# nintendops/DynamicFusion_Body

Hardware: NVIDIA B200
Metric: warped_tsdf_voxels_per_sec (higher is better)
Workload: dtype f32

## Files before the change

### dynamicfusion_body_b200/_capi.py

```python
import ctypes as C
import os

DFB_MAX_K = 8
DFB_MAX_VIEWS = 8
DFB_NODE_REC_FLOATS = 12
DFB_COMM_ID_BYTES = 128
MODE_HYBRID = 0
MODE_EXACT = 1
MODE_FAST_ONLY = 2
MODE_LIST_ONLY = 3
MODE_BRICK_CLASSIFY = 4
MODE_BRICK_STREAM = 5
MODE_BRICK_MIXED = 6
MODE_BRICK_UPDATE = 7

_PKG_DIR = os.path.dirname(os.path.abspath(__file__))
LIB_PATH = os.environ.get("DFB_LIB") or os.path.join(_PKG_DIR, "libdfb_b200.so")

c_f32p = C.POINTER(C.c_float)
c_f64p = C.POINTER(C.c_double)
c_u8p = C.POINTER(C.c_uint8)
c_u16p = C.POINTER(C.c_uint16)
c_u32p = C.POINTER(C.c_uint32)
c_i32p = C.POINTER(C.c_int32)


class Volume(C.Structure):
    _fields_ = [("tsdf", C.c_void_p), ("weight", C.c_void_p),
                ("rx", C.c_int), ("ry", C.c_int), ("rz", C.c_int),
                ("x0", C.c_int), ("x1", C.c_int)]


class WarpField(C.Structure):
    _fields_ = [("node_rec", C.c_void_p), ("node_pos", C.c_void_p), ("node_dq", C.c_void_p),
                ("node_w", C.c_void_p), ("n_nodes", C.c_int), ("k", C.c_int), ("knn", C.c_void_p),
                ("has_lw", C.c_int), ("lw_is_f32", C.c_int), ("lw", C.c_double * 8),
                ("brick_nodes", C.c_void_p), ("brick_count", C.c_void_p), ("brick_pairs", C.c_void_p),
                ("region_nodes", C.c_void_p), ("region_count", C.c_void_p), ("region_pairs", C.c_void_p),
                ("region_rec", C.c_void_p)]


class Views(C.Structure):
    _fields_ = [("n_views", C.c_int), ("depth", C.c_void_p * DFB_MAX_VIEWS),
                ("rows", C.c_int), ("cols", C.c_int),
                ("K", C.c_double * 9), ("Kinv", C.c_double * 9),
                ("has_extrinsics", C.c_int), ("E", (C.c_double * 12) * DFB_MAX_VIEWS)]


class Workspace(C.Structure):
    _fields_ = [("list", C.c_void_p), ("capacity", C.c_uint32), ("counters", C.c_void_p),
                ("brick_cls", C.c_void_p), ("brick_lists", C.c_void_p), ("overflow_bits", C.c_void_p)]


class GNProblem(C.Structure):
    _fields_ = [("n_vert", C.c_int64), ("vertices", C.c_void_p), ("normals", C.c_void_p), ("corr", C.c_void_p),
                ("vert_knn", C.c_void_p), ("n_nodes", C.c_int), ("k", C.c_int), ("node_pos", C.c_void_p),
                ("node_w", C.c_void_p), ("node_nbr", C.c_void_p), ("lw", C.c_double * 8), ("lw_is_f32", C.c_int),
                ("rw", C.c_double), ("huber", C.c_int), ("f_scale", C.c_double), ("order", C.c_void_p)]


class FrameIO(C.Structure):
    _fields_ = [("comm", C.c_void_p), ("comm_prefetch", C.c_void_p), ("root", C.c_int), ("dq_src", C.c_void_p),
                ("prefetch_dst", C.c_void_p), ("prefetch_src", C.c_void_p), ("prefetch_bytes", C.c_int64),
                ("counters_host", C.c_void_p)]


class PointGrid(C.Structure):
    _fields_ = [("pts", C.c_void_p), ("n", C.c_int64), ("origin", C.c_double * 3), ("cell", C.c_double),
                ("dims", C.c_int * 3), ("cell_start", C.c_void_p), ("order", C.c_void_p)]


def declare(lib, prefix="dfb_", device=True):
    vp = C.c_void_p
    sig = {
        "version": ([], C.c_int),
        "last_error": ([], C.c_char_p),
        "nodes_pack": ([vp, vp, vp, C.c_int, vp] + ([vp] if device else []), None if not device else C.c_int),
        "knn_build_volume": ([vp, C.c_int, C.c_int, C.c_int, C.c_int, C.c_int, C.c_int, C.c_int, vp, vp], C.c_int),
        "knn_brick_count": ([C.c_int, C.c_int, C.c_int], C.c_int64),
        "knn_build_volume_radii": ([vp, C.c_int, C.c_int, C.c_int, C.c_int, C.c_int, C.c_int, C.c_int, vp, vp, vp], C.c_int),
        "knn_update_volume": ([vp, C.c_int, C.c_int, C.c_int, C.c_int, C.c_int, C.c_int, C.c_int, C.c_int, vp, vp, vp, vp], C.c_int),
        "brick_nodes_update": ([vp, C.c_int, C.c_int, C.c_int, C.c_int, C.c_int, C.c_int, vp, vp, vp, vp, vp], C.c_int),
        "region_update": ([vp, C.c_int, C.c_int, C.c_int, C.c_int, C.c_int, C.c_int, vp, vp, vp, vp, vp], C.c_int),
        "brick_count": ([C.c_int, C.c_int, C.c_int], C.c_int64),
        "brick_nodes_build": ([vp, C.c_int, C.c_int, C.c_int, C.c_int, C.c_int, C.c_int, vp, vp, vp, vp], C.c_int),
        "region_count": ([C.c_int, C.c_int, C.c_int], C.c_int64),
        "region_build": ([vp, C.c_int, C.c_int, C.c_int, C.c_int, C.c_int, C.c_int, vp, vp, vp, vp], C.c_int),
        "knn_points": ([vp, C.c_int64, vp, C.c_int, C.c_int, vp, vp], C.c_int),
        "tsdf_update_projective": ([C.POINTER(Volume), C.POINTER(WarpField), C.POINTER(Views), C.c_double, C.c_double,
                                    C.c_int, C.POINTER(Workspace), vp, vp, vp], C.c_int),
        "fuse_depth_rigid": ([C.POINTER(Volume), C.c_int, vp, C.c_int, C.c_int, c_f64p, c_f64p, c_f64p, C.c_double,
                              c_f64p, C.c_double, C.c_double, C.c_int, C.POINTER(Workspace), vp, vp, vp], C.c_int),
        "tsdf_update_volume": ([C.POINTER(Volume), C.POINTER(WarpField), vp, C.c_int, C.c_int, C.c_int, C.c_double,
                                C.c_double, C.c_int, C.POINTER(Workspace), vp, vp], C.c_int),
        "warp_points": ([vp, vp, C.c_int64, vp, C.POINTER(WarpField), vp, vp] + ([vp] if device else []), C.c_int),
        "dq_blend_points": ([vp, C.c_int64, vp, C.POINTER(WarpField), vp] + ([vp] if device else []), C.c_int),
        "gn_residuals": ([C.POINTER(GNProblem), vp, C.c_int, vp] + ([vp] if device else []), C.c_int),
        "gn_residuals_lw": ([C.POINTER(GNProblem), vp, C.c_int, c_f64p, C.c_int, vp] + ([vp] if device else []), C.c_int),
        "gn_pattern_rows": ([C.POINTER(GNProblem), vp, vp, vp], C.c_int),
        "gn_pattern_cols": ([C.c_int, vp, vp, vp, vp], C.c_int),
        "gn_normal_eq": ([C.POINTER(GNProblem), vp, vp, vp, C.c_int64, vp, vp, vp] + ([vp] if device else []), C.c_int),
        "gn_lw_normal_eq": ([C.POINTER(GNProblem), vp, c_f64p, vp, vp, vp] + ([vp] if device else []), C.c_int),
        "gn_solve_workspace_doubles": ([C.c_int], C.c_int64),
        "point_grid_scratch_ints": ([C.c_int64], C.c_int64),
        "point_grid_build": ([C.POINTER(PointGrid), vp, vp, vp, vp], C.c_int),
        "point_grid_knn": ([C.POINTER(PointGrid), vp, C.c_int64, C.c_int, vp, vp, vp], C.c_int),
        "corr_select": ([vp, vp, C.c_int64, vp, vp, C.c_int, vp, vp, vp], C.c_int),
        "corr_projective": ([vp, vp, C.c_int64, C.POINTER(Views), C.c_double, C.c_double, vp, vp, vp] + ([vp] if device else []), C.c_int),
        "graph_unsupported": ([vp, C.c_int64, vp, C.c_int, vp, vp, vp, vp], C.c_int),
        "graph_sample_rounds": ([C.POINTER(PointGrid), C.c_double, C.c_int, vp, vp, vp], C.c_int),
        "mc_level_scratch_floats": ([], C.c_int64),
        "mc_level": ([vp, C.c_int64, vp, vp, vp], C.c_int),
        "mc_rows": ([C.c_int, C.c_int, C.c_int], C.c_int64),
        "mc_chunks": ([C.c_int, C.c_int, C.c_int, C.c_int], C.c_int64),
        "mc_count": ([vp, C.c_int, C.c_int, C.c_int, C.c_int, vp, vp, vp, vp, vp], C.c_int),
        "mc_emit": ([vp, C.c_int, C.c_int, C.c_int, C.c_int, vp, vp, vp, vp, vp, vp, vp, vp, vp], C.c_int),
        "gn_solve": ([C.c_int, vp, vp, vp, vp, C.c_double, C.c_int, C.c_double, vp, vp, vp, vp, vp], C.c_int),
        "comm_available": ([], C.c_int),
        "comm_unique_id": ([vp], C.c_int),
        "comm_init": ([C.POINTER(vp), vp, C.c_int, C.c_int, C.c_int], C.c_int),
        "comm_destroy": ([vp], C.c_int),
        "comm_rank": ([vp], C.c_int),
        "comm_world": ([vp], C.c_int),
        "comm_broadcast": ([vp, vp, C.c_int64, C.c_int, vp], C.c_int),
        "comm_broadcast_frame": ([vp, vp, C.c_int64, vp, C.c_int, vp, C.c_int, vp], C.c_int),
        "comm_allreduce_f64": ([vp, vp, C.c_int64, C.c_int, vp], C.c_int),
        "comm_sendrecv": ([vp, vp, C.c_int64, C.c_int, vp, C.c_int64, C.c_int, vp], C.c_int),
        "frame_step_create": ([C.POINTER(vp)], C.c_int),
        "frame_step_destroy": ([vp], None),
        "frame_step_run": ([vp, C.POINTER(Volume), C.POINTER(WarpField), C.POINTER(Views), C.c_double, C.c_double,
                            C.POINTER(Workspace), C.POINTER(FrameIO), vp], C.c_int),
        "frame_step_stats": ([vp, C.POINTER(C.c_int64)], C.c_int),
    }
    for name, (argtypes, restype) in sig.items():
        fn = getattr(lib, prefix + name, None)
        if fn is None:
            continue
        fn.argtypes = argtypes
        fn.restype = restype
    return lib


_lib = None


def lib():
    global _lib
    if _lib is None:
        if not os.path.isfile(LIB_PATH):
            raise ImportError(
                "libdfb_b200.so is not built (%s). There is no CPU fallback: run "
                "`python -m dynamicfusion_body_b200.build` (needs nvcc)." % LIB_PATH)
        _lib = declare(C.CDLL(LIB_PATH))
    return _lib


class DfbError(RuntimeError):
    pass


def check(rc):
    if rc != 0:
        msg = lib().dfb_last_error()
        raise DfbError("libdfb_b200 error %d: %s" % (rc, msg.decode() if msg else "?"))


EXPORTS = [
    "dfb_version", "dfb_last_error", "dfb_nodes_pack", "dfb_knn_build_volume", "dfb_knn_points", "dfb_brick_count", "dfb_brick_nodes_build", "dfb_region_count", "dfb_region_build",
    "dfb_tsdf_update_projective", "dfb_tsdf_update_volume", "dfb_fuse_depth_rigid", "dfb_warp_points", "dfb_dq_blend_points",
    "dfb_gn_residuals", "dfb_gn_residuals_lw", "dfb_gn_pattern_rows", "dfb_gn_pattern_cols", "dfb_gn_normal_eq",
    "dfb_gn_lw_normal_eq", "dfb_gn_solve_workspace_doubles", "dfb_gn_solve",
    "dfb_point_grid_scratch_ints", "dfb_point_grid_build", "dfb_point_grid_knn", "dfb_corr_select", "dfb_corr_projective", "dfb_graph_unsupported", "dfb_graph_sample_rounds",
    "dfb_mc_level_scratch_floats", "dfb_mc_level", "dfb_mc_rows", "dfb_mc_chunks", "dfb_mc_count", "dfb_mc_emit",
    "dfb_knn_brick_count", "dfb_knn_build_volume_radii", "dfb_knn_update_volume", "dfb_brick_nodes_update", "dfb_region_update",
    "dfb_comm_available", "dfb_comm_unique_id", "dfb_comm_init", "dfb_comm_destroy", "dfb_comm_rank", "dfb_comm_world",
    "dfb_comm_broadcast", "dfb_comm_broadcast_frame", "dfb_comm_allreduce_f64", "dfb_comm_sendrecv",
    "dfb_frame_step_create", "dfb_frame_step_destroy", "dfb_frame_step_run", "dfb_frame_step_stats",
]
```

### dynamicfusion_body_b200/csrc/dfb_math.h

```cpp
#pragma once
#include <math.h>
#include <stdint.h>

#if defined(__CUDACC__)
#define DFB_HD __host__ __device__ __forceinline__
#define DFB_HDN inline __host__ __device__
#else
#define DFB_HD inline
#define DFB_HDN inline
#endif

#if !defined(__CUDACC__)
struct float4 { float x, y, z, w; };
#endif

namespace dfb {

#if defined(__CUDA_ARCH__)
DFB_HD float fmul(float a, float b) { return __fmul_rn(a, b); }
DFB_HD float fadd(float a, float b) { return __fadd_rn(a, b); }
DFB_HD float fsub(float a, float b) { return __fsub_rn(a, b); }
DFB_HD float fdiv(float a, float b) { return __fdiv_rn(a, b); }
DFB_HD float fsqrt(float a) { return __fsqrt_rn(a); }
DFB_HD double dmul(double a, double b) { return __dmul_rn(a, b); }
DFB_HD double dadd(double a, double b) { return __dadd_rn(a, b); }
DFB_HD double dsub(double a, double b) { return __dsub_rn(a, b); }
DFB_HD double ddiv(double a, double b) { return __ddiv_rn(a, b); }
DFB_HD double dsqrt(double a) { return __dsqrt_rn(a); }
DFB_HD double drint(double a) { return rint(a); }
#else
DFB_HD float fmul(float a, float b) { volatile float r = a * b; return r; }
DFB_HD float fadd(float a, float b) { volatile float r = a + b; return r; }
DFB_HD float fsub(float a, float b) { volatile float r = a - b; return r; }
DFB_HD float fdiv(float a, float b) { volatile float r = a / b; return r; }
DFB_HD float fsqrt(float a) { volatile float r = sqrtf(a); return r; }
DFB_HD double dmul(double a, double b) { volatile double r = a * b; return r; }
DFB_HD double dadd(double a, double b) { volatile double r = a + b; return r; }
DFB_HD double dsub(double a, double b) { volatile double r = a - b; return r; }
DFB_HD double ddiv(double a, double b) { volatile double r = a / b; return r; }
DFB_HD double dsqrt(double a) { volatile double r = sqrt(a); return r; }
DFB_HD double drint(double a) { return nearbyint(a); }
#endif

struct OpsF {
    typedef float T;
    static DFB_HD T mul(T a, T b) { return fmul(a, b); }
    static DFB_HD T add(T a, T b) { return fadd(a, b); }
    static DFB_HD T sub(T a, T b) { return fsub(a, b); }
};
struct OpsD {
    typedef double T;
    static DFB_HD T mul(T a, T b) { return dmul(a, b); }
    static DFB_HD T add(T a, T b) { return dadd(a, b); }
    static DFB_HD T sub(T a, T b) { return dsub(a, b); }
};

template <class Ops>
DFB_HD void qmul_ref(const typename Ops::T* q1, const typename Ops::T* q0, double* out) {
    typedef typename Ops::T T;
    const T w0 = q0[0], x0 = q0[1], y0 = q0[2], z0 = q0[3];
    const T w1 = q1[0], x1 = q1[1], y1 = q1[2], z1 = q1[3];
    out[0] = (double)Ops::add(Ops::sub(Ops::sub(Ops::mul(-x1, x0), Ops::mul(y1, y0)), Ops::mul(z1, z0)), Ops::mul(w1, w0));
    out[1] = (double)Ops::add(Ops::sub(Ops::add(Ops::mul(x1, w0), Ops::mul(y1, z0)), Ops::mul(z1, y0)), Ops::mul(w1, x0));
    out[2] = (double)Ops::add(Ops::add(Ops::add(Ops::mul(-x1, z0), Ops::mul(y1, w0)), Ops::mul(z1, x0)), Ops::mul(w1, y0));
    out[3] = (double)Ops::add(Ops::add(Ops::sub(Ops::mul(x1, y0), Ops::mul(y1, x0)), Ops::mul(z1, w0)), Ops::mul(w1, z0));
}

DFB_HDN void dqb_warp_ref(const double* dq, bool dq_is_f32, const double* pos, double* out) {
    const float vr[4] = {1.f, 0.f, 0.f, 0.f};
    const float vd[4] = {0.f, (float)pos[0], (float)pos[1], (float)pos[2]};
    double qr[4], qd[4], t0[4], t1[4];
    if (dq_is_f32) {
        const float r[4] = {(float)dq[0], (float)dq[1], (float)dq[2], (float)dq[3]};
        const float d[4] = {(float)dq[4], (float)dq[5], (float)dq[6], (float)dq[7]};
        qmul_ref<OpsF>(r, vr, qr);
        qmul_ref<OpsF>(r, vd, t0);
        qmul_ref<OpsF>(d, vr, t1);
    } else {
        const double vrd[4] = {1.0, 0.0, 0.0, 0.0};
        const double vdd[4] = {0.0, (double)vd[1], (double)vd[2], (double)vd[3]};
        qmul_ref<OpsD>(dq, vrd, qr);
        qmul_ref<OpsD>(dq, vdd, t0);
        qmul_ref<OpsD>(dq + 4, vrd, t1);
    }
    for (int i = 0; i < 4; ++i) qd[i] = dadd(t0[i], t1[i]);
    const double cr[4] = {dq[0], -dq[1], -dq[2], -dq[3]};
    const double cd[4] = {-dq[4], dq[5], dq[6], dq[7]};
    qmul_ref<OpsD>(qr, cd, t0);
    qmul_ref<OpsD>(qd, cr, t1);
    out[0] = dadd(t0[1], t1[1]);
    out[1] = dadd(t0[2], t1[2]);
    out[2] = dadd(t0[3], t1[3]);
}

DFB_HDN void dqb_warp_closed(const double* q, const double* pos, double* out) {
    const double p[3] = {(double)(float)pos[0], (double)(float)pos[1], (double)(float)pos[2]};
    const double w = q[0], x = q[1], y = q[2], z = q[3], dw = q[4], dx = q[5], dy = q[6], dz = q[7];
    const double s = w * w - (x * x + y * y + z * z);
    const double vp = x * p[0] + y * p[1] + z * p[2];
    const double cx = y * p[2] - z * p[1], cy = z * p[0] - x * p[2], cz = x * p[1] - y * p[0];
    out[0] = s * p[0] + 2.0 * (vp * x + w * cx + (w * dx - dw * x + (y * dz - z * dy)));
    out[1] = s * p[1] + 2.0 * (vp * y + w * cy + (w * dy - dw * y + (z * dx - x * dz)));
    out[2] = s * p[2] + 2.0 * (vp * z + w * cz + (w * dz - dw * z + (x * dy - y * dx)));
}

DFB_HDN void dqb_warp_normal_ref(const double* dq, const double* n, double* out) {
    const double rq[8] = {dq[0], dq[1], dq[2], dq[3], 0.0, 0.0, 0.0, 0.0};
    dqb_warp_ref(rq, false, n, out);
}

DFB_HD float norm3_f32_ref(float ax, float ay, float az, float bx, float by, float bz) {
    const float dx = fsub(ax, bx), dy = fsub(ay, by), dz = fsub(az, bz);
    const double s = dadd(dadd((double)fmul(dx, dx), (double)fmul(dy, dy)), (double)fmul(dz, dz));
    return fsqrt((float)s);
}

template <int KT = 0>
DFB_HDN void dq_blend_ref(const float* p, const int* ids, int k_rt, const float* node_pos, const float* node_dq,
                          const float* node_w, double* se3, float* wi_out, double* n2_out = nullptr, const float4* rec = nullptr) {
    double b[8] = {0, 0, 0, 0, 0, 0, 0, 0};
    float wi = 0.f;
    const int k = KT > 0 ? KT : k_rt;
    double wts[KT > 0 ? KT : 1];
    if (KT > 0) {
#pragma unroll
        for (int i = 0; i < (KT > 0 ? KT : 1); ++i) {
            float nx, ny, nz;
            if (rec) { const float4 r0 = rec[3 * (size_t)ids[i]]; nx = r0.x; ny = r0.y; nz = r0.z; }
            else { const float* np_ = node_pos + 3 * (size_t)ids[i]; nx = np_[0]; ny = np_[1]; nz = np_[2]; }
            const float nrm = norm3_f32_ref(p[0], p[1], p[2], nx, ny, nz);
            const float q = fdiv(nrm, fmul(2.0f, node_w[ids[i]]));
            wts[i] = exp((double)fmul(-1.0f, fmul(q, q)));
        }
    }
#pragma unroll
    for (int i = 0; i < k; ++i) {
        const int id = ids[i];
        float npx = 0.f, npy = 0.f, npz = 0.f;
        if (!(KT > 0) || wi_out) {
            if (rec) { const float4 r0 = rec[3 * (size_t)id]; npx = r0.x; npy = r0.y; npz = r0.z; }
            else { const float* np_ = node_pos + 3 * (size_t)id; npx = np_[0]; npy = np_[1]; npz = np_[2]; }
        }
        double w;
        if (KT > 0) {
            w = wts[KT > 0 ? i : 0];
        } else {
            const float nrm = norm3_f32_ref(p[0], p[1], p[2], npx, npy, npz);
            const float two_w = fmul(2.0f, node_w[id]);
            const float q = fdiv(nrm, two_w);
            const float arg = fmul(-1.0f, fmul(q, q));
            w = exp((double)arg);
        }
        const float wf = (float)w;
        float dqi[8];
        if (rec) {
            const float4 r1 = rec[3 * (size_t)id + 1], r2 = rec[3 * (size_t)id + 2];
            dqi[0] = r1.x; dqi[1] = r1.y; dqi[2] = r1.z; dqi[3] = r1.w; dqi[4] = r2.x; dqi[5] = r2.y; dqi[6] = r2.z; dqi[7] = r2.w;
        } else {
            const float* dq_ = node_dq + 8 * (size_t)id;
            for (int c = 0; c < 8; ++c) dqi[c] = dq_[c];
        }
        for (int c = 0; c < 8; ++c) b[c] = dadd(b[c], (double)fmul(wf, dqi[c]));
        if (wi_out) {
            const float nrm2 = norm3_f32_ref(npx, npy, npz, p[0], p[1], p[2]);
            const float term = fdiv(nrm2, (float)k);
            wi = (i == 0) ? term : fadd(wi, term);
        }
    }
    if (wi_out) *wi_out = wi;
    double s = 0.0;
    for (int c = 0; c < 8; ++c) s = dadd(s, dmul(b[c], b[c]));
    if (n2_out) {
        *n2_out = s;
        if (s == 0.0) {
            se3[0] = 1.0;
            for (int c = 1; c < 8; ++c) se3[c] = 0.0;
            *n2_out = 1.0;
        } else {
            for (int c = 0; c < 8; ++c) se3[c] = b[c];
        }
        return;
    }
    const double nrm8 = dsqrt(s);
    if (nrm8 == 0.0) {
        se3[0] = 1.0;
        for (int c = 1; c < 8; ++c) se3[c] = 0.0;
        return;
    }
    for (int c = 0; c < 8; ++c) se3[c] = ddiv(b[c], nrm8);
}

template <int KT = 0>
DFB_HDN void warp_ref(const float* p, const float* nrm_in, const int* ids, int k, const float* node_pos,
                      const float* node_dq, const float* node_w, const double* lw, bool has_lw, bool lw_is_f32,
                      double* out_p, double* out_n, float* wi_out, bool closed_form = false, const float4* rec = nullptr) {
    double pd[3] = {(double)p[0], (double)p[1], (double)p[2]};
    double se3[8];
    if (k > 0) {
        if (closed_form && !(nrm_in && out_n)) {
            double n2;
            dq_blend_ref<KT>(p, ids, k, node_pos, node_dq, node_w, se3, wi_out, &n2, rec);
            dqb_warp_closed(se3, pd, out_p);
            const double inv = 1.0 / n2;
            out_p[0] *= inv; out_p[1] *= inv; out_p[2] *= inv;
        } else {
            dq_blend_ref<KT>(p, ids, k, node_pos, node_dq, node_w, se3, wi_out, nullptr, rec);
            if (closed_form) dqb_warp_closed(se3, pd, out_p);
            else dqb_warp_ref(se3, false, pd, out_p);
        }
    } else {
        out_p[0] = pd[0]; out_p[1] = pd[1]; out_p[2] = pd[2];
    }
    if (has_lw) {
        double t[3] = {out_p[0], out_p[1], out_p[2]};
        if (closed_form && !lw_is_f32) dqb_warp_closed(lw, t, out_p);
        else dqb_warp_ref(lw, lw_is_f32, t, out_p);
    }
    if (nrm_in && out_n) {
        double nd[3] = {(double)nrm_in[0], (double)nrm_in[1], (double)nrm_in[2]};
        if (k > 0) dqb_warp_normal_ref(se3, nd, out_n);
        else { out_n[0] = nd[0]; out_n[1] = nd[1]; out_n[2] = nd[2]; }
        if (has_lw) {
            double t[3] = {out_n[0], out_n[1], out_n[2]};
            dqb_warp_normal_ref(lw, t, out_n);
        }
    }
}

DFB_HD double dot3_ref(const double* r, double a, double b, double c) {
    return dadd(dadd(dmul(r[0], a), dmul(r[1], b)), dmul(r[2], c));
}
DFB_HD double dot4_ref(const double* r, double a, double b, double c, double d) {
    return dadd(dadd(dadd(dmul(r[0], a), dmul(r[1], b)), dmul(r[2], c)), dmul(r[3], d));
}

DFB_HD float fast_exp2(float x) {
#if defined(__CUDA_ARCH__)
    float y;
    asm("ex2.approx.ftz.f32 %0, %1;" : "=f"(y) : "f"(x));
    return y;
#else
    return exp2f(x);
#endif
}
DFB_HD float fast_rcp(float x) {
#if defined(__CUDA_ARCH__)
    float y;
    asm("rcp.approx.ftz.f32 %0, %1;" : "=f"(y) : "f"(x));
    return y;
#else
    return 1.0f / x;
#endif
}

DFB_HD void clamp_update(float& v, float& w, float tdist, float wmax, float scale) {
#if defined(__CUDA_ARCH__)
    v = __fmul_rn(__fmaf_rn(__fmul_rn(scale, v), w, tdist), fast_rcp(__fmul_rn(scale, __fadd_rn(1.0f, w))));
#else
    v = fmul(fmaf(fmul(scale, v), w, tdist), fast_rcp(fmul(scale, fadd(1.0f, w))));
#endif
    w = fminf(fadd(1.0f, w), wmax);
}

DFB_HDN int project_fuse_ref(const double* lpos, const float* depth, int rows, int cols, const double* K,
                             const double* Kinv, double tdist, double scale, double wmax, double* v, double* w) {
    const double p0 = dot3_ref(K, lpos[0], lpos[1], lpos[2]);
    const double p1 = dot3_ref(K + 3, lpos[0], lpos[1], lpos[2]);
    const double p2 = dot3_ref(K + 6, lpos[0], lpos[1], lpos[2]);
    if (p2 == 0.0) return 0;
    const double u = ddiv(p0, p2), vv = ddiv(p1, p2);
    if (!(u >= 0.0 && u < (double)(cols - 1) && vv >= 0.0 && vv < (double)(rows - 1))) return 0;
    const long ui = (long)drint(u), vi = (long)drint(vv);
    const double z = -1.0 * (double)depth[(size_t)vi * cols + ui];
    if (!(z > 0.0)) return 2;
    const double c2 = dot3_ref(Kinv + 6, dmul(z, u), dmul(z, vv), dmul(z, 1.0));
    const double tl = dsub(c2, lpos[2]);
    if (!(tl > -1.0 * tdist)) return 2;
    if (!(tl < tdist)) {
        float vf = (float)*v, wf = (float)*w;
        clamp_update(vf, wf, (float)tdist, (float)wmax, (float)scale);
        *v = (double)vf;
        *w = (double)wf;
        return 3;
    }
    const double m = tl;
    const double wt = *w;
    *v = ddiv(dadd(dmul(dmul(scale, *v), wt), dmul(m, 1.0)), dmul(scale, dadd(1.0, wt)));
    const double s = dadd(1.0, wt);
    *w = (wmax < s) ? wmax : s;
    return 3;
}

DFB_HDN int assoc_projective_ref(const double* w, const double* m, const float* const* depth, int n_views, int rows, int cols,
                                 const double* K, const double* Kinv, const double* E, double max_distance, double min_normal_dot,
                                 double* cost_out, double* corr_out) {
    int best = -1;
    double best_cost = INFINITY, bc[3] = {0.0, 0.0, 0.0};
    const double md2 = dmul(max_distance, max_distance);
    for (int v = 0; v < n_views; ++v) {
        const double* Ev = E ? E + 12 * v : nullptr;
        double l[3], ln[3];
        for (int r = 0; r < 3; ++r) {
            l[r] = Ev ? dot4_ref(Ev + 4 * r, w[0], w[1], w[2], 1.0) : w[r];
            ln[r] = Ev ? dot3_ref(Ev + 4 * r, m[0], m[1], m[2]) : m[r];
        }
        if (!(dot3_ref(ln, l[0], l[1], l[2]) < 0.0)) continue;
        const double p0 = dot3_ref(K, l[0], l[1], l[2]);
        const double p1 = dot3_ref(K + 3, l[0], l[1], l[2]);
        const double p2 = dot3_ref(K + 6, l[0], l[1], l[2]);
        if (p2 == 0.0) continue;
        const double u = ddiv(p0, p2), vv = ddiv(p1, p2);
        if (!(u >= 0.0 && u < (double)(cols - 1) && vv >= 0.0 && vv < (double)(rows - 1))) continue;
        const long ui = (long)drint(u), vi = (long)drint(vv);
        if (ui < 1 || ui > cols - 2 || vi < 1 || vi > rows - 2) continue;
        const float* D = depth[v];
        const long pu[5] = {ui, ui - 1, ui + 1, ui, ui};
        const long pv[5] = {vi, vi, vi, vi - 1, vi + 1};
        double z[5];
        bool ok = true;
        for (int j = 0; j < 5 && ok; ++j) {
            z[j] = -1.0 * (double)D[(size_t)pv[j] * cols + pu[j]];
            ok = z[j] > 0.0 && (j == 0 || fabs(dsub(z[j], z[0])) <= max_distance);
        }
        if (!ok) continue;
        double P[5][3];
        for (int j = 0; j < 5; ++j) {
            const double a = dmul(z[j], (double)pu[j]), b = dmul(z[j], (double)pv[j]), c2 = dmul(z[j], 1.0);
            for (int r = 0; r < 3; ++r) P[j][r] = dot3_ref(Kinv + 3 * r, a, b, c2);
        }
        const double* c = P[0];
        const double du[3] = {dsub(P[2][0], P[1][0]), dsub(P[2][1], P[1][1]), dsub(P[2][2], P[1][2])};
        const double dv[3] = {dsub(P[4][0], P[3][0]), dsub(P[4][1], P[3][1]), dsub(P[4][2], P[3][2])};
        double g[3] = {dsub(dmul(du[1], dv[2]), dmul(du[2], dv[1])), dsub(dmul(du[2], dv[0]), dmul(du[0], dv[2])),
                       dsub(dmul(du[0], dv[1]), dmul(du[1], dv[0]))};
        const double gc = dot3_ref(g, c[0], c[1], c[2]);
        if (gc == 0.0) continue;
        if (gc > 0.0) { g[0] = -g[0]; g[1] = -g[1]; g[2] = -g[2]; }
        const double d[3] = {dsub(l[0], c[0]), dsub(l[1], c[1]), dsub(l[2], c[2])};
        if (!(dot3_ref(d, d[0], d[1], d[2]) <= md2)) continue;
        const double nl = dsqrt(dot3_ref(ln, ln[0], ln[1], ln[2])), ng = dsqrt(dot3_ref(g, g[0], g[1], g[2]));
        if (!(dot3_ref(ln, g[0], g[1], g[2]) >= dmul(dmul(min_normal_dot, nl), ng))) continue;
        const double cost = fabs(dot3_ref(ln, d[0], d[1], d[2]));
        if (!(cost < best_cost)) continue;
        best = v;
        best_cost = cost;
        if (Ev) {
            const double e[3] = {dsub(c[0], Ev[3]), dsub(c[1], Ev[7]), dsub(c[2], Ev[11])};
            for (int j = 0; j < 3; ++j) bc[j] = dadd(dadd(dmul(Ev[j], e[0]), dmul(Ev[4 + j], e[1])), dmul(Ev[8 + j], e[2]));
        } else {
            bc[0] = c[0]; bc[1] = c[1]; bc[2] = c[2];
        }
    }
    *cost_out = best_cost;
    corr_out[0] = bc[0]; corr_out[1] = bc[1]; corr_out[2] = bc[2];
    return best;
}

DFB_HDN bool interpolate_tsdf_ref(const double* pos, const float* t, int rx, int ry, int rz, double* out) {
    const double mn = fmin(fmin(pos[0], pos[1]), pos[2]);
    if (!(mn >= 0.0) || pos[0] > rx - 1 || pos[1] > ry - 1 || pos[2] > rz - 1) return false;
    if (!(pos[0] == pos[0] && pos[1] == pos[1] && pos[2] == pos[2])) return false;
    const double fx = floor(pos[0]), fy = floor(pos[1]), fz = floor(pos[2]);
    const long x0 = (long)fx, y0 = (long)fy, z0 = (long)fz;
    const long x1 = (long)ceil(pos[0]), y1 = (long)ceil(pos[1]), z1 = (long)ceil(pos[2]);
    const double xd = dsub(pos[0], fx), yd = dsub(pos[1], fy), zd = dsub(pos[2], fz);
#define DFB_T(a, b, c) ((double)t[((size_t)(a) * ry + (size_t)(b)) * rz + (size_t)(c)])
    const double c000 = DFB_T(x0, y0, z0), c100 = DFB_T(x1, y0, z0), c001 = DFB_T(x0, y1, z0), c101 = DFB_T(x1, y1, z0);
    const double c010 = DFB_T(x0, y0, z1), c110 = DFB_T(x1, y0, z1), c011 = DFB_T(x0, y1, z1), c111 = DFB_T(x1, y1, z1);
#undef DFB_T
    const double ix = dsub(1.0, xd), iy = dsub(1.0, yd), iz = dsub(1.0, zd);
    const double c00 = dadd(dmul(c000, ix), dmul(c100, xd));
    const double c01 = dadd(dmul(c001, ix), dmul(c101, xd));
    const double c10 = dadd(dmul(c010, ix), dmul(c110, xd));
    const double c11 = dadd(dmul(c011, ix), dmul(c111, xd));
    const double c0 = dadd(dmul(c00, iy), dmul(c10, yd));
    const double c1 = dadd(dmul(c01, iy), dmul(c11, yd));
    *out = dadd(dmul(c0, iz), dmul(c1, zd));
    return true;
}

DFB_HD bool volume_fuse_ref(bool valid, double tl, float wi_f, int k, double tdist, double wmax, double* v, double* w) {
    if (!valid || !(tl > -1.0 * tdist)) return false;
    if (k == 0) {
        const double wt = *w;
        const double m = (tl < tdist) ? tl : tdist;
        *v = ddiv(dadd(dmul(*v, wt), dmul(m, 1.0)), dadd(1.0, wt));
        const double s = dadd(1.0, wt);
        *w = (wmax < s) ? wmax : s;
        return true;
    }
    const double wi = (double)wi_f;
    const double wt = (*w == 0.0) ? wi : *w;
    const double term = (tl < tdist) ? dmul(tl, wi) : (double)fmul((float)tdist, wi_f);
    *v = ddiv(dadd(dmul(*v, wt), term), dadd(wi, wt));
    const double s = dadd(wi, wt);
    *w = (wmax < s) ? wmax : s;
    return true;
}

struct Affine34 {
    float m[12];
};

DFB_HD void dq_apply_unnormalised(const float* b, float px, float py, float pz, float* o) {
    const float w = b[0], x = b[1], y = b[2], z = b[3], dw = b[4], dx = b[5], dy = b[6], dz = b[7];
    const float vv = x * x + y * y + z * z;
    const float s = w * w - vv;
    const float vp = x * px + y * py + z * pz;
    const float cx = y * pz - z * py, cy = z * px - x * pz, cz = x * py - y * px;
    const float tx = w * dx - dw * x + (y * dz - z * dy);
    const float ty = w * dy - dw * y + (z * dx - x * dz);
    const float tz = w * dz - dw * z + (x * dy - y * dx);
    o[0] = s * px + 2.f * (vp * x + w * cx + tx);
    o[1] = s * py + 2.f * (vp * y + w * cy + ty);
    o[2] = s * pz + 2.f * (vp * z + w * cz + tz);
}

inline void dq_to_affine(const double* q, double* A ) {
    const double w = q[0], x = q[1], y = q[2], z = q[3], dw = q[4], dx = q[5], dy = q[6], dz = q[7];
    const double s = w * w - (x * x + y * y + z * z);
    A[0] = s + 2 * x * x;        A[1] = 2 * (x * y - w * z);  A[2] = 2 * (x * z + w * y);
    A[4] = 2 * (x * y + w * z);  A[5] = s + 2 * y * y;        A[6] = 2 * (y * z - w * x);
    A[8] = 2 * (x * z - w * y);  A[9] = 2 * (y * z + w * x);  A[10] = s + 2 * z * z;
    A[3] = 2 * (w * dx - dw * x + (y * dz - z * dy));
    A[7] = 2 * (w * dy - dw * y + (z * dx - x * dz));
    A[11] = 2 * (w * dz - dw * z + (x * dy - y * dx));
}

}
```

### dynamicfusion_body_b200/csrc/dfb_params.h

```cpp
#pragma once
#include <math.h>
#include <stdarg.h>
#include <stdio.h>
#include <string.h>

#include "../../include/dfb.h"
#include "dfb_voxel.h"

namespace dfb {

void set_error(const char* fmt, ...);

#define DFB_REQUIRE(cond, ...)            \
    do {                                  \
        if (!(cond)) {                    \
            dfb::set_error(__VA_ARGS__);  \
            return DFB_ERR_INVALID;       \
        }                                 \
    } while (0)

inline void mat34_mul(const double* A, const double* B, double* C) {
    for (int r = 0; r < 3; ++r)
        for (int c = 0; c < 4; ++c) {
            double s = 0;
            for (int j = 0; j < 3; ++j) s += A[4 * r + j] * B[4 * j + c];
            if (c == 3) s += A[4 * r + 3];
            C[4 * r + c] = s;
        }
}

inline void k_mul34(const double* K, const double* A, double* C) {
    for (int r = 0; r < 3; ++r)
        for (int c = 0; c < 4; ++c) {
            double s = 0;
            for (int j = 0; j < 3; ++j) s += K[3 * r + j] * A[4 * j + c];
            C[4 * r + c] = s;
        }
}

inline double affine_corner_mag(const double* A, double ex, double ey, double ez) {
    double mag = 0;
    for (int c = 0; c < 8; ++c) {
        const double p[3] = {(c & 1) * ex, ((c >> 1) & 1) * ey, ((c >> 2) & 1) * ez};
        for (int r = 0; r < 3; ++r) {
            const double v = A[4 * r] * p[0] + A[4 * r + 1] * p[1] + A[4 * r + 2] * p[2] + A[4 * r + 3];
            mag = fmax(mag, fabs(v));
            for (int j = 0; j < 3; ++j) mag = fmax(mag, fabs(A[4 * r + j] * p[j]));
            mag = fmax(mag, fabs(A[4 * r + 3]));
        }
    }
    return mag;
}

inline int validate_volume(const dfb_volume* vol) {
    DFB_REQUIRE(vol && vol->tsdf && vol->weight, "volume pointers are null");
    DFB_REQUIRE(vol->rx > 0 && vol->ry > 0 && vol->rz > 0, "bad volume resolution");
    DFB_REQUIRE(vol->x0 >= 0 && vol->x1 > vol->x0 && vol->x1 <= vol->rx, "bad slab [%d,%d) of %d", vol->x0, vol->x1, vol->rx);
    DFB_REQUIRE(vol->ry <= 65535 && (vol->x1 - vol->x0) <= 65535, "ry and slab thickness must be <= 65535");
    DFB_REQUIRE((size_t)(vol->x1 - vol->x0) * vol->ry * vol->rz < ((size_t)1 << 32), "slab has >= 2^32 voxels");
    return DFB_OK;
}

inline int validate_warpfield(const dfb_warpfield* wf, bool need_knn) {
    DFB_REQUIRE(wf, "warpfield is null");
    DFB_REQUIRE(wf->k >= 0 && wf->k <= DFB_MAX_K, "k=%d out of range [0,%d]", wf->k, DFB_MAX_K);
    if (wf->k > 0) {
        DFB_REQUIRE(wf->node_rec && wf->node_pos && wf->node_dq && wf->node_w, "node arrays are null");
        DFB_REQUIRE(wf->n_nodes >= wf->k && wf->n_nodes <= 65535, "n_nodes=%d must be in [k,65535]", wf->n_nodes);
        if (need_knn) DFB_REQUIRE(wf->knn, "knn table is null");
    }
    return DFB_OK;
}

inline int validate_ws(const dfb_workspace* ws) {
    DFB_REQUIRE(ws && ws->counters, "workspace/counters are null");
    DFB_REQUIRE(ws->capacity == 0 || ws->list, "workspace list is null");
    return DFB_OK;
}

inline void fill_common(ProjParams& P, const dfb_volume* vol, const dfb_workspace* ws, double tdist, double wmax,
                        uint8_t* mask_out, uint8_t* frustum_out) {
    P.tsdf = vol->tsdf; P.weight = vol->weight;
    P.rx = vol->rx; P.ry = vol->ry; P.rz = vol->rz; P.x0 = vol->x0; P.x1 = vol->x1;
    P.tdist = fabs(tdist); P.wmax = wmax;
    P.tdist_f = (float)fabs(tdist); P.wmax_f = (float)wmax;
    P.list = ws->list; P.capacity = ws->capacity; P.counters = ws->counters; P.overflow_bits = ws->overflow_bits;
    P.mask_out = mask_out; P.frustum_out = frustum_out;
}

inline void fill_intrinsics(ProjParams& P, const double* K, const double* Kinv) {
    for (int i = 0; i < 9; ++i) { P.K[i] = K[i]; P.Kinv[i] = Kinv[i]; }
    for (int i = 0; i < 3; ++i) P.kin[i] = (float)Kinv[6 + i];
    for (int i = 0; i < 6; ++i) P.kf[i] = (float)K[i];
    P.k_pinhole = (K[6] == 0.0 && K[7] == 0.0 && K[8] == 1.0) ? 1 : 0;
    P.knorm = (float)fmax(fabs(K[0]) + fabs(K[1]) + fabs(K[2]), fabs(K[3]) + fabs(K[4]) + fabs(K[5]));
    P.kin_uv = (float)(fabs(Kinv[6]) + fabs(Kinv[7]));
    P.ezf = (float)(fmax(1.0, fabs(K[6]) + fabs(K[7]) + fabs(K[8])) * 1.000001);
}

static const double kIdent34[12] = {1, 0, 0, 0, 0, 1, 0, 0, 0, 0, 1, 0};

inline int build_projective(ProjParams& P, const dfb_volume* vol, const dfb_warpfield* wf, const dfb_views* views,
                            double tdist, double wmax, int mode, const dfb_workspace* ws, uint8_t* mask_out,
                            uint8_t* frustum_out) {
    if (int r = validate_volume(vol)) return r;
    if (int r = validate_warpfield(wf, true)) return r;
    if (int r = validate_ws(ws)) return r;
    DFB_REQUIRE(views && views->n_views >= 1 && views->n_views <= DFB_MAX_VIEWS, "n_views out of range");
    DFB_REQUIRE(views->rows >= 2 && views->cols >= 2, "depth map too small");
    DFB_REQUIRE(mode >= DFB_MODE_HYBRID && mode <= DFB_MODE_BRICK_UPDATE, "bad mode");
    DFB_REQUIRE(wf->k > 0, "projective update needs k >= 1 (use dfb_fuse_depth_rigid for the rigid path)");
    DFB_REQUIRE(tdist != 0, "truncation distance must be non-zero");
    memset(&P, 0, sizeof(P));
    fill_common(P, vol, ws, tdist, wmax, mask_out, frustum_out);
    P.scale = 1.0;
    P.node_rec = reinterpret_cast<const float4*>(wf->node_rec);
    P.node_pos = wf->node_pos; P.node_dq = wf->node_dq; P.node_w = wf->node_w; P.knn = wf->knn; P.k = wf->k;
    P.has_lw = wf->has_lw; P.lw_is_f32 = wf->lw_is_f32;
    for (int i = 0; i < 8; ++i) P.lw[i] = wf->lw[i];
    P.n_views = views->n_views; P.rows = views->rows; P.cols = views->cols; P.has_E = views->has_extrinsics;
    fill_intrinsics(P, views->K, views->Kinv);
    double A[12];
    if (wf->has_lw) dq_to_affine(wf->lw, A);
    else memcpy(A, kIdent34, sizeof(A));
    double mag = fmax(fmax(vol->rx, vol->ry), vol->rz);
    mag = fmax(mag, affine_corner_mag(A, vol->rx, vol->ry, vol->rz));
    double tnorm = 0.0;
    for (int v = 0; v < views->n_views; ++v) {
        DFB_REQUIRE(views->depth[v], "depth[%d] is null", v);
        P.depth[v] = views->depth[v];
        double T[12], PK[12];
        if (views->has_extrinsics) {
            for (int i = 0; i < 12; ++i) P.E[v][i] = views->E[v][i];
            mat34_mul(views->E[v], A, T);
        } else {
            memcpy(T, A, sizeof(T));
        }
        mag = fmax(mag, affine_corner_mag(T, vol->rx, vol->ry, vol->rz));
        k_mul34(views->K, T, PK);
        for (int i = 0; i < 12; ++i) P.vf[v].P[i] = (float)PK[i];
        for (int i = 0; i < 4; ++i) P.vf[v].L[i] = (float)T[8 + i];
        for (int i = 0; i < 12; ++i) P.vf[v].T[i] = (float)T[i];
        for (int r = 0; r < 3; ++r) tnorm = fmax(tnorm, fabs(T[4 * r]) + fabs(T[4 * r + 1]) + fabs(T[4 * r + 2]));
    }
    P.tnorm = (float)(tnorm * 1.000001);
    P.coord_mag = (float)(2.0 * mag + 8.0);
    return DFB_OK;
}

inline int build_rigid(ProjParams& P, const dfb_volume* vol, int tsdf_res, const float* depth, int rows, int cols,
                       const double* lw34, const double* K, const double* Kinv, double scale, const double* center,
                       double tdist, double wmax, int mode, const dfb_workspace* ws, uint8_t* mask_out,
                       uint8_t* frustum_out) {
    if (int r = validate_volume(vol)) return r;
    if (int r = validate_ws(ws)) return r;
    DFB_REQUIRE(depth && lw34 && K && Kinv && center, "null pointer");
    DFB_REQUIRE(rows >= 2 && cols >= 2, "depth map too small");
    DFB_REQUIRE(mode >= DFB_MODE_HYBRID && mode <= DFB_MODE_BRICK_UPDATE, "bad mode");
    DFB_REQUIRE(scale > 0, "scale must be positive");
    DFB_REQUIRE(tdist != 0, "truncation distance must be non-zero");
    memset(&P, 0, sizeof(P));
    fill_common(P, vol, ws, tdist, wmax, mask_out, frustum_out);
    P.scale = scale;
    P.rigid = 1;
    P.k = 0;
    P.g_scale = scale; P.g_half = tsdf_res / 2.0;
    for (int i = 0; i < 3; ++i) P.g_center[i] = center[i];
    for (int i = 0; i < 12; ++i) P.lw34[i] = lw34[i];
    P.n_views = 1; P.rows = rows; P.cols = cols; P.has_E = 0;
    P.depth[0] = depth;
    fill_intrinsics(P, K, Kinv);
    const double G[12] = {scale, 0, 0, center[0] - scale * P.g_half, 0, scale, 0, center[1] - scale * P.g_half,
                          0, 0, scale, center[2] - scale * P.g_half};
    double T[12], PK[12];
    mat34_mul(lw34, G, T);
    k_mul34(K, T, PK);
    for (int i = 0; i < 12; ++i) P.vf[0].P[i] = (float)PK[i];
    for (int i = 0; i < 4; ++i) P.vf[0].L[i] = (float)T[8 + i];
    for (int i = 0; i < 12; ++i) P.vf[0].T[i] = (float)T[i];
    const double mag = fmax(affine_corner_mag(G, vol->rx, vol->ry, vol->rz), affine_corner_mag(T, vol->rx, vol->ry, vol->rz));
    P.coord_mag = (float)(2.0 * mag + 8.0 * scale);
    return DFB_OK;
}

inline int build_volume(VolParams& P, const dfb_volume* vol, const dfb_warpfield* wf, const float* curr, int cx, int cy,
                        int cz, double tdist, double wmax, int mode, const dfb_workspace* ws, uint8_t* mask_out) {
    if (int r = validate_volume(vol)) return r;
    if (int r = validate_warpfield(wf, true)) return r;
    if (int r = validate_ws(ws)) return r;
    DFB_REQUIRE(curr && cx > 0 && cy > 0 && cz > 0, "tsdf of live frame has not been loaded");
    DFB_REQUIRE(mode >= DFB_MODE_HYBRID && mode <= DFB_MODE_BRICK_UPDATE, "bad mode");
    DFB_REQUIRE(tdist != 0, "truncation distance must be non-zero");
    memset(&P, 0, sizeof(P));
    P.tsdf = vol->tsdf; P.weight = vol->weight;
    P.rx = vol->rx; P.ry = vol->ry; P.rz = vol->rz; P.x0 = vol->x0; P.x1 = vol->x1;
    P.node_rec = reinterpret_cast<const float4*>(wf->node_rec);
    P.node_pos = wf->node_pos; P.node_dq = wf->node_dq; P.node_w = wf->node_w; P.knn = wf->knn; P.k = wf->k;
    P.has_lw = wf->has_lw; P.lw_is_f32 = wf->lw_is_f32;
    for (int i = 0; i < 8; ++i) P.lw[i] = wf->lw[i];
    double A[12];
    if (wf->has_lw) dq_to_affine(wf->lw, A);
    else memcpy(A, kIdent34, sizeof(A));
    for (int i = 0; i < 12; ++i) P.A[i] = (float)A[i];
    P.curr = curr; P.cx = cx; P.cy = cy; P.cz = cz;
    P.tdist = fabs(tdist); P.wmax = wmax; P.tdist_f = (float)fabs(tdist); P.wmax_f = (float)wmax;
    double mag = fmax(fmax(vol->rx, vol->ry), vol->rz);
    mag = fmax(mag, affine_corner_mag(A, vol->rx, vol->ry, vol->rz));
    P.coord_mag = (float)(2.0 * mag + 8.0);
    P.list = ws->list; P.capacity = ws->capacity; P.counters = ws->counters; P.overflow_bits = ws->overflow_bits;
    P.mask_out = mask_out;
    return DFB_OK;
}

}
```

### dynamicfusion_body_b200/csrc/dfb_voxel.h

```cpp
#pragma once
#include "dfb_math.h"

namespace dfb {

enum { CLS_SKIP = 0, CLS_CLAMP = 1, CLS_UNCERTAIN = 2 };

struct ViewFast {
    float P[12];
    float L[4];
    float T[12];
};

struct ProjParams {
    float* tsdf;
    float* weight;
    int rx, ry, rz, x0, x1;
    const float4* node_rec;
    const float* node_pos;
    const float* node_dq;
    const float* node_w;
    const uint16_t* knn;
    int k;
    int has_lw, lw_is_f32;
    double lw[8];
    int rigid;
    double g_scale, g_half, g_center[3];
    double lw34[12];
    float G[12];
    int n_views, rows, cols, has_E;
    const float* depth[8];
    double K[9], Kinv[9];
    double E[8][12];
    ViewFast vf[8];
    float kf[6];
    int k_pinhole;
    float kin[3];
    float tnorm;
    float knorm;
    float ezf;
    float kin_uv;
    float coord_mag;
    double tdist, wmax, scale;
    float tdist_f, wmax_f;
    uint32_t* list;
    uint32_t capacity;
    uint32_t* counters;
    uint32_t* overflow_bits;
    uint8_t* mask_out;
    uint8_t* frustum_out;
};

struct VolParams {
    float* tsdf;
    float* weight;
    int rx, ry, rz, x0, x1;
    const float4* node_rec;
    const float* node_pos;
    const float* node_dq;
    const float* node_w;
    const uint16_t* knn;
    int k;
    int has_lw, lw_is_f32;
    double lw[8];
    float A[12];
    const float* curr;
    int cx, cy, cz;
    double tdist, wmax;
    float tdist_f, wmax_f, coord_mag;
    uint32_t* list;
    uint32_t capacity;
    uint32_t* counters;
    uint32_t* overflow_bits;
    uint8_t* mask_out;
};

struct RecGlobal {
    const float4* p;
    DFB_HD float4 ld(size_t i) const { return p[i]; }
};
#if defined(__CUDACC__)
struct RecShared {
    uint32_t base;
    __device__ __forceinline__ float4 ld(size_t i) const {
        float4 r;
        asm("ld.shared.v4.f32 {%0, %1, %2, %3}, [%4];" : "=f"(r.x), "=f"(r.y), "=f"(r.z), "=f"(r.w) : "r"(base + (uint32_t)i * 16u));
        return r;
    }
};
#endif

template <int KMAX, class Rec>
DFB_HD bool blend_warp_fast(const Rec rec, const uint16_t* ids, int k_rt, float px, float py, float pz, float* out,
                            float* amin_out, bool exact_k = false) {
    const int k = exact_k ? KMAX : k_rt;
    float a[KMAX];
    float amax = -3.0e38f, amin = 0.f;
#pragma unroll
    for (int i = 0; i < KMAX; ++i) {
        if (i < k) {
            const float4 r0 = rec.ld(3 * (size_t)ids[i]);
            const float dx = px - r0.x, dy = py - r0.y, dz = pz - r0.z;
            a[i] = (dx * dx + dy * dy + dz * dz) * r0.w;
            amax = fmaxf(amax, a[i]);
            amin = fminf(amin, a[i]);
        }
    }
    *amin_out = amin * 0.69314718f;
    if (!(amax > -125.f)) return false;
    float b[8] = {0.f, 0.f, 0.f, 0.f, 0.f, 0.f, 0.f, 0.f};
#pragma unroll
    for (int i = 0; i < KMAX; ++i) {
        if (i < k) {
            const float w = fast_exp2(a[i] - amax);
            const float4 r1 = rec.ld(3 * (size_t)ids[i] + 1);
            const float4 r2 = rec.ld(3 * (size_t)ids[i] + 2);
            b[0] += w * r1.x; b[1] += w * r1.y; b[2] += w * r1.z; b[3] += w * r1.w;
            b[4] += w * r2.x; b[5] += w * r2.y; b[6] += w * r2.z; b[7] += w * r2.w;
        }
    }
    float n2 = 0.f;
#pragma unroll
    for (int c = 0; c < 8; ++c) n2 += b[c] * b[c];
    if (!(n2 > 1e-30f)) return false;
    float o[3];
    dq_apply_unnormalised(b, px, py, pz, o);
    const float inv = fast_rcp(n2);
    out[0] = o[0] * inv; out[1] = o[1] * inv; out[2] = o[2] * inv;
    return true;
}

DFB_HD float pos_err_bound(float coord_mag, float amin_nat) {
    return 1.1920929e-7f * coord_mag * (32.f - 4.f * amin_nat);
}

DFB_HD int classify_view(float pu, float pv, float pz, float lz, float e, const float* depth, int rows, int cols,
                         const float* kin, float knorm, float ezf, float kin_uv, float tdist, int* frustum_bit) {
    *frustum_bit = 0;
    const float apz = fabsf(pz);
    const float ez = e * ezf;
    if (!(apz > 64.f * ez)) return CLS_UNCERTAIN;
    const float inv = fast_rcp(pz);
    const float u = pu * inv, v = pv * inv;
    const float ainv = fabsf(inv) * 1.02f;
    const float eu = (knorm * e + fabsf(u) * ez) * ainv + 4.8e-7f * fabsf(u) + 1e-6f;
    const float ev = (knorm * e + fabsf(v) * ez) * ainv + 4.8e-7f * fabsf(v) + 1e-6f;
    const float umax = (float)(cols - 1), vmax = (float)(rows - 1);
    if (u < -eu || u >= umax + eu || v < -ev || v >= vmax + ev) return CLS_SKIP;
    if (!(u >= eu && u < umax - eu && v >= ev && v < vmax - ev)) return CLS_UNCERTAIN;
    *frustum_bit = 1;
    const int u0 = (int)rintf(u - eu), u1 = (int)rintf(u + eu);
    const int v0 = (int)rintf(v - ev), v1 = (int)rintf(v + ev);
    const float kz = kin[0] * u + kin[1] * v + kin[2];
    const float et0 = kin_uv * (eu + ev) + 4.8e-7f * fabsf(kz);
    const float et1 = e + 2.4e-7f * fabsf(lz);
    if ((u0 != u1 && v0 != v1) || u1 - u0 > 1 || v1 - v0 > 1) return CLS_UNCERTAIN;
    const float za = -depth[(size_t)v0 * cols + u0];
    const float zb = -depth[(size_t)v1 * cols + u1];
    const float tla = za * kz - lz, tlb = zb * kz - lz;
    const float eta = fabsf(za) * et0 + et1, etb = fabsf(zb) * et0 + et1;
    const bool skip_a = !(za > 0.f) || tla < -tdist - eta, skip_b = !(zb > 0.f) || tlb < -tdist - etb;
    const bool clamp_a = za > 0.f && tla > tdist + eta, clamp_b = zb > 0.f && tlb > tdist + etb;
    if (skip_a && skip_b) return CLS_SKIP;
    if (clamp_a && clamp_b) return CLS_CLAMP;
    return CLS_UNCERTAIN;
}

template <int KT = 0>
DFB_HDN void voxel_projective_exact(const ProjParams& P, int x, int y, int z, const uint16_t* ids16, float* v_io,
                                    float* w_io, int* mask, int* frus) {
    double base[3];
    if (P.rigid) {
        const double idx[3] = {(double)x, (double)y, (double)z};
        for (int c = 0; c < 3; ++c) base[c] = dadd(dmul(P.g_scale, dsub(idx[c], P.g_half)), P.g_center[c]);
    } else {
        const float p[3] = {(float)x, (float)y, (float)z};
        int ids[8];
        if (KT > 0) {
#pragma unroll
            for (int i = 0; i < (KT > 0 ? KT : 1); ++i) ids[i] = ids16[i];
        } else {
            for (int i = 0; i < P.k; ++i) ids[i] = ids16[i];
        }
#ifndef DFB_EXACT_REC
#define DFB_EXACT_REC 0
#endif
        warp_ref<KT>(p, nullptr, ids, P.k, P.node_pos, P.node_dq, P.node_w, P.lw, P.has_lw != 0, P.lw_is_f32 != 0, base,
                     nullptr, nullptr, true, DFB_EXACT_REC ? P.node_rec : nullptr);
    }
    double v = (double)*v_io, w = (double)*w_io;
    int m = 0, f = 0;
    for (int vi = 0; vi < P.n_views; ++vi) {
        double lpos[3];
        if (P.rigid) {
            for (int r = 0; r < 3; ++r) lpos[r] = dot4_ref(P.lw34 + 4 * r, base[0], base[1], base[2], 1.0);
        } else if (P.has_E) {
            for (int r = 0; r < 3; ++r) lpos[r] = dot4_ref(P.E[vi] + 4 * r, base[0], base[1], base[2], 1.0);
        } else {
            lpos[0] = base[0]; lpos[1] = base[1]; lpos[2] = base[2];
        }
        const int r = project_fuse_ref(lpos, P.depth[vi], P.rows, P.cols, P.K, P.Kinv, P.tdist, P.scale, P.wmax, &v, &w);
        if (r & 1) m |= 1 << vi;
        if (r & 2) f |= 1 << vi;
    }
    *v_io = (float)v;
    *w_io = (float)w;
    *mask = m;
    *frus = f;
}

template <int KMAX, bool EXACTK, bool ONEVIEW, class Rec>
DFB_HD int voxel_projective_classify_rec(const ProjParams& P, int x, int y, int z, const uint16_t* ids, int* mask, int* frus,
                                         int views, int m0, int f0, const Rec rec) {
    float pw[3];
    float e;
    if (P.rigid) {
        pw[0] = (float)x; pw[1] = (float)y; pw[2] = (float)z;
        e = 1.1920929e-7f * P.coord_mag * 32.f;
    } else {
        float amin;
        if (!blend_warp_fast<KMAX>(rec, ids, P.k, (float)x, (float)y, (float)z, pw, &amin, EXACTK)) return CLS_UNCERTAIN;
        e = pos_err_bound(P.coord_mag, amin);
    }
    int m = m0, f = f0;
    const int nv = ONEVIEW ? 1 : P.n_views;
#pragma unroll 1
    for (int vi = 0; vi < nv; ++vi) {
        if (!ONEVIEW && !((views >> vi) & 1)) continue;
        const ViewFast& V = P.vf[ONEVIEW ? 0 : vi];
        const float pu = V.P[0] * pw[0] + V.P[1] * pw[1] + V.P[2] * pw[2] + V.P[3];
        const float pv = V.P[4] * pw[0] + V.P[5] * pw[1] + V.P[6] * pw[2] + V.P[7];
        const float pz = V.P[8] * pw[0] + V.P[9] * pw[1] + V.P[10] * pw[2] + V.P[11];
        const float lz = V.L[0] * pw[0] + V.L[1] * pw[1] + V.L[2] * pw[2] + V.L[3];
        int fb;
        const int c = classify_view(pu, pv, pz, lz, e, P.depth[ONEVIEW ? 0 : vi], P.rows, P.cols, P.kin, P.knorm, P.ezf, P.kin_uv, P.tdist_f, &fb);
        if (c == CLS_UNCERTAIN) return CLS_UNCERTAIN;
        if (c == CLS_CLAMP) m |= 1 << vi;
        if (fb) f |= 1 << vi;
    }
    *mask = m;
    *frus = f;
    return m ? CLS_CLAMP : CLS_SKIP;
}

template <int KMAX, bool EXACTK = false, bool ONEVIEW = false>
DFB_HD int voxel_projective_classify(const ProjParams& P, int x, int y, int z, const uint16_t* ids, int* mask, int* frus,
                                     int views = 0xff, int m0 = 0, int f0 = 0) {
    const RecGlobal rec = {P.node_rec};
    return voxel_projective_classify_rec<KMAX, EXACTK, ONEVIEW>(P, x, y, z, ids, mask, frus, views, m0, f0, rec);
}

template <int KT = 0>
DFB_HDN bool voxel_volume_exact(const VolParams& P, int x, int y, int z, const uint16_t* ids16, float* v_io, float* w_io) {
    const float p[3] = {(float)x, (float)y, (float)z};
    int ids[8];
    if (KT > 0) {
#pragma unroll
        for (int i = 0; i < (KT > 0 ? KT : 1); ++i) ids[i] = ids16[i];
    } else {
        for (int i = 0; i < P.k; ++i) ids[i] = ids16[i];
    }
    double pw[3];
    float wi = 0.f;
    warp_ref<KT>(p, nullptr, ids, P.k, P.node_pos, P.node_dq, P.node_w, P.lw, P.has_lw != 0, P.lw_is_f32 != 0, pw, nullptr, &wi, true);
    double tl = 0.0;
    const bool valid = interpolate_tsdf_ref(pw, P.curr, P.cx, P.cy, P.cz, &tl);
    double v = (double)*v_io, w = (double)*w_io;
    const bool upd = volume_fuse_ref(valid, tl, wi, P.k, P.tdist, P.wmax, &v, &w);
    if (upd) { *v_io = (float)v; *w_io = (float)w; }
    return upd;
}

template <int KMAX>
DFB_HD int voxel_volume_classify(const VolParams& P, int x, int y, int z, const uint16_t* ids, float* wi_out) {
    float pw[3];
    float e;
    const float px = (float)x, py = (float)y, pz = (float)z;
    if (P.k > 0) {
        float amin;
        const RecGlobal rec = {P.node_rec};
        if (!blend_warp_fast<KMAX>(rec, ids, P.k, px, py, pz, pw, &amin)) return CLS_UNCERTAIN;
        e = pos_err_bound(P.coord_mag, amin);
    } else {
        pw[0] = px; pw[1] = py; pw[2] = pz;
        e = 1.1920929e-7f * P.coord_mag * 32.f;
    }
    const float qx = P.A[0] * pw[0] + P.A[1] * pw[1] + P.A[2] * pw[2] + P.A[3];
    const float qy = P.A[4] * pw[0] + P.A[5] * pw[1] + P.A[6] * pw[2] + P.A[7];
    const float qz = P.A[8] * pw[0] + P.A[9] * pw[1] + P.A[10] * pw[2] + P.A[11];
    const float mx = (float)(P.cx - 1), my = (float)(P.cy - 1), mz = (float)(P.cz - 1);
    if (qx < -e || qy < -e || qz < -e || qx > mx + e || qy > my + e || qz > mz + e) return CLS_SKIP;
    if (!(qx >= e && qy >= e && qz >= e && qx <= mx - e && qy <= my - e && qz <= mz - e)) return CLS_UNCERTAIN;
    const int x0 = (int)floorf(qx - e), x1 = (int)ceilf(qx + e);
    const int y0 = (int)floorf(qy - e), y1 = (int)ceilf(qy + e);
    const int z0 = (int)floorf(qz - e), z1 = (int)ceilf(qz + e);
    float mn = 3.0e38f, mxc = -3.0e38f;
    for (int a = x0; a <= x1; ++a)
        for (int b = y0; b <= y1; ++b)
            for (int c = z0; c <= z1; ++c) {
                const float t = P.curr[((size_t)a * P.cy + b) * P.cz + c];
                mn = fminf(mn, t);
                mxc = fmaxf(mxc, t);
            }
    if (mxc <= -P.tdist_f * 1.000001f) return CLS_SKIP;
    if (!(mn >= P.tdist_f)) return CLS_UNCERTAIN;
    if (P.k > 0) {
        float wi = 0.f;
        for (int i = 0; i < P.k; ++i) {
            const float4 r0 = P.node_rec[3 * (size_t)ids[i]];
            const float nr = norm3_f32_ref(r0.x, r0.y, r0.z, px, py, pz);
            const float term = fdiv(nr, (float)P.k);
            wi = (i == 0) ? term : fadd(wi, term);
        }
        *wi_out = wi;
    } else {
        *wi_out = 1.f;
    }
    return CLS_CLAMP;
}

}
```

### dynamicfusion_body_b200/csrc/knn.cu

```cuda
#include <stdlib.h>

#include "common.h"
#include "dfb_math.h"

using namespace dfb;

namespace {

constexpr int TILE = 1024;

template <int KMAX>
struct TopK {
    float d[KMAX + 1];
    int id[KMAX + 1];
    __device__ __forceinline__ void init() {
#pragma unroll
        for (int j = 0; j <= KMAX; ++j) { d[j] = 3.0e38f; id[j] = 0; }
    }
    __device__ __forceinline__ void insert(float v, int i, int kk) {
        if (!(v < d[kk])) return;
        d[kk] = v; id[kk] = i;
#pragma unroll
        for (int j = KMAX; j > 0; --j) {
            if (j <= kk && d[j] < d[j - 1]) {
// ... 36 lines not shown
        __syncthreads();
        if (active) {
#pragma unroll 4
            for (int j = 0; j < cnt; ++j) {
                const float4 p = tile[j];
                const float dx = qx - p.x, dy = qy - p.y, dz = qz - p.z;
                const float d2 = dx * dx + dy * dy + dz * dz;
                top.insert(d2, base + j, kk);
            }
        }
    }
    if (!active) return;
    bool ambiguous = false;
#pragma unroll
    for (int j = 0; j < KMAX; ++j)
        if (j < kk && top.d[j + 1] - top.d[j] <= 4.0e-6f * top.d[j + 1]) ambiguous = true;
    if (ambiguous) {
        knn_exact_f64<KMAX>(qx, qy, qz, node_pos, n, k, out);
    } else {
#pragma unroll
        for (int j = 0; j < KMAX; ++j)
            if (j < k) out[j] = top.id[j];
    }
}

template <int KMAX>
__global__ void __launch_bounds__(256) knn_volume_kernel(const float* node_pos, int n, int k, int ry, int rz, int x0,
                                                         uint16_t* knn) {
    __shared__ float4 tile[TILE];
    const int z = blockIdx.x * blockDim.x + threadIdx.x;
    const int y = blockIdx.y;
    const int xs = blockIdx.z;
    const bool in = z < rz;
    int out[KMAX];
    knn_query<KMAX>((float)(xs + x0), (float)y, (float)z, in, node_pos, n, k, tile, out);
    if (!in) return;
    const size_t i = ((size_t)xs * ry + y) * rz + z;
    if (KMAX == 4 && k == 4) {
        uint2 r;
        r.x = (uint32_t)out[0] | ((uint32_t)out[1] << 16);
        r.y = (uint32_t)out[2] | ((uint32_t)out[3] << 16);
        reinterpret_cast<uint2*>(knn)[i] = r;
    } else {
#pragma unroll
        for (int j = 0; j < KMAX; ++j)
            if (j < k) knn[i * (size_t)k + j] = (uint16_t)out[j];
    }
}


constexpr int KB = 8;
constexpr int KCAP = 1024;

template <int KMAX>
__device__ __noinline__ void knn_exact_f64_list(float qx, float qy, float qz, const float4* cand, int nc, int k, int* out) {
    double bd[KMAX];
    int bi[KMAX];
    for (int j = 0; j < KMAX; ++j) { bd[j] = 1.0e300; bi[j] = 0x7fffffff; }
    for (int t = 0; t < nc; ++t) {
        const float4 p = cand[t];
        const int id = __float_as_int(p.w);
        const double dx = dfb::dsub((double)qx, (double)p.x), dy = dfb::dsub((double)qy, (double)p.y), dz = dfb::dsub((double)qz, (double)p.z);
        const double d2 = dfb::dadd(dfb::dadd(dfb::dmul(dx, dx), dfb::dmul(dy, dy)), dfb::dmul(dz, dz));
        if (!(d2 < bd[k - 1] || (d2 == bd[k - 1] && id < bi[k - 1]))) continue;
        int j = k - 1;
        while (j > 0 && (d2 < bd[j - 1] || (d2 == bd[j - 1] && id < bi[j - 1]))) { bd[j] = bd[j - 1]; bi[j] = bi[j - 1]; --j; }
        bd[j] = d2; bi[j] = id;
    }
    for (int j = 0; j < k; ++j) out[j] = bi[j];
}

template <int KMAX>
__global__ void __launch_bounds__(128) knn_brick_kernel(const float* node_pos, int n, int k, int sx, int ry, int rz, int x0, int nby, int nbz,
                                                        uint16_t* knn, float* brick_T, int n_old, uint8_t* dirty) {
    __shared__ float4 cand[KCAP];
    __shared__ float wtop[4][KMAX];
    __shared__ int ncand;
    __shared__ float T2s;
    const int b = blockIdx.x;
    const int bz = b % nbz, by = (b / nbz) % nby, bxs = b / (nbz * nby);
    const int xlo = bxs * KB, ylo = by * KB, zlo = bz * KB;
    const int xhi = min(xlo + KB, sx) - 1, yhi = min(ylo + KB, ry) - 1, zhi = min(zlo + KB, rz) - 1;
    const float cx = 0.5f * (xlo + xhi) + (float)x0, cy = 0.5f * (ylo + yhi), cz = 0.5f * (zlo + zhi);
    const float hx = 0.5f * (xhi - xlo), hy = 0.5f * (yhi - ylo), hz = 0.5f * (zhi - zlo);
    const float hd = sqrtf(hx * hx + hy * hy + hz * hz);
    const int lane = threadIdx.x & 31, wid = threadIdx.x >> 5;
    if (n_old > 0) {
        if (dirty[b] != 2) return;
        __syncthreads();
        if (threadIdx.x == 0) dirty[b] = 1;
    } else if (threadIdx.x == 0 && dirty) {
        dirty[b] = 1;
    }
    float lt[KMAX];
#pragma unroll
    for (int j = 0; j < KMAX; ++j) lt[j] = 3.0e38f;
    for (int t = threadIdx.x; t < n; t += blockDim.x) {
        const float dx = node_pos[3 * t] - cx, dy = node_pos[3 * t + 1] - cy, dz = node_pos[3 * t + 2] - cz;
        float v = dx * dx + dy * dy + dz * dz;
#pragma unroll
        for (int j = 0; j < KMAX; ++j)
            if (j < k && v < lt[j]) { const float tmp = lt[j]; lt[j] = v; v = tmp; }
    }
    for (int j = 0; j < k; ++j) {
        float m = lt[0];
        for (int o = 16; o > 0; o >>= 1) m = fminf(m, __shfl_xor_sync(0xffffffffu, m, o));
        const unsigned who = __ballot_sync(0xffffffffu, lt[0] == m);
        if (lane == __ffs(who) - 1) {
#pragma unroll
            for (int q = 0; q < KMAX - 1; ++q) lt[q] = lt[q + 1];
            lt[KMAX - 1] = 3.0e38f;
        }
        if (lane == 0) wtop[wid][j] = m;
    }
    if (threadIdx.x == 0) ncand = 0;
    __syncthreads();
    if (threadIdx.x == 0) {
        float all[4 * KMAX];
        int m = 0;
        for (int w = 0; w < 4; ++w)
            for (int j = 0; j < k; ++j) all[m++] = wtop[w][j];
        for (int a = 1; a < m; ++a) {
            const float v = all[a];
            int q = a - 1;
            while (q >= 0 && all[q] > v) { all[q + 1] = all[q]; --q; }
            all[q + 1] = v;
        }
        const float T = sqrtf(all[k - 1]) * 1.00001f + 2.f * hd + 1e-3f;
        T2s = T * T * 1.00001f;
        if (brick_T) brick_T[b] = T;
    }
    __syncthreads();
    const float T2 = T2s;
    for (int t = threadIdx.x; t < n; t += blockDim.x) {
        const float px = node_pos[3 * t], py = node_pos[3 * t + 1], pz = node_pos[3 * t + 2];
        const float dx = px - cx, dy = py - cy, dz = pz - cz;
        if (dx * dx + dy * dy + dz * dz <= T2) {
            const int pos = atomicAdd(&ncand, 1);
            if (pos < KCAP) cand[pos] = make_float4(px, py, pz, __int_as_float(t));
        }
    }
    __syncthreads();
    const int nc = ncand;
    const bool overflow = nc > KCAP;
    TopK<KMAX> top[4];
    float qx[4], qy[4], qz[4];
    bool in[4];
#pragma unroll
    for (int q = 0; q < 4; ++q) {
        const int j = threadIdx.x * 4 + q;
        const int z = zlo + (j & 7), y = ylo + ((j >> 3) & 7), xs = xlo + (j >> 6);
        in[q] = xs < sx && y < ry && z < rz;
        qx[q] = (float)(xs + x0); qy[q] = (float)y; qz[q] = (float)z;
        top[q].init();
    }
    const int ntot = overflow ? n : nc;
    const int kk = (ntot > k) ? k : k - 1;
    if (!overflow) {
        for (int t = 0; t < nc; ++t) {
            const float4 p = cand[t];
#pragma unroll
            for (int q = 0; q < 4; ++q) {
                const float dx = qx[q] - p.x, dy = qy[q] - p.y, dz = qz[q] - p.z;
                top[q].insert(dx * dx + dy * dy + dz * dz, __float_as_int(p.w), kk);
            }
        }
    } else {
        for (int base = 0; base < n; base += KCAP) {
            const int cnt = min(KCAP, n - base);
            __syncthreads();
            for (int t = threadIdx.x; t < cnt; t += blockDim.x)
                cand[t] = make_float4(node_pos[3 * (base + t)], node_pos[3 * (base + t) + 1], node_pos[3 * (base + t) + 2], __int_as_float(base + t));
            __syncthreads();
            for (int t = 0; t < cnt; ++t) {
                const float4 p = cand[t];
#pragma unroll
                for (int q = 0; q < 4; ++q) {
                    const float dx = qx[q] - p.x, dy = qy[q] - p.y, dz = qz[q] - p.z;
                    top[q].insert(dx * dx + dy * dy + dz * dz, base + t, kk);
                }
            }
        }
    }
#pragma unroll
    for (int q = 0; q < 4; ++q) {
        if (!in[q]) continue;
        int out[KMAX];
        bool ambiguous = false;
#pragma unroll
        for (int a = 0; a < KMAX; ++a)
            if (a < kk && top[q].d[a + 1] - top[q].d[a] <= 4.0e-6f * top[q].d[a + 1]) ambiguous = true;
        if (ambiguous) {
            if (overflow) knn_exact_f64<KMAX>(qx[q], qy[q], qz[q], node_pos, n, k, out);
            else knn_exact_f64_list<KMAX>(qx[q], qy[q], qz[q], cand, nc, k, out);
        } else {
#pragma unroll
            for (int a = 0; a < KMAX; ++a)
                if (a < k) out[a] = top[q].id[a];
        }
        const int j = threadIdx.x * 4 + q;
        const int z = zlo + (j & 7), y = ylo + ((j >> 3) & 7), xs = xlo + (j >> 6);
        const size_t i = ((size_t)xs * ry + y) * rz + z;
        if (KMAX == 4 && k == 4) {
            uint2 r;
            r.x = (uint32_t)out[0] | ((uint32_t)out[1] << 16);
            r.y = (uint32_t)out[2] | ((uint32_t)out[3] << 16);
            reinterpret_cast<uint2*>(knn)[i] = r;
        } else {
#pragma unroll
            for (int a = 0; a < KMAX; ++a)
                if (a < k) knn[i * (size_t)k + a] = (uint16_t)out[a];
        }
    }
}

constexpr int KNEW = 48;
template <int KMAX>
__global__ void __launch_bounds__(128) knn_merge_kernel(const float* node_pos, int n_old, int n, int k, int sx, int ry, int rz, int x0, int nby, int nbz,
                                                        uint16_t* knn, const float* brick_T, uint8_t* dirty) {
    __shared__ float4 newc[KNEW];
    __shared__ int n_new_s, changed_s;
    const int b = blockIdx.x;
    const int bz = b % nbz, by = (b / nbz) % nby, bxs = b / (nbz * nby);
    const int xlo = bxs * KB, ylo = by * KB, zlo = bz * KB;
    const int xhi = min(xlo + KB, sx) - 1, yhi = min(ylo + KB, ry) - 1, zhi = min(zlo + KB, rz) - 1;
    const float cx = 0.5f * (xlo + xhi) + (float)x0, cy = 0.5f * (ylo + yhi), cz = 0.5f * (zlo + zhi);
    if (threadIdx.x == 0) { n_new_s = 0; changed_s = 0; }
    __syncthreads();
    const float T = brick_T[b];
    const float T2 = T * T * 1.00001f;
    for (int t = n_old + threadIdx.x; t < n; t += blockDim.x) {
        const float px = node_pos[3 * t], py = node_pos[3 * t + 1], pz = node_pos[3 * t + 2];
        const float dx = px - cx, dy = py - cy, dz = pz - cz;
        if (dx * dx + dy * dy + dz * dz <= T2) {
            const int pos = atomicAdd(&n_new_s, 1);
            if (pos < KNEW) newc[pos] = make_float4(px, py, pz, __int_as_float(t));
        }
    }
    __syncthreads();
    const int m = n_new_s;
    if (m == 0 || m > KNEW) {
        if (threadIdx.x == 0) dirty[b] = m == 0 ? 0 : 2;
        return;
    }
    if (threadIdx.x == 0) {
        for (int a = 1; a < m; ++a) {
            const float4 v = newc[a];
            int q = a - 1;
            while (q >= 0 && __float_as_int(newc[q].w) > __float_as_int(v.w)) { newc[q + 1] = newc[q]; --q; }
            newc[q + 1] = v;
        }
    }
    __syncthreads();
    bool changed = false;
    for (int q = 0; q < 4; ++q) {
        const int j = threadIdx.x * 4 + q;
        const int z = zlo + (j & 7), y = ylo + ((j >> 3) & 7), xs = xlo + (j >> 6);
        if (!(xs < sx && y < ry && z < rz)) continue;
        const size_t i = ((size_t)xs * ry + y) * rz + z;
        const double qx = (double)(float)(xs + x0), qy = (double)y, qz = (double)z;
        int id[KMAX];
        double d[KMAX];
#pragma unroll
        for (int a = 0; a < KMAX; ++a) {
            id[a] = 0; d[a] = 1.0e300;
            if (a < k) {
                id[a] = knn[i * (size_t)k + a];
                const float* np_ = node_pos + 3 * (size_t)id[a];
                const double dx = dfb::dsub(qx, (double)np_[0]), dy = dfb::dsub(qy, (double)np_[1]), dz = dfb::dsub(qz, (double)np_[2]);
                d[a] = dfb::dadd(dfb::dadd(dfb::dmul(dx, dx), dfb::dmul(dy, dy)), dfb::dmul(dz, dz));
            }
        }
        bool ch = false;
        for (int t = 0; t < m; ++t) {
            const float4 p = newc[t];
            const double dx = dfb::dsub(qx, (double)p.x), dy = dfb::dsub(qy, (double)p.y), dz = dfb::dsub(qz, (double)p.z);
            const double dn = dfb::dadd(dfb::dadd(dfb::dmul(dx, dx), dfb::dmul(dy, dy)), dfb::dmul(dz, dz));
            if (!(dn < d[k - 1])) continue;
            int idn = __float_as_int(p.w);
            double dcur = dn;
            bool ins = false;
#pragma unroll
            for (int a = 0; a < KMAX; ++a) {
                if (a < k) {
                    if (!ins && dcur < d[a]) ins = true;
                    if (ins) {
                        const double td = d[a]; d[a] = dcur; dcur = td;
                        const int ti = id[a]; id[a] = idn; idn = ti;
                    }
                }
            }
            ch = true;
        }
        if (ch) {
#pragma unroll
            for (int a = 0; a < KMAX; ++a)
                if (a < k) knn[i * (size_t)k + a] = (uint16_t)id[a];
            changed = true;
        }
    }
    if (changed) changed_s = 1;
    __syncthreads();
    if (threadIdx.x == 0) dirty[b] = changed_s ? 1 : 0;
}

template <int KMAX>
__global__ void __launch_bounds__(256) knn_points_kernel(const float* pts, int64_t m, const float* node_pos, int n, int k,
                                                         int32_t* idx) {
    __shared__ float4 tile[TILE];
    const int64_t t = (int64_t)blockIdx.x * blockDim.x + threadIdx.x;
    const bool in = t < m;
    const int64_t tt = in ? t : 0;
    int out[KMAX];
    knn_query<KMAX>(pts[3 * tt], pts[3 * tt + 1], pts[3 * tt + 2], in, node_pos, n, k, tile, out);
    if (!in) return;
#pragma unroll
    for (int j = 0; j < KMAX; ++j)
        if (j < k) idx[t * k + j] = out[j];
}

}

namespace {
int knn_build(const float* node_pos, int n_old, int n_nodes, int k, int rx, int ry, int rz, int x0, int x1, uint16_t* knn, float* brick_T,
              uint8_t* dirty, dfb_stream_t stream) {
    DFB_REQUIRE(node_pos && knn, "null pointer");
    DFB_REQUIRE(k >= 1 && k <= DFB_MAX_K, "k=%d out of range [1,%d]", k, DFB_MAX_K);
    DFB_REQUIRE(n_nodes >= k && n_nodes <= 65535, "n_nodes=%d must be in [k,65535]", n_nodes);
    DFB_REQUIRE(rx > 0 && ry > 0 && rz > 0 && x0 >= 0 && x1 > x0 && x1 <= rx, "bad grid / slab");
    DFB_REQUIRE(ry <= 65535 && (x1 - x0) <= 65535, "ry and slab thickness must be <= 65535");
    DFB_REQUIRE(n_old == 0 || (n_old >= k && n_old <= n_nodes && brick_T), "incremental build needs the radii of a table over >= k nodes");
    cudaStream_t s = (cudaStream_t)stream;
    const char* env = getenv("DFB_KNN_BRUTE");
    const int brute = (env && atoi(env)) ? 1 : 0;
    const int64_t nbx = (x1 - x0 + KB - 1) / KB, nby = (ry + KB - 1) / KB, nbz = (rz + KB - 1) / KB;
    if ((brute && n_old == 0 && !brick_T) || nbx * nby * nbz >= ((int64_t)1 << 31)) {
        DFB_REQUIRE(n_old == 0 && !brick_T, "slab too large for the brick build");
        const int threads = rz >= 256 ? 256 : ((rz + 31) / 32) * 32;
        const dim3 grid((rz + threads - 1) / threads, ry, x1 - x0);
        if (k <= 4) knn_volume_kernel<4><<<grid, threads, 0, s>>>(node_pos, n_nodes, k, ry, rz, x0, knn);
        else knn_volume_kernel<8><<<grid, threads, 0, s>>>(node_pos, n_nodes, k, ry, rz, x0, knn);
        DFB_LAUNCH_CHECK("knn_volume_kernel");
        return DFB_OK;
    }
    const unsigned nb = (unsigned)(nbx * nby * nbz);
    if (n_old > 0) {
        if (k <= 4) knn_merge_kernel<4><<<nb, 128, 0, s>>>(node_pos, n_old, n_nodes, k, x1 - x0, ry, rz, x0, (int)nby, (int)nbz, knn, brick_T, dirty);
        else knn_merge_kernel<8><<<nb, 128, 0, s>>>(node_pos, n_old, n_nodes, k, x1 - x0, ry, rz, x0, (int)nby, (int)nbz, knn, brick_T, dirty);
        DFB_LAUNCH_CHECK("knn_merge_kernel");
        if (n_nodes - n_old <= KNEW) return DFB_OK;
    }
    if (k <= 4) knn_brick_kernel<4><<<nb, 128, 0, s>>>(node_pos, n_nodes, k, x1 - x0, ry, rz, x0, (int)nby, (int)nbz, knn, brick_T, n_old, dirty);
    else knn_brick_kernel<8><<<nb, 128, 0, s>>>(node_pos, n_nodes, k, x1 - x0, ry, rz, x0, (int)nby, (int)nbz, knn, brick_T, n_old, dirty);
    DFB_LAUNCH_CHECK("knn_brick_kernel");
    return DFB_OK;
}
}

extern "C" int dfb_knn_build_volume(const float* node_pos, int n_nodes, int k, int rx, int ry, int rz, int x0, int x1,
                                    uint16_t* knn, dfb_stream_t stream) {
    return knn_build(node_pos, 0, n_nodes, k, rx, ry, rz, x0, x1, knn, nullptr, nullptr, stream);
}

extern "C" int64_t dfb_knn_brick_count(int slab_x, int ry, int rz) {
    return (int64_t)((slab_x + KB - 1) / KB) * ((ry + KB - 1) / KB) * ((rz + KB - 1) / KB);
}

extern "C" int dfb_knn_build_volume_radii(const float* node_pos, int n_nodes, int k, int rx, int ry, int rz, int x0, int x1, uint16_t* knn,
                                          float* brick_radius, dfb_stream_t stream) {
    DFB_REQUIRE(brick_radius, "null pointer");
    return knn_build(node_pos, 0, n_nodes, k, rx, ry, rz, x0, x1, knn, brick_radius, nullptr, stream);
}

extern "C" int dfb_knn_update_volume(const float* node_pos, int n_old, int n_nodes, int k, int rx, int ry, int rz, int x0, int x1, uint16_t* knn,
                                     float* brick_radius, uint8_t* dirty, dfb_stream_t stream) {
    DFB_REQUIRE(brick_radius && dirty, "null pointer");
    DFB_REQUIRE(n_old > 0, "n_old must be positive (use dfb_knn_build_volume_radii for the first build)");
    return knn_build(node_pos, n_old, n_nodes, k, rx, ry, rz, x0, x1, knn, brick_radius, dirty, stream);
}

extern "C" int dfb_knn_points(const float* pts, int64_t m, const float* node_pos, int n_nodes, int k, int32_t* idx,
                              dfb_stream_t stream) {
    DFB_REQUIRE(pts && node_pos && idx, "null pointer");
    DFB_REQUIRE(k >= 1 && k <= DFB_MAX_K, "k=%d out of range [1,%d]", k, DFB_MAX_K);
    DFB_REQUIRE(n_nodes >= k, "n_nodes=%d < k=%d", n_nodes, k);
    DFB_REQUIRE(m >= 0, "negative point count");
    if (m == 0) return DFB_OK;
    const int64_t blocks = (m + 255) / 256;
    cudaStream_t s = (cudaStream_t)stream;
    if (k <= 4) knn_points_kernel<4><<<(unsigned)blocks, 256, 0, s>>>(pts, m, node_pos, n_nodes, k, idx);
    else knn_points_kernel<8><<<(unsigned)blocks, 256, 0, s>>>(pts, m, node_pos, n_nodes, k, idx);
    DFB_LAUNCH_CHECK("knn_points_kernel");
    return DFB_OK;
}
```

### dynamicfusion_body_b200/csrc/tsdf.cu

```cuda
#include <stdlib.h>

#include "common.h"
#include "dfb_params.h"
#include "dfb_brick.h"

using namespace dfb;

namespace {

#ifndef DFB_STREAM_HINTS
#define DFB_STREAM_HINTS 1
#endif
__device__ __forceinline__ float4 ld_stream(const float* p) {
#if DFB_STREAM_HINTS
    return __ldcs(reinterpret_cast<const float4*>(p));
#else
    return *reinterpret_cast<const float4*>(p);
#endif
}
__device__ __forceinline__ void prefetch_l1(const void* p) { asm volatile("prefetch.global.L1 [%0];" ::"l"(p)); }
__device__ __forceinline__ void st_stream(float* p, float4 v) {
#if DFB_STREAM_HINTS
    __stcs(reinterpret_cast<float4*>(p), v);
#else
// ... 512 lines not shown
template <int KMAX, bool EXACTK, bool ONEVIEW, class Rec>
__device__ __forceinline__ void queue_process(const ProjParams& P, const uint8_t* cls, int nb, int nby, int nbz, float sc, const Rec rec,
                                              WarpQueue& Q, int count) {
    const int lane = threadIdx.x & 31;
    const bool act = lane < count;
    const int e = Q.n - count + lane;
    uint32_t i = 0;
    int c = CLS_SKIP, mv = 0, fv = 0;
    float v = 0.f, w = 0.f;
    if (act) {
        i = Q.vox[e];
        v = P.tsdf[i];
        w = P.weight[i];
        const uint32_t xy = Q.xy[e];
        const int xs = (int)(xy >> 16), y = (int)(xy & 0xffffu);
        const int z = (int)(i - ((uint32_t)xs * (uint32_t)P.ry + (uint32_t)y) * (uint32_t)P.rz);
        int views = 0xff, m0 = 0, f0 = 0;
        if (!ONEVIEW) {
            const int b = ((xs / BRICK_X) * nby + y / BRICK_Y) * nbz + z / BRICK_Z;
            f0 = cls[nb + b]; views = cls[2 * nb + b]; m0 = cls[3 * nb + b];
        }
        uint16_t ids[KMAX];
        load_ids<KMAX>(P.knn, i, EXACTK ? KMAX : P.k, ids);
        c = voxel_projective_classify_rec<KMAX, EXACTK, ONEVIEW>(P, xs + P.x0, y, z, ids, &mv, &fv, views, m0, f0, rec);
    }
    push_uncertain(act && c == CLS_UNCERTAIN, i, P.list, P.capacity, P.counters, P.overflow_bits);
    if (act) {
        if (c == CLS_UNCERTAIN) { mv = 0; fv = 0; }
        if (mv) {
            if (ONEVIEW) clamp_update(v, w, P.tdist_f, P.wmax_f, sc);
            else
                for (int vi = 0; vi < P.n_views; ++vi)
                    if (mv & (1 << vi)) clamp_update(v, w, P.tdist_f, P.wmax_f, sc);
            P.tsdf[i] = v;
            P.weight[i] = w;
        }
        if (P.mask_out) P.mask_out[i] = (uint8_t)mv;
        if (P.frustum_out) P.frustum_out[i] = (uint8_t)fv;
    }
    Q.n -= count;
    __syncwarp();
}

template <bool ONEVIEW>
__device__ __forceinline__ uint32_t mixed_layer_quads(const ProjParams& P, const float* rr, int xs, int y, int z0, uint32_t i0, float sc, int views, int m0,
                                                      int f0) {
    const int lane = threadIdx.x & 31;
    QuadView qv[ONEVIEW ? 1 : DFB_MAX_VIEWS];
    const int nv = ONEVIEW ? 1 : P.n_views;
    if (ONEVIEW) {
        const float4* q4 = reinterpret_cast<const float4*>(rr + 16);
        const float4 a = __ldg(q4), b = __ldg(q4 + 1), c = __ldg(q4 + 2), d = __ldg(q4 + 3);
        qv[0].M[0] = a.x; qv[0].M[1] = a.y; qv[0].M[2] = a.z; qv[0].M[3] = a.w;
        qv[0].M[4] = b.x; qv[0].M[5] = b.y; qv[0].M[6] = b.z; qv[0].M[7] = b.w;
        qv[0].M[8] = c.x; qv[0].M[9] = c.y; qv[0].M[10] = c.z; qv[0].M[11] = c.w;
        qv[0].d[0] = d.x; qv[0].d[1] = d.y; qv[0].d[2] = d.z;
    }
    for (int v = 0; v < (ONEVIEW ? 0 : nv); ++v) {
        if (!((views >> v) & 1)) continue;
        float val = 0.f;
        {
            const float* T = P.vf[v].T;
            if (lane < 12) {
                const int r = lane >> 2, c = lane & 3;
                val = T[4 * r] * rr[c] + T[4 * r + 1] * rr[4 + c] + T[4 * r + 2] * rr[8 + c] + (c == 3 ? T[4 * r + 3] : 0.f);
            } else if (lane < 15) {
                const int r = lane - 12;
                const float pad = 2e-3f + 2e-6f * P.coord_mag;
                val = fabsf(T[4 * r]) * (rr[12] + pad) + fabsf(T[4 * r + 1]) * (rr[13] + pad) + fabsf(T[4 * r + 2]) * (rr[14] + pad) +
                      8e-6f * P.coord_mag + 1e-3f;
            }
        }
#pragma unroll
        for (int t = 0; t < 12; ++t) qv[v].M[t] = __shfl_sync(0xffffffffu, val, t);
#pragma unroll
        for (int t = 0; t < 3; ++t) qv[v].d[t] = __shfl_sync(0xffffffffu, val, 12 + t);
    }
    int st[4], mq[4], fq[4];
    quad_pretest(P, qv, xs + P.x0, y, z0, 4, ONEVIEW ? 1 : views, m0, f0, st, mq, fq);
    uint32_t om = 0, bm = 0;
    bool any_upd = false;
#pragma unroll
    for (int q = 0; q < 4; ++q) {
        if (st[q] == QV_BAND) { mq[q] = 0; fq[q] = 0; bm |= 1u << q; }
        if (st[q] == QV_OPEN) om |= 1u << q;
        any_upd |= st[q] == QV_SKIP && mq[q] != 0;
    }
    if (any_upd) {
        const float4 v4 = ld_stream(P.tsdf + i0), w4 = ld_stream(P.weight + i0);
        float v[4] = {v4.x, v4.y, v4.z, v4.w}, w[4] = {w4.x, w4.y, w4.z, w4.w};
#pragma unroll
        for (int q = 0; q < 4; ++q) {
            if (st[q] != QV_SKIP || !mq[q]) continue;
            if (ONEVIEW) clamp_update(v[q], w[q], P.tdist_f, P.wmax_f, sc);
            else
                for (int vi = 0; vi < P.n_views; ++vi)
                    if (mq[q] & (1 << vi)) clamp_update(v[q], w[q], P.tdist_f, P.wmax_f, sc);
        }
        if (!om) {
            st_stream(P.tsdf + i0, make_float4(v[0], v[1], v[2], v[3]));
            st_stream(P.weight + i0, make_float4(w[0], w[1], w[2], w[3]));
        } else {
#pragma unroll
            for (int q = 0; q < 4; ++q)
                if (st[q] == QV_SKIP && mq[q]) { P.tsdf[i0 + q] = v[q]; P.weight[i0 + q] = w[q]; }
        }
    }
    if (P.mask_out || P.frustum_out) {
        if (!om) {
            if (P.mask_out) *reinterpret_cast<uchar4*>(P.mask_out + i0) = make_uchar4(mq[0], mq[1], mq[2], mq[3]);
            if (P.frustum_out) *reinterpret_cast<uchar4*>(P.frustum_out + i0) = make_uchar4(fq[0], fq[1], fq[2], fq[3]);
        } else {
#pragma unroll
            for (int q = 0; q < 4; ++q)
                if (st[q] != QV_OPEN) {
                    if (P.mask_out) P.mask_out[i0 + q] = (uint8_t)mq[q];
                    if (P.frustum_out) P.frustum_out[i0 + q] = (uint8_t)fq[q];
                }
        }
    }
    if (__any_sync(0xffffffffu, bm != 0)) {
        const int mine = __popc(bm);
        int incl = mine;
#pragma unroll
        for (int o = 1; o < 32; o <<= 1) {
            const int up = __shfl_up_sync(0xffffffffu, incl, o);
            if (lane >= o) incl += up;
        }
        const int total = __shfl_sync(0xffffffffu, incl, 31);
        uint32_t base = 0;
        if (lane == 0) base = atomicAdd(P.counters, (uint32_t)total);
        base = __shfl_sync(0xffffffffu, base, 0) + (uint32_t)(incl - mine);
#pragma unroll
        for (int q = 0; q < 4; ++q)
            if ((bm >> q) & 1u) defer_voxel(base++, i0 + q, P.list, P.capacity, P.overflow_bits);
    }
    return om;
}

__device__ __forceinline__ const float* brick_region_rec(const ProjParams& P, const float* region_rec, int bxs, int by, int bz) {
    if (!region_rec || P.rigid) return nullptr;
    const int nry = (P.ry + REGION_Y - 1) / REGION_Y, nrz = (P.rz + REGION_Z - 1) / REGION_Z;
    const uint32_t reg = ((uint32_t)(bxs * BRICK_X / REGION_X) * (uint32_t)nry + (uint32_t)(by * BRICK_Y / REGION_Y)) * (uint32_t)nrz + (uint32_t)(bz * BRICK_Z / REGION_Z);
    const float* rr = region_rec + (size_t)reg * REGION_REC_FLOATS;
    return rr[15] > 0.5f ? rr : nullptr;
}

template <int KMAX, bool EXACTK, bool ONEVIEW, class Rec>
__device__ __forceinline__ uint32_t mixed_layer(const ProjParams& P, const float* region_rec, int nb, int nby, int nbz, const uint8_t* cls, uint32_t entry,
                                                int t128, float sc, const Rec rec, uint32_t* i0_out, uint32_t* xy_out) {
    int bxs, by, bz;
    brick_unpack(entry, bxs, by, bz);
    int views = 0xff, m0 = 0, f0 = 0;
    if (!ONEVIEW) {
        const int b = (bxs * nby + by) * nbz + bz;
        f0 = cls[nb + b]; views = cls[2 * nb + b]; m0 = cls[3 * nb + b];
    }
    int dx, dy, dz;
    brick_lane(t128, dx, dy, dz);
    const bool full = (P.rz & 3) == 0 && (bxs + 1) * BRICK_X <= P.x1 - P.x0 && (by + 1) * BRICK_Y <= P.ry && (bz + 1) * BRICK_Z <= P.rz;
    if (!full) {
        mixed_brick_edge<KMAX, EXACTK, ONEVIEW>(P, bxs, by, bz, dx, dy, dz, sc, views, m0, f0, rec);
        return 0u;
    }
    const int xs = bxs * BRICK_X + dx, y = by * BRICK_Y + dy, z0 = bz * BRICK_Z + dz;
    const uint32_t i0 = (uint32_t)(((size_t)xs * P.ry + y) * P.rz + z0);
    *i0_out = i0;
    *xy_out = ((uint32_t)xs << 16) | (uint32_t)y;
    const float* rr = ONEVIEW ? brick_region_rec(P, region_rec, bxs, by, bz) : nullptr;
    if (!rr) return 0xfu;
    return mixed_layer_quads<ONEVIEW>(P, rr, xs, y, z0, i0, sc, views, m0, f0);
}

template <int KMAX, bool EXACTK, bool ONEVIEW, class Rec>
__device__ __forceinline__ void update_body(const ProjParams& P, const float* region_rec, int nbx, int nby, int nbz, const uint8_t* cls,
                                            const uint32_t* stream_list, uint32_t cnt_s, const uint32_t* mixed_list, uint32_t cnt_m, uint32_t first,
                                            uint32_t stride, uint32_t n_t, int t128, const Rec rec, WarpQueue& Q) {
    const int nb = nbx * nby * nbz;
    const uint32_t share = n_t ? (cnt_s + n_t - 1) / n_t : 0u;
    const int lane = threadIdx.x & 31;
    int dx, dy, dz;
    brick_lane(t128, dx, dy, dz);
    const float sc = (float)P.scale;
    const bool vec = (P.rz & 3) == 0;
    uint32_t n_dqb = 0;
    for (uint32_t t = first;; t += stride) {
        const bool last = !(t < n_t);
        uint32_t om = 0, i0 = 0, xy = 0;
        if (!last) {
            if (t < cnt_m) om = mixed_layer<KMAX, EXACTK, ONEVIEW>(P, region_rec, nb, nby, nbz, cls, mixed_list[t], t128, sc, rec, &i0, &xy);
            const uint32_t s1 = (t + 1) * share < cnt_s ? (t + 1) * share : cnt_s;
            for (uint32_t s = t * share; s < s1; ++s) stream_brick<ONEVIEW>(P, nb, nby, nbz, cls, stream_list[s], dx, dy, dz, sc, vec);
        }
        const bool any = __any_sync(0xffffffffu, om != 0);
        if (om) {
            prefetch_l1(P.knn + (size_t)i0 * P.k);
            prefetch_l1(P.tsdf + i0);
            prefetch_l1(P.weight + i0);
        }
#pragma unroll 1
        for (int half = 0; half < 2; ++half) {
            if (any) {
#pragma unroll
                for (int j = 0; j < 2; ++j) {
                    const int q = 2 * half + j;
                    const bool open = (om >> q) & 1u;
                    const unsigned bo = __ballot_sync(0xffffffffu, open);
                    if (open) {
                        const int pos = Q.n + __popc(bo & ((1u << lane) - 1u));
                        Q.vox[pos] = i0 + (uint32_t)q;
                        Q.xy[pos] = xy;
                    }
                    Q.n += __popc(bo);
                    n_dqb += __popc(bo);
                }
                __syncwarp();
            }
            const int thr = last ? 1 : 32;
            while (Q.n >= thr) queue_process<KMAX, EXACTK, ONEVIEW>(P, cls, nb, nby, nbz, sc, rec, Q, Q.n < 32 ? Q.n : 32);
        }
        if (last) break;
    }
    if (lane == 0 && n_dqb) atomicAdd(P.counters + 4, n_dqb);
}

__global__ void __launch_bounds__(128) brick_stream_kernel(const __grid_constant__ ProjParams P, int nbx, int nby, int nbz,
                                                           const uint8_t* cls, const uint32_t* list) {
    const uint32_t count = P.counters[2];
    int dx, dy, dz;
    brick_lane(threadIdx.x, dx, dy, dz);
    for (uint32_t t = blockIdx.x; t < count; t += gridDim.x)
        stream_brick(P, nbx * nby * nbz, nby, nbz, cls, list[t], dx, dy, dz, (float)P.scale, (P.rz & 3) == 0);
}

template <int KMAX, bool EXACTK, bool ONEVIEW>
__global__ void __launch_bounds__(128) brick_mixed_kernel(const __grid_constant__ ProjParams P, int nbx, int nby, int nbz,
                                                          const uint8_t* cls, const uint32_t* list, const float* region_rec) {
    __shared__ uint32_t s_queue[4][2 * WQ_CAP];
    WarpQueue Q = {s_queue[threadIdx.x >> 5], s_queue[threadIdx.x >> 5] + WQ_CAP, 0};
    const uint32_t count = P.counters[3];
    update_body<KMAX, EXACTK, ONEVIEW>(P, region_rec, nbx, nby, nbz, cls, nullptr, 0u, list, count, blockIdx.x, gridDim.x, count, threadIdx.x,
                                       RecGlobal{P.node_rec}, Q);
}

#ifndef DFB_UPDATE_MINB
#define DFB_UPDATE_MINB 8
#endif
#define DFB_UPDATE_BOUNDS __launch_bounds__(128, DFB_UPDATE_MINB)
template <int KMAX, bool EXACTK, bool ONEVIEW>
__global__ void DFB_UPDATE_BOUNDS brick_update_kernel(const __grid_constant__ ProjParams P, int nbx, int nby, int nbz,
                                                           const uint8_t* cls, const uint32_t* stream_list, const uint32_t* mixed_list,
                                                           const float* region_rec) {
    __shared__ uint32_t s_queue[4][2 * WQ_CAP];
    WarpQueue Q = {s_queue[threadIdx.x >> 5], s_queue[threadIdx.x >> 5] + WQ_CAP, 0};
    const uint32_t cnt_s = P.counters[2], cnt_m = P.counters[3];
    const uint32_t n_t = cnt_m > gridDim.x ? cnt_m : gridDim.x;
    update_body<KMAX, EXACTK, ONEVIEW>(P, region_rec, nbx, nby, nbz, cls, stream_list, cnt_s, mixed_list, cnt_m, blockIdx.x, gridDim.x, n_t, threadIdx.x,
                                       RecGlobal{P.node_rec}, Q);
}

constexpr int UPDATE_SMEM_THREADS = 1024, UPDATE_SMEM_GROUPS = UPDATE_SMEM_THREADS / 128;
constexpr size_t UPDATE_SMEM_MAX_BYTES = 226 * 1024;
template <int KMAX, bool EXACTK, bool ONEVIEW>
__global__ void __launch_bounds__(UPDATE_SMEM_THREADS, 1) brick_update_smem_kernel(const __grid_constant__ ProjParams P, int n_nodes, int nbx, int nby,
                                                                                    int nbz, const uint8_t* cls, const uint32_t* stream_list,
                                                                                    const uint32_t* mixed_list, const float* region_rec) {
    extern __shared__ __align__(128) unsigned char smem_raw[];
    float4* s_rec = reinterpret_cast<float4*>(smem_raw);
    uint32_t* wq = reinterpret_cast<uint32_t*>(smem_raw + (((size_t)n_nodes * DFB_NODE_REC_FLOATS * sizeof(float) + 127) & ~(size_t)127)) +
                   (size_t)(threadIdx.x >> 5) * 2 * WQ_CAP;
    WarpQueue Q = {wq, wq + WQ_CAP, 0};
    __shared__ __align__(8) unsigned long long bar;
    const uint32_t bytes = (uint32_t)n_nodes * (uint32_t)(DFB_NODE_REC_FLOATS * sizeof(float));
    const uint32_t bar_a = (uint32_t)__cvta_generic_to_shared(&bar);
    if (threadIdx.x == 0) {
        asm volatile("mbarrier.init.shared::cta.b64 [%0], 1;" ::"r"(bar_a));
        asm volatile("fence.mbarrier_init.release.cluster;" ::: "memory");
    }
    __syncthreads();
    if (threadIdx.x == 0) {
        asm volatile("mbarrier.arrive.expect_tx.shared::cta.b64 _, [%0], %1;" ::"r"(bar_a), "r"(bytes) : "memory");
        const char* src = reinterpret_cast<const char*>(P.node_rec);
        const uint32_t dst = (uint32_t)__cvta_generic_to_shared(s_rec);
        for (uint32_t off = 0; off < bytes; off += 32768u) {
            const uint32_t n = bytes - off < 32768u ? bytes - off : 32768u;
            asm volatile("cp.async.bulk.shared::cluster.global.mbarrier::complete_tx::bytes [%0], [%1], %2, [%3];" ::"r"(dst + off),
                         "l"(src + off), "r"(n), "r"(bar_a)
                         : "memory");
        }
    }
    const uint32_t cnt_s = P.counters[2], cnt_m = P.counters[3];
    const uint32_t n_groups = gridDim.x * UPDATE_SMEM_GROUPS;
    const uint32_t n_t = cnt_m > n_groups ? cnt_m : n_groups;
    const uint32_t rec_a = (uint32_t)__cvta_generic_to_shared(s_rec);
    {
        uint32_t done = 0;
        while (!done)
            asm volatile("{ .reg .pred p; mbarrier.try_wait.parity.shared::cta.b64 p, [%1], 0; selp.u32 %0, 1, 0, p; }" : "=r"(done) : "r"(bar_a) : "memory");
    }
    update_body<KMAX, EXACTK, ONEVIEW>(P, region_rec, nbx, nby, nbz, cls, stream_list, cnt_s, mixed_list, cnt_m,
                                       blockIdx.x * UPDATE_SMEM_GROUPS + (threadIdx.x >> 7), n_groups, n_t, threadIdx.x & 127, RecShared{rec_a}, Q);
}

template <int KMAX, int KT>
__device__ __forceinline__ void exact_voxel(const ProjParams& P, size_t i, size_t nvox, size_t plane, const uint16_t* ids, float v, float w) {
    int xs, y, z;
    if (nvox <= 0xffffffffull) {
        const uint32_t i32 = (uint32_t)i, plane32 = (uint32_t)plane, rz32 = (uint32_t)P.rz;
        const uint32_t xq = i32 / plane32, rem = i32 - xq * plane32, yq = rem / rz32;
        xs = (int)xq; y = (int)yq; z = (int)(rem - yq * rz32);
    } else {
        xs = (int)(i / plane);
        const size_t rem = i - (size_t)xs * plane;
        y = (int)(rem / P.rz);
        z = (int)(rem - (size_t)y * P.rz);
    }
    int m, f;
    voxel_projective_exact<KT>(P, xs + P.x0, y, z, ids, &v, &w, &m, &f);
    if (m) {
        P.tsdf[i] = v;
        P.weight[i] = w;
    }
    if (P.mask_out) P.mask_out[i] = (uint8_t)m;
    if (P.frustum_out) P.frustum_out[i] = (uint8_t)f;
}

#ifndef DFB_EXACT_MINB
#define DFB_EXACT_MINB 8
#endif
template <int KMAX, int KT>
__global__ void __launch_bounds__(128, DFB_EXACT_MINB) proj_exact_kernel(const __grid_constant__ ProjParams P, int all_mode) {
    const size_t nvox = (size_t)(P.x1 - P.x0) * P.ry * P.rz;
    const uint32_t count = P.counters[0];
    const bool overflow = !all_mode && count > P.capacity;
    const bool sweep_bits = overflow && P.overflow_bits != nullptr;
    const bool use_list = !all_mode && (!overflow || sweep_bits);
    const size_t n = use_list ? (size_t)(overflow ? P.capacity : count) : nvox;
    const size_t plane = (size_t)P.ry * P.rz;
    const int kk = KT > 0 ? KT : P.k;
    uint32_t done = 0;
    if (use_list && KT > 0 && !P.rigid && nvox <= 0xffffffffull) {
        const uint32_t stride = gridDim.x * blockDim.x, cnt = (uint32_t)n;
        uint32_t t = blockIdx.x * blockDim.x + threadIdx.x;
        if (t < cnt) {
            uint32_t i0 = P.list[t];
            uint32_t i1 = t + stride < cnt && t + stride >= t ? P.list[t + stride] : i0;
            uint16_t ids0[KMAX];
            load_ids<KMAX>(P.knn, i0, KMAX, ids0);
            float v0 = P.tsdf[i0], w0 = P.weight[i0];
            for (;;) {
                const uint32_t tn = t + stride, tnn = tn + stride;
                const bool has1 = tn < cnt && tn > t;
                const uint32_t i2 = (has1 && tnn < cnt && tnn > tn) ? P.list[tnn] : i1;
                uint16_t ids1[KMAX];
                load_ids<KMAX>(P.knn, i1, KMAX, ids1);
                const float v1 = P.tsdf[i1], w1 = P.weight[i1];
                exact_voxel<KMAX, KT>(P, i0, nvox, plane, ids0, v0, w0);
                ++done;
                if (!has1) break;
                t = tn; i0 = i1; i1 = i2; v0 = v1; w0 = w1;
#pragma unroll
                for (int j = 0; j < KMAX; ++j) ids0[j] = ids1[j];
            }
        }
    } else {
        for (size_t t = (size_t)blockIdx.x * blockDim.x + threadIdx.x; t < n; t += (size_t)gridDim.x * blockDim.x) {
            const size_t i = use_list ? (size_t)P.list[t] : t;
            uint16_t ids[KMAX];
            if (!P.rigid) load_ids<KMAX>(P.knn, i, kk, ids);
            if (!use_list && !all_mode) {
                const size_t xq = i / plane, rem = i - xq * plane;
                int m0, f0;
                if (voxel_projective_classify<KMAX>(P, (int)xq + P.x0, (int)(rem / P.rz), (int)(rem % P.rz), ids, &m0, &f0) != CLS_UNCERTAIN) continue;
            }
            exact_voxel<KMAX, KT>(P, i, nvox, plane, ids, P.tsdf[i], P.weight[i]);
            ++done;
        }
    }
    if (sweep_bits) {
        const size_t nwords = (nvox + 31) / 32;
        const size_t warp0 = ((size_t)blockIdx.x * blockDim.x + threadIdx.x) >> 5, nwarps = ((size_t)gridDim.x * blockDim.x) >> 5;
        const int lane = threadIdx.x & 31;
        for (size_t wd = warp0; wd < nwords; wd += nwarps) {
            const uint32_t bits = P.overflow_bits[wd];
            if (!bits) continue;
            __syncwarp();
            if (lane == 0) P.overflow_bits[wd] = 0u;
            if ((bits >> lane) & 1u) {
                const size_t i = wd * 32 + (size_t)lane;
                uint16_t ids[KMAX];
                if (!P.rigid) load_ids<KMAX>(P.knn, i, kk, ids);
                exact_voxel<KMAX, KT>(P, i, nvox, plane, ids, P.tsdf[i], P.weight[i]);
                ++done;
            }
        }
    }
    for (int o = 16; o > 0; o >>= 1) done += __shfl_xor_sync(0xffffffffu, done, o);
    if ((threadIdx.x & 31) == 0 && done) atomicAdd(P.counters + 1, done);
}

#ifndef DFB_VOL_FAST_MINB
#define DFB_VOL_FAST_MINB 6
#endif
template <int KMAX>
__global__ void __launch_bounds__(256, DFB_VOL_FAST_MINB) vol_fast_kernel(const __grid_constant__ VolParams P) {
    const int z = blockIdx.x * blockDim.x + threadIdx.x;
    const int y = blockIdx.y;
    const int xs = blockIdx.z;
    const bool in = z < P.rz;
    const size_t i = ((size_t)xs * P.ry + y) * P.rz + (in ? z : 0);
    int cls = CLS_SKIP;
    float wi = 0.f;
    if (in) {
        uint16_t ids[KMAX];
        if (P.k > 0) load_ids<KMAX>(P.knn, i, P.k, ids);
        cls = voxel_volume_classify<KMAX>(P, xs + P.x0, y, z, ids, &wi);
    }
    push_uncertain(in && cls == CLS_UNCERTAIN, (uint32_t)i, P.list, P.capacity, P.counters, P.overflow_bits);
    if (!in || cls == CLS_UNCERTAIN) return;
    if (cls == CLS_CLAMP) {
        float v = P.tsdf[i], w = P.weight[i];
        if (P.k > 0) {
            const float wt = (w == 0.f) ? wi : w;
            v = (v * wt + fmul(P.tdist_f, wi)) / (wi + wt);
            w = fminf(wi + wt, P.wmax_f);
        } else {
            v = (v * w + P.tdist_f) / (1.0f + w);
            w = fminf(1.0f + w, P.wmax_f);
        }
        P.tsdf[i] = v;
        P.weight[i] = w;
    }
    if (P.mask_out) P.mask_out[i] = (cls == CLS_CLAMP) ? 1 : 0;
}

template <int KMAX, int KT>
__device__ __forceinline__ void vol_exact_voxel(const VolParams& P, size_t i, size_t plane) {
    int xs, y, z;
    if (plane * (size_t)(P.x1 - P.x0) <= 0xffffffffull) {
        const uint32_t i32 = (uint32_t)i, plane32 = (uint32_t)plane, rz32 = (uint32_t)P.rz;
        const uint32_t xq = i32 / plane32, rem = i32 - xq * plane32, yq = rem / rz32;
        xs = (int)xq; y = (int)yq; z = (int)(rem - yq * rz32);
    } else {
        xs = (int)(i / plane);
        const size_t rem = i - (size_t)xs * plane;
        y = (int)(rem / P.rz);
        z = (int)(rem - (size_t)y * P.rz);
    }
    uint16_t ids[KMAX];
    if (P.k > 0) load_ids<KMAX>(P.knn, i, P.k, ids);
    float v = P.tsdf[i], w = P.weight[i];
    const bool upd = voxel_volume_exact<KT>(P, xs + P.x0, y, z, ids, &v, &w);
    if (upd) {
        P.tsdf[i] = v;
        P.weight[i] = w;
    }
    if (P.mask_out) P.mask_out[i] = upd ? 1 : 0;
}

#ifndef DFB_VOL_EXACT_MINB
#define DFB_VOL_EXACT_MINB 8
#endif
template <int KMAX, int KT>
__global__ void __launch_bounds__(128, DFB_VOL_EXACT_MINB) vol_exact_kernel(const __grid_constant__ VolParams P, int all_mode) {
    const size_t nvox = (size_t)(P.x1 - P.x0) * P.ry * P.rz;
    const uint32_t count = P.counters[0];
    const bool overflow = !all_mode && count > P.capacity;
    const bool sweep_bits = overflow && P.overflow_bits != nullptr;
    const bool use_list = !all_mode && (!overflow || sweep_bits);
    const size_t n = use_list ? (size_t)(overflow ? P.capacity : count) : nvox;
    const size_t plane = (size_t)P.ry * P.rz;
    uint32_t done = 0;
    for (size_t t = (size_t)blockIdx.x * blockDim.x + threadIdx.x; t < n; t += (size_t)gridDim.x * blockDim.x) {
        const size_t i = use_list ? (size_t)P.list[t] : t;
        if (!use_list && !all_mode) {
            const int xs = (int)(i / plane);
            const size_t rem = i - (size_t)xs * plane;
            uint16_t ids[KMAX];
            if (P.k > 0) load_ids<KMAX>(P.knn, i, P.k, ids);
            float wi;
            if (voxel_volume_classify<KMAX>(P, xs + P.x0, (int)(rem / P.rz), (int)(rem % P.rz), ids, &wi) != CLS_UNCERTAIN) continue;
        }
        vol_exact_voxel<KMAX, KT>(P, i, plane);
        ++done;
    }
    if (sweep_bits) {
        const size_t nwords = (nvox + 31) / 32;
        const size_t warp0 = ((size_t)blockIdx.x * blockDim.x + threadIdx.x) >> 5, nwarps = ((size_t)gridDim.x * blockDim.x) >> 5;
        const int lane = threadIdx.x & 31;
        for (size_t wd = warp0; wd < nwords; wd += nwarps) {
            const uint32_t bits = P.overflow_bits[wd];
            if (!bits) continue;
            __syncwarp();
            if (lane == 0) P.overflow_bits[wd] = 0u;
            if ((bits >> lane) & 1u) {
                vol_exact_voxel<KMAX, KT>(P, wd * 32 + (size_t)lane, plane);
                ++done;
            }
        }
    }
    for (int o = 16; o > 0; o >>= 1) done += __shfl_xor_sync(0xffffffffu, done, o);
    if ((threadIdx.x & 31) == 0 && done) atomicAdd(P.counters + 1, done);
}

__global__ void warp_points_kernel(const float* pts, const float* normals, int64_t m, const int32_t* idx, int k,
                                   const float* node_pos, const float* node_dq, const float* node_w,
                                   const __grid_constant__ dfb_warpfield wf, double* out_p, double* out_n) {
    for (int64_t t = (int64_t)blockIdx.x * blockDim.x + threadIdx.x; t < m; t += (int64_t)gridDim.x * blockDim.x) {
        int ids[DFB_MAX_K];
        for (int j = 0; j < k; ++j) ids[j] = idx[t * k + j];
        double op[3], on[3];
        warp_ref(pts + 3 * t, normals ? normals + 3 * t : nullptr, ids, k, node_pos, node_dq, node_w, wf.lw, wf.has_lw != 0,
                 wf.lw_is_f32 != 0, op, on, nullptr);
        for (int c = 0; c < 3; ++c) out_p[3 * t + c] = op[c];
        if (normals && out_n)
            for (int c = 0; c < 3; ++c) out_n[3 * t + c] = on[c];
    }
}

__global__ void dq_blend_points_kernel(const float* pts, int64_t m, const int32_t* idx, int k, const float* node_pos,
                                       const float* node_dq, const float* node_w, double* out) {
    for (int64_t t = (int64_t)blockIdx.x * blockDim.x + threadIdx.x; t < m; t += (int64_t)gridDim.x * blockDim.x) {
        int ids[DFB_MAX_K];
        for (int j = 0; j < k; ++j) ids[j] = idx[t * k + j];
        double se3[8];
        dq_blend_ref(pts + 3 * t, ids, k, node_pos, node_dq, node_w, se3, nullptr);
        for (int c = 0; c < 8; ++c) out[8 * t + c] = se3[c];
    }
}

__global__ void nodes_pack_kernel(const float* pos, const float* dq, const float* w, int n, float* rec) {
    const int i = blockIdx.x * blockDim.x + threadIdx.x;
    if (i >= n) return;
    float* r = rec + (size_t)i * DFB_NODE_REC_FLOATS;
    r[0] = pos[3 * i]; r[1] = pos[3 * i + 1]; r[2] = pos[3 * i + 2];
    const double ww = (double)w[i];
    r[3] = (float)(-1.4426950408889634 / (4.0 * ww * ww));
    for (int c = 0; c < 8; ++c) r[4 + c] = dq[8 * i + c];
}

dim3 fast_grid(const dfb_volume* vol, int& threads) {
    threads = vol->rz >= 256 ? 256 : ((vol->rz + 31) / 32) * 32;
    return dim3((vol->rz + threads - 1) / threads, vol->ry, vol->x1 - vol->x0);
}

int exact_blocks(size_t nvox) {
    static int per_sm = 0;
    if (per_sm == 0) { const char* e = getenv("DFB_EXACT_CTAS_PER_SM"); per_sm = e ? atoi(e) : 32; if (per_sm < 1) per_sm = 32; }
    const size_t want = (nvox + 127) / 128, cap = (size_t)148 * per_sm;
    return (int)(want < cap ? (want ? want : 1) : cap);
}

struct BrickArgs {
    int n_nodes;
    const uint16_t* nodes;
    const uint8_t* count;
    const uint32_t* pairs;
    const uint16_t* rnodes;
    const uint8_t* rcount;
    const uint32_t* rpairs;
    float* rrec;
    uint8_t* cls;
    uint32_t* lists;
};

int run_projective(ProjParams& P, int mode, cudaStream_t s, const dfb_volume* vol, const BrickArgs& B) {
    const bool bricks = B.cls != nullptr && B.lists != nullptr && (P.rigid || (B.nodes != nullptr && B.count != nullptr));
    const bool do_classify = mode == DFB_MODE_HYBRID || mode == DFB_MODE_FAST_ONLY || mode == DFB_MODE_BRICK_CLASSIFY;
    const bool do_stream = mode == DFB_MODE_HYBRID || mode == DFB_MODE_FAST_ONLY || mode == DFB_MODE_BRICK_STREAM || mode == DFB_MODE_BRICK_UPDATE;
    const bool do_mixed = mode == DFB_MODE_HYBRID || mode == DFB_MODE_FAST_ONLY || mode == DFB_MODE_BRICK_MIXED || mode == DFB_MODE_BRICK_UPDATE;
    if (mode >= DFB_MODE_BRICK_CLASSIFY) DFB_REQUIRE(bricks, "brick modes need the brick workspace / candidate sets");
    if (mode != DFB_MODE_HYBRID && mode != DFB_MODE_EXACT) P.overflow_bits = nullptr;
    if (mode == DFB_MODE_HYBRID || mode == DFB_MODE_EXACT || mode == DFB_MODE_FAST_ONLY || mode == DFB_MODE_BRICK_CLASSIFY)
        DFB_CUDA(cudaMemsetAsync(P.counters, 0, 8 * sizeof(uint32_t), s));
    const size_t nvox = (size_t)(P.x1 - P.x0) * P.ry * P.rz;
    if (mode != DFB_MODE_EXACT && mode != DFB_MODE_LIST_ONLY) {
        if (bricks) {
            const int nbx = (P.x1 - P.x0 + BRICK_X - 1) / BRICK_X, nby = (P.ry + BRICK_Y - 1) / BRICK_Y, nbz = (P.rz + BRICK_Z - 1) / BRICK_Z;
            const int nb = nbx * nby * nbz;
            DFB_REQUIRE(nbx <= BRICK_PACK_MAX_XY && nby <= BRICK_PACK_MAX_XY && nbz <= BRICK_PACK_MAX_Z,
                        "volume too large for the brick work lists (4096 x 4096 x 131072 voxels per slab)");
            const float* rrec = nullptr;
            const bool have_regions = !P.rigid && B.rnodes && B.rcount && B.rpairs && B.rrec;
            uint32_t* stream_list = B.lists;
            uint32_t* mixed_list = B.lists + nb;
            const bool classified = false;
            if (have_regions) {
                rrec = B.rrec;
                if (do_classify) {
                    const int nrx = (P.x1 - P.x0 + REGION_X - 1) / REGION_X, nry = (P.ry + REGION_Y - 1) / REGION_Y, nrz = (P.rz + REGION_Z - 1) / REGION_Z;
                    region_bounds_kernel<<<dim3(nrz, nry, nrx), DFB_REGION_THREADS, 0, s>>>(P, B.rnodes, B.rcount, B.rpairs, nry, nrz, B.rrec);
                    DFB_LAUNCH_CHECK("region_bounds_kernel");
                }
            }
            static int upd_per_sm = 0;
            if (upd_per_sm == 0) { const char* e = getenv("DFB_UPDATE_CTAS_PER_SM"); upd_per_sm = e ? atoi(e) : 16; if (upd_per_sm < 1) upd_per_sm = 16; }
            const int grid = nb < 148 * upd_per_sm ? nb : 148 * upd_per_sm;
            if (do_classify && !classified) {
                static int G = 0;
                if (G == 0) { const char* e = getenv("DFB_CLASSIFY_G"); G = e ? atoi(e) : 8; }
                const int per_cta = 128 / G;
                const int nb_pad = ((nbx + 3) / 4) * ((nby + 3) / 4) * nbz * 16;
                const int cgrid = (nb_pad + per_cta - 1) / per_cta < 148 * 32 ? (nb_pad + per_cta - 1) / per_cta : 148 * 32;
                if (G == 1) brick_classify_kernel<1><<<cgrid, 128, 0, s>>>(P, B.nodes, B.count, B.pairs, rrec, nbx, nby, nbz, B.cls, stream_list, mixed_list);
                else if (G == 2) brick_classify_kernel<2><<<cgrid, 128, 0, s>>>(P, B.nodes, B.count, B.pairs, rrec, nbx, nby, nbz, B.cls, stream_list, mixed_list);
                else if (G == 4) brick_classify_kernel<4><<<cgrid, 128, 0, s>>>(P, B.nodes, B.count, B.pairs, rrec, nbx, nby, nbz, B.cls, stream_list, mixed_list);
                else if (G == 16) brick_classify_kernel<16><<<cgrid, 128, 0, s>>>(P, B.nodes, B.count, B.pairs, rrec, nbx, nby, nbz, B.cls, stream_list, mixed_list);
                else if (G == 32) brick_classify_kernel<32><<<cgrid, 128, 0, s>>>(P, B.nodes, B.count, B.pairs, rrec, nbx, nby, nbz, B.cls, stream_list, mixed_list);
                else brick_classify_kernel<8><<<cgrid, 128, 0, s>>>(P, B.nodes, B.count, B.pairs, rrec, nbx, nby, nbz, B.cls, stream_list, mixed_list);
                DFB_LAUNCH_CHECK("brick_classify_kernel");
            }
            if (do_stream && do_mixed) {
#define DFB_BRICK_DISPATCH(KERNEL, ...)                                                                                  \
    do {                                                                                                                 \
        const bool one = P.n_views == 1;                                                                                 \
        if (P.k == 4 && !P.rigid) { if (one) KERNEL<4, true, true><<<grid, 128, 0, s>>>(__VA_ARGS__); else KERNEL<4, true, false><<<grid, 128, 0, s>>>(__VA_ARGS__); } \
        else if (P.k == 8 && !P.rigid) { if (one) KERNEL<8, true, true><<<grid, 128, 0, s>>>(__VA_ARGS__); else KERNEL<8, true, false><<<grid, 128, 0, s>>>(__VA_ARGS__); } \
        else if (P.k <= 4) { if (one) KERNEL<4, false, true><<<grid, 128, 0, s>>>(__VA_ARGS__); else KERNEL<4, false, false><<<grid, 128, 0, s>>>(__VA_ARGS__); } \
        else { if (one) KERNEL<8, false, true><<<grid, 128, 0, s>>>(__VA_ARGS__); else KERNEL<8, false, false><<<grid, 128, 0, s>>>(__VA_ARGS__); } \
    } while (0)
                static int smem_env = -2;
                if (smem_env == -2) { const char* e = getenv("DFB_UPDATE_SMEM"); smem_env = e ? atoi(e) : -1; }
                const int use_smem = smem_env >= 0 ? smem_env : (P.n_views > 1 || P.k > 4);
                static int use_quads = -1;
                if (use_quads < 0) { const char* e = getenv("DFB_QUADS"); use_quads = e ? atoi(e) : 1; }
                const float* qrec = use_quads ? rrec : nullptr;
                const size_t rec_bytes = (((size_t)B.n_nodes * DFB_NODE_REC_FLOATS * sizeof(float) + 127) & ~(size_t)127) + (UPDATE_SMEM_THREADS / 32) * WQ_BYTES;
                if (use_smem && !P.rigid && B.n_nodes > 0 && rec_bytes <= UPDATE_SMEM_MAX_BYTES) {
                    static int n_sm = 0;
                    if (n_sm == 0) {
                        int dev = 0;
                        DFB_CUDA(cudaGetDevice(&dev));
                        DFB_CUDA(cudaDeviceGetAttribute(&n_sm, cudaDevAttrMultiProcessorCount, dev));
                    }
                    const int sgrid = nb < n_sm * UPDATE_SMEM_GROUPS ? (nb + UPDATE_SMEM_GROUPS - 1) / UPDATE_SMEM_GROUPS : n_sm;
#define DFB_SMEM_LAUNCH(K_, E_, O_)                                                                                              \
    do {                                                                                                                         \
        DFB_CUDA(cudaFuncSetAttribute(brick_update_smem_kernel<K_, E_, O_>, cudaFuncAttributeMaxDynamicSharedMemorySize,        \
                                      (int)UPDATE_SMEM_MAX_BYTES));                                                              \
        brick_update_smem_kernel<K_, E_, O_><<<sgrid, UPDATE_SMEM_THREADS, rec_bytes, s>>>(P, B.n_nodes, nbx, nby, nbz, B.cls,   \
                                                                                          stream_list, mixed_list, qrec);      \
    } while (0)
                    const bool one = P.n_views == 1;
                    if (P.k == 4) { if (one) DFB_SMEM_LAUNCH(4, true, true); else DFB_SMEM_LAUNCH(4, true, false); }
                    else if (P.k == 8) { if (one) DFB_SMEM_LAUNCH(8, true, true); else DFB_SMEM_LAUNCH(8, true, false); }
                    else if (P.k < 4) { if (one) DFB_SMEM_LAUNCH(4, false, true); else DFB_SMEM_LAUNCH(4, false, false); }
                    else { if (one) DFB_SMEM_LAUNCH(8, false, true); else DFB_SMEM_LAUNCH(8, false, false); }
                    DFB_LAUNCH_CHECK("brick_update_smem_kernel");
                } else {
                    DFB_BRICK_DISPATCH(brick_update_kernel, P, nbx, nby, nbz, B.cls, stream_list, mixed_list, qrec);
                    DFB_LAUNCH_CHECK("brick_update_kernel");
                }
            } else if (do_stream) {
                brick_stream_kernel<<<grid, 128, 0, s>>>(P, nbx, nby, nbz, B.cls, stream_list);
                DFB_LAUNCH_CHECK("brick_stream_kernel");
            } else if (do_mixed) {
                static int use_quads_m = -1;
                if (use_quads_m < 0) { const char* e = getenv("DFB_QUADS"); use_quads_m = e ? atoi(e) : 1; }
                DFB_BRICK_DISPATCH(brick_mixed_kernel, P, nbx, nby, nbz, B.cls, mixed_list, use_quads_m ? rrec : nullptr);
                DFB_LAUNCH_CHECK("brick_mixed_kernel");
            }
        } else {
            int threads;
            const dim3 grid = fast_grid(vol, threads);
            if (P.k <= 4) proj_fast_kernel<4><<<grid, threads, 0, s>>>(P);
            else proj_fast_kernel<8><<<grid, threads, 0, s>>>(P);
            DFB_LAUNCH_CHECK("proj_fast_kernel");
        }
        if (mode != DFB_MODE_HYBRID) return DFB_OK;
    }
    const int all = mode == DFB_MODE_EXACT ? 1 : 0;
    if (P.k == 4 && !P.rigid) proj_exact_kernel<4, 4><<<exact_blocks(nvox), 128, 0, s>>>(P, all);
    else if (P.k == 8 && !P.rigid) proj_exact_kernel<8, 8><<<exact_blocks(nvox), 128, 0, s>>>(P, all);
    else if (P.k <= 4) proj_exact_kernel<4, 0><<<exact_blocks(nvox), 128, 0, s>>>(P, all);
    else proj_exact_kernel<8, 0><<<exact_blocks(nvox), 128, 0, s>>>(P, all);
    DFB_LAUNCH_CHECK("proj_exact_kernel");
    return DFB_OK;
}

}

extern "C" int dfb_nodes_pack(const float* node_pos, const float* node_dq, const float* node_w, int n_nodes,
                              float* node_rec, dfb_stream_t stream) {
    DFB_REQUIRE(node_pos && node_dq && node_w && node_rec, "null pointer");
    DFB_REQUIRE(n_nodes > 0, "n_nodes must be positive");
    nodes_pack_kernel<<<(n_nodes + 127) / 128, 128, 0, (cudaStream_t)stream>>>(node_pos, node_dq, node_w, n_nodes, node_rec);
    DFB_LAUNCH_CHECK("nodes_pack_kernel");
    return DFB_OK;
}

extern "C" int dfb_tsdf_update_projective(const dfb_volume* vol, const dfb_warpfield* wf, const dfb_views* views,
                                          double tdist, double wmax, int mode, const dfb_workspace* ws,
                                          uint8_t* mask_out, uint8_t* frustum_out, dfb_stream_t stream) {
    ProjParams P;
    if (int r = build_projective(P, vol, wf, views, tdist, wmax, mode, ws, mask_out, frustum_out)) return r;
    const BrickArgs B = {wf->n_nodes, wf->brick_nodes, wf->brick_count, wf->brick_pairs, wf->region_nodes, wf->region_count, wf->region_pairs, wf->region_rec,
                         ws->brick_cls, ws->brick_lists};
    return run_projective(P, mode, (cudaStream_t)stream, vol, B);
}

extern "C" int dfb_fuse_depth_rigid(const dfb_volume* vol, int tsdf_res, const float* depth, int rows, int cols,
                                    const double lw34[12], const double K[9], const double Kinv[9], double scale,
                                    const double center[3], double tdist, double wmax, int mode,
                                    const dfb_workspace* ws, uint8_t* mask_out, uint8_t* frustum_out,
                                    dfb_stream_t stream) {
    ProjParams P;
    if (int r = build_rigid(P, vol, tsdf_res, depth, rows, cols, lw34, K, Kinv, scale, center, tdist, wmax, mode, ws,
                            mask_out, frustum_out))
        return r;
    const BrickArgs B = {0, nullptr, nullptr, nullptr, nullptr, nullptr, nullptr, nullptr, ws->brick_cls, ws->brick_lists};
    return run_projective(P, mode, (cudaStream_t)stream, vol, B);
}

extern "C" int dfb_tsdf_update_volume(const dfb_volume* vol, const dfb_warpfield* wf, const float* curr, int cx,
                                      int cy, int cz, double tdist, double wmax, int mode, const dfb_workspace* ws,
                                      uint8_t* mask_out, dfb_stream_t stream) {
    VolParams P;
    if (int r = build_volume(P, vol, wf, curr, cx, cy, cz, tdist, wmax, mode, ws, mask_out)) return r;
    cudaStream_t s = (cudaStream_t)stream;
    if (mode != DFB_MODE_HYBRID && mode != DFB_MODE_EXACT) P.overflow_bits = nullptr;
    if (mode != DFB_MODE_LIST_ONLY) DFB_CUDA(cudaMemsetAsync(P.counters, 0, 8 * sizeof(uint32_t), s));
    const size_t nvox = (size_t)(P.x1 - P.x0) * P.ry * P.rz;
    if (mode == DFB_MODE_HYBRID || mode == DFB_MODE_FAST_ONLY) {
        int threads;
        const dim3 grid = fast_grid(vol, threads);
        if (P.k <= 4) vol_fast_kernel<4><<<grid, threads, 0, s>>>(P);
        else vol_fast_kernel<8><<<grid, threads, 0, s>>>(P);
        DFB_LAUNCH_CHECK("vol_fast_kernel");
        if (mode == DFB_MODE_FAST_ONLY) return DFB_OK;
    }
    const int all = mode == DFB_MODE_EXACT ? 1 : 0;
    if (P.k == 4) vol_exact_kernel<4, 4><<<exact_blocks(nvox), 128, 0, s>>>(P, all);
    else if (P.k == 8) vol_exact_kernel<8, 8><<<exact_blocks(nvox), 128, 0, s>>>(P, all);
    else if (P.k <= 4) vol_exact_kernel<4, 0><<<exact_blocks(nvox), 128, 0, s>>>(P, all);
    else vol_exact_kernel<8, 0><<<exact_blocks(nvox), 128, 0, s>>>(P, all);
    DFB_LAUNCH_CHECK("vol_exact_kernel");
    return DFB_OK;
}

extern "C" int dfb_warp_points(const float* pts, const float* normals, int64_t m, const int32_t* idx,
                               const dfb_warpfield* wf, double* out_pts, double* out_normals, dfb_stream_t stream) {
    if (int r = validate_warpfield(wf, false)) return r;
    DFB_REQUIRE(pts && out_pts && m >= 0, "null pointer / negative count");
    DFB_REQUIRE(wf->k == 0 || idx, "neighbour indices are null");
    if (m == 0) return DFB_OK;
    const int blocks = (int)((m + 127) / 128 < 148 * 8 ? (m + 127) / 128 : 148 * 8);
    warp_points_kernel<<<blocks, 128, 0, (cudaStream_t)stream>>>(pts, normals, m, idx, wf->k, wf->node_pos, wf->node_dq,
                                                                 wf->node_w, *wf, out_pts, out_normals);
    DFB_LAUNCH_CHECK("warp_points_kernel");
    return DFB_OK;
}

extern "C" int dfb_dq_blend_points(const float* pts, int64_t m, const int32_t* idx, const dfb_warpfield* wf, double* out_dq,
                                   dfb_stream_t stream) {
    if (int r = validate_warpfield(wf, false)) return r;
    DFB_REQUIRE(pts && idx && out_dq && m >= 0 && wf->k > 0, "bad arguments");
    if (m == 0) return DFB_OK;
    const int blocks = (int)((m + 127) / 128 < 148 * 8 ? (m + 127) / 128 : 148 * 8);
    dq_blend_points_kernel<<<blocks, 128, 0, (cudaStream_t)stream>>>(pts, m, idx, wf->k, wf->node_pos, wf->node_dq, wf->node_w, out_dq);
    DFB_LAUNCH_CHECK("dq_blend_points_kernel");
    return DFB_OK;
}

extern "C" int64_t dfb_brick_count(int sx, int ry, int rz) {
    return (int64_t)((sx + BRICK_X - 1) / BRICK_X) * ((ry + BRICK_Y - 1) / BRICK_Y) * ((rz + BRICK_Z - 1) / BRICK_Z);
}

extern "C" int dfb_brick_nodes_build(const uint16_t* knn, int k, int rx, int ry, int rz, int x0, int x1, uint16_t* brick_nodes,
                                     uint8_t* brick_count, uint32_t* brick_pairs, dfb_stream_t stream) {
    return dfb_brick_nodes_update(knn, k, rx, ry, rz, x0, x1, nullptr, brick_nodes, brick_count, brick_pairs, stream);
}

extern "C" int dfb_brick_nodes_update(const uint16_t* knn, int k, int rx, int ry, int rz, int x0, int x1, const uint8_t* dirty8, uint16_t* brick_nodes,
                                      uint8_t* brick_count, uint32_t* brick_pairs, dfb_stream_t stream) {
    DFB_REQUIRE(knn && brick_nodes && brick_count && brick_pairs, "null pointer");
    DFB_REQUIRE(k >= 1 && k <= DFB_MAX_K && rx > 0 && ry > 0 && rz > 0 && x0 >= 0 && x1 > x0 && x1 <= rx, "bad arguments");
    const int sx = x1 - x0;
    const int nby = (ry + BRICK_Y - 1) / BRICK_Y, nbz = (rz + BRICK_Z - 1) / BRICK_Z;
    const int64_t nb = dfb_brick_count(sx, ry, rz);
    DFB_REQUIRE(nb < ((int64_t)1 << 31), "too many bricks");
    brick_nodes_kernel<<<(unsigned)nb, 128, 0, (cudaStream_t)stream>>>(knn, k, sx, ry, rz, nby, nbz, brick_nodes, brick_count, brick_pairs, dirty8);
    DFB_LAUNCH_CHECK("brick_nodes_kernel");
    return DFB_OK;
}

extern "C" int64_t dfb_region_count(int sx, int ry, int rz) {
    return (int64_t)((sx + REGION_X - 1) / REGION_X) * ((ry + REGION_Y - 1) / REGION_Y) * ((rz + REGION_Z - 1) / REGION_Z);
}

extern "C" int dfb_region_build(const uint16_t* knn, int k, int rx, int ry, int rz, int x0, int x1, uint16_t* region_nodes,
                                uint8_t* region_count, uint32_t* region_pairs, dfb_stream_t stream) {
    return dfb_region_update(knn, k, rx, ry, rz, x0, x1, nullptr, region_nodes, region_count, region_pairs, stream);
}

extern "C" int dfb_region_update(const uint16_t* knn, int k, int rx, int ry, int rz, int x0, int x1, const uint8_t* dirty8, uint16_t* region_nodes,
                                 uint8_t* region_count, uint32_t* region_pairs, dfb_stream_t stream) {
    DFB_REQUIRE(knn && region_nodes && region_count && region_pairs, "null pointer");
    DFB_REQUIRE(k >= 1 && k <= DFB_MAX_K && rx > 0 && ry > 0 && rz > 0 && x0 >= 0 && x1 > x0 && x1 <= rx, "bad arguments");
    const int sx = x1 - x0;
    const int nry = (ry + REGION_Y - 1) / REGION_Y, nrz = (rz + REGION_Z - 1) / REGION_Z;
    const int64_t nr = dfb_region_count(sx, ry, rz);
    DFB_REQUIRE(nr < ((int64_t)1 << 31), "too many regions");
    region_build_kernel<<<(unsigned)nr, 256, 0, (cudaStream_t)stream>>>(knn, k, sx, ry, rz, nry, nrz, region_nodes, region_count, region_pairs, dirty8);
    DFB_LAUNCH_CHECK("region_build_kernel");
    return DFB_OK;
// ... 2 lines not shown
```

### dynamicfusion_body_b200/engine.py

```python
import ctypes as C
import os

import numpy as np
import torch

from . import _capi


USE_REGIONS = True


def _stream():
    return C.c_void_p(torch.cuda.current_stream().cuda_stream)


def _ptr(t):
    return C.c_void_p(t.data_ptr()) if t is not None else None


def _require_cuda(device):
    if not torch.cuda.is_available():
        raise RuntimeError("dynamicfusion_body_b200 needs a CUDA device (B200); there is no CPU path")
    return torch.device(device if device is not None else "cuda:%d" % torch.cuda.current_device())


def _to_dev(a, dtype, device):
    if isinstance(a, torch.Tensor):
        return a.to(device=device, dtype=dtype).contiguous()
    a = np.ascontiguousarray(a)
    if not a.flags.writeable:
        a = a.copy()
    return torch.from_numpy(a).to(device=device, dtype=dtype).contiguous()


class Workspace:

    def __init__(self, n_voxels, device, fraction=0.25, n_bricks=0):
        self.capacity = int(max(1024, n_voxels * fraction))
        self.list = torch.empty(self.capacity, dtype=torch.int32, device=device)
        self.counters = torch.zeros(8, dtype=torch.int32, device=device)
        self.n_bricks = int(n_bricks)
        self.brick_cls = torch.zeros(4 * self.n_bricks, dtype=torch.uint8, device=device) if n_bricks else None
        self.brick_lists = torch.zeros(2 * self.n_bricks, dtype=torch.int32, device=device) if n_bricks else None
        self.overflow_bits = torch.zeros((int(n_voxels) + 31) // 32, dtype=torch.int32, device=device)

    def struct(self, use_bricks=True):
        s = _capi.Workspace()
        s.list = self.list.data_ptr()
        s.capacity = self.capacity
        s.counters = self.counters.data_ptr()
        s.overflow_bits = self.overflow_bits.data_ptr()
        if use_bricks and self.brick_cls is not None:
            s.brick_cls = self.brick_cls.data_ptr()
            s.brick_lists = self.brick_lists.data_ptr()
        return s

    def _decode(self, c):
        c = c.astype(np.int64) & 0xffffffff
        return {"deferred": int(c[0]), "exact_processed": int(c[1]), "bricks_streamed": int(c[2]), "bricks_mixed": int(c[3]),
                "bricks": self.n_bricks, "dqb_voxels": int(c[4])}

    def stats(self):
        return self._decode(self.counters.cpu().numpy())

    def stats_async(self):
        if not hasattr(self, "_pinned"):
            self._pinned = [torch.empty(8, dtype=torch.int32).pin_memory() for _ in range(4)]
            self._pin_i = 0
        buf = self._pinned[self._pin_i % len(self._pinned)]
        self._pin_i += 1
        buf.copy_(self.counters, non_blocking=True)
        ev = torch.cuda.Event()
        ev.record()
        ws = self

        class _Pending:
            def result(self):
                ev.synchronize()
                return ws._decode(buf.numpy().copy())
        return _Pending()


class DeviceVolume:

    def __init__(self, res, x0=0, x1=None, device=None, tsdf=None, weight=None, fill=None):
        self.device = _require_cuda(device)
        self.res = tuple(int(r) for r in res)
        self.x0 = int(x0)
        self.x1 = int(self.res[0] if x1 is None else x1)
        shape = (self.x1 - self.x0, self.res[1], self.res[2])
        if tsdf is not None:
            self.tsdf = _to_dev(tsdf, torch.float32, self.device).reshape(shape)
        else:
            self.tsdf = torch.full(shape, float(fill if fill is not None else 0.0), dtype=torch.float32, device=self.device)
        if weight is not None:
            self.weight = _to_dev(weight, torch.float32, self.device).reshape(shape)
        else:
            self.weight = torch.zeros(shape, dtype=torch.float32, device=self.device)
        nb = int(_capi.lib().dfb_brick_count(self.x1 - self.x0, self.res[1], self.res[2]))
        self.workspace = Workspace(self.n_voxels, self.device, n_bricks=nb)

    @property
    def n_voxels(self):
        return (self.x1 - self.x0) * self.res[1] * self.res[2]

    def struct(self):
        s = _capi.Volume()
        s.tsdf = self.tsdf.data_ptr()
        s.weight = self.weight.data_ptr()
        s.rx, s.ry, s.rz = self.res
        s.x0, s.x1 = self.x0, self.x1
        return s


class DeviceWarpField:

    def __init__(self, k, device=None):
        self.device = _require_cuda(device)
        self.k = int(k)
        self.n_nodes = 0
        self.node_pos = self.node_dq = self.node_w = self.node_rec = None
        self._knn = {}
        self._knn_radii = {}
        self._bricks = {}

    def set_nodes(self, node_pos, node_dq, node_w):
        n = len(node_pos)
        self.node_pos = _to_dev(node_pos, torch.float32, self.device).reshape(n, 3)
        w = np.broadcast_to(np.asarray(node_w, dtype=np.float32), (n,)) if not isinstance(node_w, torch.Tensor) else node_w
        self.node_w = _to_dev(w, torch.float32, self.device).reshape(n)
        self.n_nodes = n
        self._knn = {}
        self._knn_radii = {}
        self._bricks = {}
        self.node_dq = None
        self.set_dq(node_dq)

    def set_dq(self, node_dq):
        if (self.node_dq is not None and tuple(self.node_dq.shape) == (self.n_nodes, 8)
                and (isinstance(node_dq, torch.Tensor) or isinstance(node_dq, np.ndarray))):
            src = node_dq if isinstance(node_dq, torch.Tensor) else torch.from_numpy(np.ascontiguousarray(node_dq, dtype=np.float32))
            if src.data_ptr() != self.node_dq.data_ptr():
                self.node_dq.copy_(src.reshape(self.n_nodes, 8), non_blocking=True)
        else:
            self.node_dq = _to_dev(node_dq, torch.float32, self.device).reshape(self.n_nodes, 8)
        self.repack()

    def repack(self):
        if self.node_rec is None or self.node_rec.shape[0] != self.n_nodes:
            self.node_rec = torch.empty((self.n_nodes, _capi.DFB_NODE_REC_FLOATS), dtype=torch.float32, device=self.device)
        _capi.check(_capi.lib().dfb_nodes_pack(_ptr(self.node_pos), _ptr(self.node_dq), _ptr(self.node_w), self.n_nodes,
                                               _ptr(self.node_rec), _stream()))

    def knn_table(self, res, x0, x1):
        key = (tuple(res), x0, x1)
        t = self._knn.get(key)
        if t is None:
            n = (x1 - x0) * res[1] * res[2]
            t = torch.empty((n, self.k), dtype=torch.int16, device=self.device)
            L = _capi.lib()
            if os.environ.get("DFB_KNN_BRUTE"):
                _capi.check(L.dfb_knn_build_volume(_ptr(self.node_pos), self.n_nodes, self.k, res[0], res[1], res[2], x0, x1, _ptr(t), _stream()))
            else:
                radii = torch.empty(int(L.dfb_knn_brick_count(x1 - x0, res[1], res[2])), dtype=torch.float32, device=self.device)
                _capi.check(L.dfb_knn_build_volume_radii(_ptr(self.node_pos), self.n_nodes, self.k, res[0], res[1], res[2], x0, x1, _ptr(t),
                                                         _ptr(radii), _stream()))
                self._knn_radii[key] = radii
            self._knn[key] = t
        return t

    def append_nodes(self, node_pos, node_dq, node_w):
        m = len(node_pos)
        if m == 0:
            return
        n_old = self.n_nodes
        new_pos = _to_dev(node_pos, torch.float32, self.device).reshape(m, 3)
        new_dq = _to_dev(node_dq, torch.float32, self.device).reshape(m, 8)
        w = np.broadcast_to(np.asarray(node_w, dtype=np.float32), (m,)) if not isinstance(node_w, torch.Tensor) else node_w
        new_w = _to_dev(w, torch.float32, self.device).reshape(m)
        self.node_pos = torch.cat([self.node_pos, new_pos]).contiguous()
        self.node_w = torch.cat([self.node_w, new_w]).contiguous()
        dq = torch.cat([self.node_dq, new_dq]).contiguous()
        self.n_nodes = n_old + m
        self.node_dq = None
        self.set_dq(dq)
        L = _capi.lib()
        for key, t in list(self._knn.items()):
            res, x0, x1 = key
            radii = self._knn_radii.get(key)
            if radii is None or n_old < self.k:
                del self._knn[key]
                self._bricks.pop(key, None)
                continue
            dirty = torch.empty(radii.numel(), dtype=torch.uint8, device=self.device)
            _capi.check(L.dfb_knn_update_volume(_ptr(self.node_pos), n_old, self.n_nodes, self.k, res[0], res[1], res[2], x0, x1, _ptr(t),
                                                _ptr(radii), _ptr(dirty), _stream()))
            self.last_dirty = dirty
            b = self._bricks.get(key)
            if b is not None:
                nodes, count, pairs, rnodes, rcount, rpairs, rrec = b
                _capi.check(L.dfb_brick_nodes_update(_ptr(t), self.k, res[0], res[1], res[2], x0, x1, _ptr(dirty), _ptr(nodes), _ptr(count),
                                                     _ptr(pairs), _stream()))
                _capi.check(L.dfb_region_update(_ptr(t), self.k, res[0], res[1], res[2], x0, x1, _ptr(dirty), _ptr(rnodes), _ptr(rcount),
                                                _ptr(rpairs), _stream()))

    def brick_nodes(self, res, x0, x1):
        key = (tuple(res), x0, x1)
        t = self._bricks.get(key)
        if t is None:
            knn = self.knn_table(res, x0, x1)
            nb = int(_capi.lib().dfb_brick_count(x1 - x0, res[1], res[2]))
            nodes = torch.zeros((nb, 24), dtype=torch.int16, device=self.device)
            count = torch.zeros(nb, dtype=torch.uint8, device=self.device)
            pairs = torch.zeros((nb, 10), dtype=torch.int32, device=self.device)
            _capi.check(_capi.lib().dfb_brick_nodes_build(_ptr(knn), self.k, res[0], res[1], res[2], x0, x1, _ptr(nodes), _ptr(count),
                                                          _ptr(pairs), _stream()))
            nr = int(_capi.lib().dfb_region_count(x1 - x0, res[1], res[2]))
            rnodes = torch.zeros((nr, 64), dtype=torch.int16, device=self.device)
            rcount = torch.zeros(nr, dtype=torch.uint8, device=self.device)
            rpairs = torch.zeros((nr, 65), dtype=torch.int32, device=self.device)
            rrec = torch.zeros((nr, 32), dtype=torch.float32, device=self.device)
            _capi.check(_capi.lib().dfb_region_build(_ptr(knn), self.k, res[0], res[1], res[2], x0, x1, _ptr(rnodes), _ptr(rcount),
                                                     _ptr(rpairs), _stream()))
            t = (nodes, count, pairs, rnodes, rcount, rpairs, rrec)
            self._bricks[key] = t
        return t

    def knn_points(self, pts, k=None):
        k = self.k if k is None else k
        p = _to_dev(pts, torch.float32, self.device).reshape(-1, 3)
        out = torch.empty((p.shape[0], k), dtype=torch.int32, device=self.device)
        _capi.check(_capi.lib().dfb_knn_points(_ptr(p), p.shape[0], _ptr(self.node_pos), self.n_nodes, k, _ptr(out), _stream()))
        return out

    def struct(self, lw=None, knn=None, k=None, bricks=None):
        s = _capi.WarpField()
        if bricks is not None:
            s.brick_nodes = bricks[0].data_ptr()
            s.brick_count = bricks[1].data_ptr()
            s.brick_pairs = bricks[2].data_ptr()
            if USE_REGIONS:
                s.region_nodes = bricks[3].data_ptr()
                s.region_count = bricks[4].data_ptr()
                s.region_pairs = bricks[5].data_ptr()
                s.region_rec = bricks[6].data_ptr()
        k = self.k if k is None else k
        if k > 0:
            s.node_rec = self.node_rec.data_ptr()
            s.node_pos = self.node_pos.data_ptr()
            s.node_dq = self.node_dq.data_ptr()
            s.node_w = self.node_w.data_ptr()
        s.n_nodes = self.n_nodes
        s.k = k
        s.knn = knn.data_ptr() if knn is not None else None
        fill_lw(s, lw)
        return s


def fill_lw(s, lw):
    s.has_lw = 0 if lw is None else 1
    s.lw_is_f32 = 0
    if lw is not None:
        if isinstance(lw, torch.Tensor):
            lw = lw.detach().cpu().numpy()
        lw = np.asarray(lw)
        s.lw_is_f32 = 1 if lw.dtype == np.float32 else 0
        for i in range(8):
            s.lw[i] = float(lw[i])


def make_views(depths, K, Kinv=None, extrinsics=None):
    if depths.dim() == 2:
        depths = depths[None]
    assert depths.is_cuda and depths.dtype == torch.float32 and depths.is_contiguous()
    K = np.asarray(K, dtype=np.float64)
    Kinv = np.linalg.inv(K) if Kinv is None else np.asarray(Kinv, dtype=np.float64)
    v = _capi.Views()
    v.n_views = depths.shape[0]
    if v.n_views > _capi.DFB_MAX_VIEWS:
        raise ValueError("at most %d views per pass" % _capi.DFB_MAX_VIEWS)
    for i in range(v.n_views):
        v.depth[i] = depths[i].data_ptr()
    v.rows, v.cols = int(depths.shape[1]), int(depths.shape[2])
    for i in range(9):
        v.K[i] = float(K.ravel()[i])
        v.Kinv[i] = float(Kinv.ravel()[i])
    v.has_extrinsics = 0 if extrinsics is None else 1
    if extrinsics is not None:
        E = np.asarray(extrinsics, dtype=np.float64).reshape(v.n_views, 12)
        for j in range(v.n_views):
            for i in range(12):
                v.E[j][i] = float(E[j, i])
    return v


def _mask_bufs(vol, want):
    if not want:
        return None, None
    return (torch.zeros(vol.n_voxels, dtype=torch.uint8, device=vol.device),
            torch.zeros(vol.n_voxels, dtype=torch.uint8, device=vol.device))


def update_projective(vol, wf, lw, depths, K, Kinv=None, extrinsics=None, tdist=1.0, wmax=100.0,
                      mode=_capi.MODE_HYBRID, want_masks=False, views=None, use_bricks=True):
    views = views if views is not None else make_views(depths, K, Kinv, extrinsics)
    knn = wf.knn_table(vol.res, vol.x0, vol.x1)
    bricks = wf.brick_nodes(vol.res, vol.x0, vol.x1) if use_bricks else None
    ws = vol.workspace.struct(use_bricks)
    mask, frus = _mask_bufs(vol, want_masks)
    v = vol.struct()
    s = wf.struct(lw, knn, bricks=bricks)
    _capi.check(_capi.lib().dfb_tsdf_update_projective(C.byref(v), C.byref(s), C.byref(views), float(tdist), float(wmax),
                                                       int(mode), C.byref(ws), _ptr(mask), _ptr(frus), _stream()))
    return (mask, frus) if want_masks else None


def update_volume(vol, wf, lw, curr, tdist, wmax=100.0, mode=_capi.MODE_HYBRID, want_masks=False, rigid=False):
    assert curr.is_cuda and curr.dtype == torch.float32 and curr.is_contiguous() and curr.dim() == 3
    k = 0 if rigid else wf.k
    knn = None if rigid else wf.knn_table(vol.res, vol.x0, vol.x1)
    ws = vol.workspace.struct(False)
    mask = torch.zeros(vol.n_voxels, dtype=torch.uint8, device=vol.device) if want_masks else None
    v = vol.struct()
    s = wf.struct(lw, knn, k=k) if wf is not None else _rigid_struct(lw)
    _capi.check(_capi.lib().dfb_tsdf_update_volume(C.byref(v), C.byref(s), _ptr(curr), curr.shape[0], curr.shape[1],
                                                   curr.shape[2], float(tdist), float(wmax), int(mode), C.byref(ws),
                                                   _ptr(mask), _stream()))
    return mask


def _rigid_struct(lw):
    s = _capi.WarpField()
    s.k = 0
    fill_lw(s, lw)
    return s


def fuse_depth_rigid(vol, tsdf_res, depth, lw34, K, Kinv=None, scale=1.0, center=None, tdist=1.0, wmax=100.0,
                     mode=_capi.MODE_HYBRID, want_masks=False, use_bricks=True):
    assert depth.is_cuda and depth.dtype == torch.float32 and depth.is_contiguous() and depth.dim() == 2
    K = np.ascontiguousarray(K, dtype=np.float64)
    Kinv = np.ascontiguousarray(np.linalg.inv(K) if Kinv is None else Kinv, dtype=np.float64)
    lw34 = np.ascontiguousarray(lw34, dtype=np.float64).reshape(12)
    center = np.ascontiguousarray(np.zeros(3) if center is None else center, dtype=np.float64)
    ws = vol.workspace.struct(use_bricks)
    mask, frus = _mask_bufs(vol, want_masks)
    v = vol.struct()
    f64 = _capi.c_f64p
    _capi.check(_capi.lib().dfb_fuse_depth_rigid(C.byref(v), int(tsdf_res), _ptr(depth), depth.shape[0], depth.shape[1],
                                                 lw34.ctypes.data_as(f64), K.ctypes.data_as(f64), Kinv.ctypes.data_as(f64),
                                                 float(scale), center.ctypes.data_as(f64), float(tdist), float(wmax), int(mode),
                                                 C.byref(ws), _ptr(mask), _ptr(frus), _stream()))
    return (mask, frus) if want_masks else None


def warp_points(wf, lw, pts, normals=None, idx=None, k=None):
    dev = wf.device
    p = _to_dev(pts, torch.float32, dev).reshape(-1, 3)
    n = None if normals is None else _to_dev(normals, torch.float32, dev).reshape(-1, 3)
    k = wf.k if k is None else k
    if k > 0:
        idx = wf.knn_points(p, k) if idx is None else _to_dev(idx, torch.int32, dev).reshape(-1, k)
    out = torch.empty((p.shape[0], 3), dtype=torch.float64, device=dev)
    outn = torch.empty((p.shape[0], 3), dtype=torch.float64, device=dev) if n is not None else None
    s = wf.struct(lw, None, k=k)
    _capi.check(_capi.lib().dfb_warp_points(_ptr(p), _ptr(n), p.shape[0], _ptr(idx), C.byref(s), _ptr(out), _ptr(outn), _stream()))
    return (out, outn) if n is not None else out


class PointGrid:

    MAX_CELLS = 1 << 24

    def __init__(self, pts, cell=None, device=None):
        dev = _require_cuda(device)
        self.device = dev
        self.pts = _to_dev(pts, torch.float32, dev).reshape(-1, 3)
        n = self.pts.shape[0]
        if n:
            lo = self.pts.amin(0).double().cpu().numpy()
            hi = self.pts.amax(0).double().cpu().numpy()
        else:
            lo = hi = np.zeros(3)
        ext = np.maximum(hi - lo, 1e-6)
        if cell is None:
            cell = float(ext.max()) / float(min(256, max(4, int(round(np.sqrt(max(n, 1)) / 2)))))
            cell = max(cell, float(np.cbrt(ext.prod() / (8.0 * max(n, 1)))))
        cell = float(cell)
        while True:
            dims = np.floor(ext / cell).astype(np.int64) + 1
            if int(dims.prod()) <= self.MAX_CELLS:
                break
            cell *= 1.26
        self.cell, self.origin, self.dims = cell, lo, [int(d) for d in dims]
        cells = int(dims.prod())
        self.cell_start = torch.empty(cells + 1, dtype=torch.int32, device=dev)
        self.order = torch.empty(max(n, 1), dtype=torch.int32, device=dev)
        scratch = torch.empty(int(_capi.lib().dfb_point_grid_scratch_ints(cells)), dtype=torch.int32, device=dev)
        if n == 0:
            self.pts = torch.zeros((1, 3), dtype=torch.float32, device=dev)
        self.n = n
        _capi.check(_capi.lib().dfb_point_grid_build(C.byref(self.struct()), _ptr(self.cell_start), _ptr(self.order), _ptr(scratch), _stream()))

    def struct(self):
        s = _capi.PointGrid()
        s.pts = self.pts.data_ptr()
        s.n = self.n
        for i in range(3):
            s.origin[i] = float(self.origin[i])
            s.dims[i] = self.dims[i]
        s.cell = self.cell
        s.cell_start = self.cell_start.data_ptr()
        s.order = self.order.data_ptr()
        return s

    def knn(self, queries, k, want_d2=False):
        q = _to_dev(queries, torch.float64, self.device).reshape(-1, 3)
        idx = torch.empty((q.shape[0], k), dtype=torch.int32, device=self.device)
        d2 = torch.empty((q.shape[0], k), dtype=torch.float64, device=self.device) if want_d2 else None
        _capi.check(_capi.lib().dfb_point_grid_knn(C.byref(self.struct()), _ptr(q), q.shape[0], k, _ptr(idx), _ptr(d2), _stream()))
        return (idx, d2) if want_d2 else idx


def corr_select(warped_pts, warped_normals, live_verts, nn):
    dev = nn.device
    wv = _to_dev(warped_pts, torch.float64, dev).reshape(-1, 3)
    wn = _to_dev(warped_normals, torch.float64, dev).reshape(-1, 3)
    lv = _to_dev(live_verts, torch.float32, dev).reshape(-1, 3)
    best = torch.empty(wv.shape[0], dtype=torch.int32, device=dev)
    cost = torch.empty(wv.shape[0], dtype=torch.float64, device=dev)
    _capi.check(_capi.lib().dfb_corr_select(_ptr(wv), _ptr(wn), wv.shape[0], _ptr(lv), _ptr(nn), nn.shape[1], _ptr(best), _ptr(cost), _stream()))
    return best, cost


def corr_projective(warped_pts, warped_normals, views, max_distance, min_normal_dot):
    dev = warped_pts.device if isinstance(warped_pts, torch.Tensor) and warped_pts.is_cuda else _require_cuda(None)
    wv = _to_dev(warped_pts, torch.float64, dev).reshape(-1, 3)
    wn = _to_dev(warped_normals, torch.float64, dev).reshape(-1, 3)
    m = wv.shape[0]
    view = torch.empty(m, dtype=torch.int32, device=dev)
    cost = torch.empty(m, dtype=torch.float64, device=dev)
    corr = torch.empty((m, 3), dtype=torch.float64, device=dev)
    _capi.check(_capi.lib().dfb_corr_projective(_ptr(wv), _ptr(wn), m, C.byref(views), float(max_distance), float(min_normal_dot),
                                                _ptr(view), _ptr(cost), _ptr(corr), _stream()))
    return view, cost, corr


def graph_unsupported(wf, verts, vert_knn):
    dev = wf.device
    v = _to_dev(verts, torch.float32, dev).reshape(-1, 3)
    kn = _to_dev(vert_knn, torch.int32, dev).reshape(v.shape[0], -1)
    out = torch.empty(v.shape[0], dtype=torch.uint8, device=dev)
    _capi.check(_capi.lib().dfb_graph_unsupported(_ptr(v), v.shape[0], _ptr(kn), kn.shape[1], _ptr(wf.node_pos), _ptr(wf.node_w), _ptr(out), _stream()))
    return out.bool()


def uniform_sample(pts, radius, device=None, rounds_per_call=16):
    dev = _require_cuda(device)
    p = _to_dev(pts, torch.float32, dev).reshape(-1, 3)
    n = p.shape[0]
    if n == 0:
        return np.zeros((0, 3), np.float32), np.zeros(0, np.int64)
    grid = PointGrid(p, cell=float(radius) * 1.001, device=dev)
    state = torch.zeros(n, dtype=torch.uint8, device=dev)
    undecided = torch.ones(1, dtype=torch.int32, device=dev)
    s = grid.struct()
    while True:
        _capi.check(_capi.lib().dfb_graph_sample_rounds(C.byref(s), float(radius), rounds_per_call, _ptr(state), _ptr(undecided), _stream()))
        if int(undecided.item()) == 0:
            break
    idx = torch.nonzero(state == 1).reshape(-1)
    return p[idx].cpu().numpy(), idx.cpu().numpy().astype(np.int64)


def marching_cubes(vol, step_size=1, level=None, x_origin=0, plane_offsets=False, keep_on_device=False):
    if not isinstance(vol, torch.Tensor):
        vol = _to_dev(np.asarray(vol), torch.float32, _require_cuda(None))
    if vol.dim() != 3:
        raise ValueError("marching_cubes needs a 3-D volume")
    step = int(step_size)
    if step < 1:
        raise ValueError("step_size must be >= 1")
    if not vol.is_cuda:
        vol = vol.to(_require_cuda(None))
    vol = vol.to(dtype=torch.float32).contiguous()
    rx, ry, rz = (int(n) for n in vol.shape)
    if min(rx, ry, rz) < 2:
        raise ValueError("marching_cubes needs at least 2 samples per axis")
    L = _capi.lib()
    dev = vol.device
    with torch.cuda.device(dev):
        lv = torch.empty(3, dtype=torch.float32, device=dev)
        if level is None:
            scratch = torch.empty(int(L.dfb_mc_level_scratch_floats()), dtype=torch.float32, device=dev)
            _capi.check(L.dfb_mc_level(_ptr(vol), vol.numel(), _ptr(scratch), _ptr(lv), _stream()))
        else:
            lv.fill_(float(np.float32(level)))
        rows = int(L.dfb_mc_rows(rx, ry, step))
        chunks = torch.empty((int(L.dfb_mc_chunks(rx, ry, rz, step)), 4), dtype=torch.int32, device=dev)
        offs = torch.empty((2, rows + 1), dtype=torch.int32, device=dev)
        _capi.check(L.dfb_mc_count(_ptr(vol), rx, ry, rz, step, int(x_origin), _ptr(lv), _ptr(chunks), _ptr(offs[0]), _ptr(offs[1]), _stream()))
        nv, nt = (int(x) for x in offs[:, rows].tolist())
        verts = torch.empty((nv, 3), dtype=torch.float32, device=dev)
        normals = torch.empty((nv, 3), dtype=torch.float32, device=dev)
        values = torch.empty(nv, dtype=torch.float32, device=dev)
        faces = torch.empty((nt, 3), dtype=torch.int32, device=dev)
        if nv or nt:
            _capi.check(L.dfb_mc_emit(_ptr(vol), rx, ry, rz, step, int(x_origin), _ptr(lv), _ptr(chunks), _ptr(offs[0]), _ptr(offs[1]),
                                      _ptr(verts), _ptr(normals), _ptr(values), _ptr(faces), _stream()))
        if keep_on_device:
            out = (verts, faces, normals, values)
        else:
            out = (verts.cpu().numpy(), faces.cpu().numpy(), normals.cpu().numpy(), values.cpu().numpy())
        if plane_offsets:
            ny = (ry - 1) // step + 1
            po = offs[:, ::ny].cpu().numpy().astype(np.int64)
            out += (po[0], po[1])
        return out


class Comm:

    def __init__(self, unique_id, world, rank, device=None):
        dev = _require_cuda(device)
        self.device = dev
        self.world, self.rank = int(world), int(rank)
        self._h = C.c_void_p()
        buf = (C.c_char * _capi.DFB_COMM_ID_BYTES).from_buffer_copy(bytes(unique_id))
        _capi.check(_capi.lib().dfb_comm_init(C.byref(self._h), buf, self.world, self.rank, dev.index if dev.index is not None else torch.cuda.current_device()))

    @staticmethod
    def unique_id():
        buf = (C.c_char * _capi.DFB_COMM_ID_BYTES)()
        _capi.check(_capi.lib().dfb_comm_unique_id(buf))
        return bytes(buf)

    @classmethod
    def from_torch(cls, device=None, group=None):
        import torch.distributed as dist
        world, rank = dist.get_world_size(group), dist.get_rank(group)
        box = [cls.unique_id() if rank == 0 else None]
        dist.broadcast_object_list(box, src=dist.get_global_rank(group, 0) if group is not None else 0, group=group)
        return cls(box[0], world, rank, device)

    @property
    def handle(self):
        return self._h

    def broadcast(self, t, root=0):
        assert t.is_cuda and t.is_contiguous()
        _capi.check(_capi.lib().dfb_comm_broadcast(self._h, _ptr(t), t.numel() * t.element_size(), int(root), _stream()))
        return t

    def broadcast_frame(self, depths=None, node_dq=None, lw=None, root=0):
        for t, dt in ((depths, torch.float32), (node_dq, torch.float32), (lw, torch.float64)):
            assert t is None or (t.is_cuda and t.is_contiguous() and t.dtype == dt)
        _capi.check(_capi.lib().dfb_comm_broadcast_frame(self._h, _ptr(depths), 0 if depths is None else depths.numel(), _ptr(node_dq),
                                                         0 if node_dq is None else node_dq.shape[0], _ptr(lw), int(root), _stream()))

    def allreduce_f64(self, t, op="sum"):
        assert t.is_cuda and t.is_contiguous() and t.dtype == torch.float64
        _capi.check(_capi.lib().dfb_comm_allreduce_f64(self._h, _ptr(t), t.numel(), 0 if op == "sum" else 1, _stream()))
        return t

    def sendrecv(self, send=None, send_peer=-1, recv=None, recv_peer=-1):
        _capi.check(_capi.lib().dfb_comm_sendrecv(self._h, _ptr(send), 0 if send is None else send.numel() * send.element_size(), int(send_peer),
                                                  _ptr(recv), 0 if recv is None else recv.numel() * recv.element_size(), int(recv_peer), _stream()))

    def close(self):
        if self._h:
            _capi.lib().dfb_comm_destroy(self._h)
            self._h = C.c_void_p()


class FrameStep:

    def __init__(self, vol, wf, lw, views, tdist, wmax=100.0):
        self._h = C.c_void_p()
        _capi.check(_capi.lib().dfb_frame_step_create(C.byref(self._h)))
        self.vol, self.wf, self.views = vol, wf, views
        knn = wf.knn_table(vol.res, vol.x0, vol.x1)
        bricks = wf.brick_nodes(vol.res, vol.x0, vol.x1)
        self._keep = (knn, bricks)
        self._v = vol.struct()
        self._w = wf.struct(lw, knn, bricks=bricks)
        self._ws = vol.workspace.struct(True)
        self.tdist, self.wmax = float(tdist), float(wmax)

    def set_lw(self, lw):
        fill_lw(self._w, lw)

    def set_views(self, views):
        self.views = views

    def io(self, comm=None, comm_prefetch=None, root=0, dq_src=None, prefetch_dst=None, prefetch_src=None, counters_host=None):
        io = _capi.FrameIO()
        io.comm = comm.handle if comm is not None else None
        io.comm_prefetch = comm_prefetch.handle if comm_prefetch is not None else None
        io.root = int(root)
        io.dq_src = dq_src.data_ptr() if dq_src is not None else None
        if prefetch_dst is not None:
            io.prefetch_dst = prefetch_dst.data_ptr()
            io.prefetch_bytes = prefetch_dst.numel() * prefetch_dst.element_size()
            io.prefetch_src = prefetch_src.data_ptr() if prefetch_src is not None else None
        io.counters_host = counters_host.data_ptr() if counters_host is not None else None
        io._keep = (comm, comm_prefetch, dq_src, prefetch_dst, prefetch_src, counters_host)
        return io

    def run(self, io=None):
        _capi.check(_capi.lib().dfb_frame_step_run(self._h, C.byref(self._v), C.byref(self._w), C.byref(self.views), self.tdist, self.wmax,
                                                   C.byref(self._ws), C.byref(io) if io is not None else None, _stream()))

    def stats(self):
        out = (C.c_int64 * 5)()
        _capi.check(_capi.lib().dfb_frame_step_stats(self._h, out))
        return {"captures": out[0], "updates": out[1], "replays": out[2], "direct": out[3], "graph_nodes": out[4]}

    def __del__(self):
        try:
            if self._h:
                _capi.lib().dfb_frame_step_destroy(self._h)
        except Exception:
            pass


def slab_cost_profile(vol, unit_planes=16):
    sx, ry, rz = vol.x1 - vol.x0, vol.res[1], vol.res[2]
    nbx, nby, nbz = (sx + 3) // 4, (ry + 3) // 4, (rz + 31) // 32
    nb = nbx * nby * nbz
    cls = vol.workspace.brick_cls[:nb].view(nbx, nby * nbz)
    mixed = (cls == 0xFF).sum(1).double()
    clamp = ((cls != 0xFF) & (cls != 0)).sum(1).double()
    layer = (0.6 * nby * nbz + 1.6 * clamp + 10.7 * mixed).cpu().numpy()
    per_unit = unit_planes // 4
    n_units = (nbx + per_unit - 1) // per_unit
    pad = np.zeros(n_units * per_unit)
    pad[:nbx] = layer
    return pad.reshape(n_units, per_unit).sum(1)
```

### include/dfb.h

```cpp
#ifndef DFB_H_
#define DFB_H_

#include <stdint.h>

#ifdef __cplusplus
extern "C" {
#endif

#define DFB_MAX_K 8
#define DFB_MAX_VIEWS 8
#define DFB_NODE_REC_FLOATS 12

#define DFB_OK 0
#define DFB_ERR_INVALID (-1)
#define DFB_ERR_CUDA (-2)

#define DFB_MODE_HYBRID 0
#define DFB_MODE_EXACT 1
#define DFB_MODE_FAST_ONLY 2
#define DFB_MODE_LIST_ONLY 3
#define DFB_MODE_BRICK_CLASSIFY 4
#define DFB_MODE_BRICK_STREAM 5
#define DFB_MODE_BRICK_MIXED 6
#define DFB_MODE_BRICK_UPDATE 7

typedef void* dfb_stream_t;

typedef struct dfb_volume {
    float* tsdf;
    float* weight;
    int rx, ry, rz;
    int x0, x1;
} dfb_volume;

typedef struct dfb_warpfield {
    const float* node_rec;
    const float* node_pos;
    const float* node_dq;
    const float* node_w;
    int n_nodes;
    int k;
    const uint16_t* knn;
    int has_lw;
    int lw_is_f32;
    double lw[8];
    const uint16_t* brick_nodes;
    const uint8_t* brick_count;
    const uint32_t* brick_pairs;
    const uint16_t* region_nodes;
    const uint8_t* region_count;
    const uint32_t* region_pairs;
    float* region_rec;
} dfb_warpfield;

typedef struct dfb_views {
    int n_views;
    const float* depth[DFB_MAX_VIEWS];
    int rows, cols;
    double K[9];
    double Kinv[9];
    int has_extrinsics;
    double E[DFB_MAX_VIEWS][12];
} dfb_views;

typedef struct dfb_workspace {
    uint32_t* list;
    uint32_t capacity;
    uint32_t* counters;
    uint8_t* brick_cls;
    uint32_t* brick_lists;
    uint32_t* overflow_bits;
} dfb_workspace;

int dfb_version(void);
const char* dfb_last_error(void);

int dfb_nodes_pack(const float* node_pos, const float* node_dq, const float* node_w, int n_nodes,
                   float* node_rec, dfb_stream_t stream);

int dfb_knn_build_volume(const float* node_pos, int n_nodes, int k, int rx, int ry, int rz, int x0, int x1,
                         uint16_t* knn, dfb_stream_t stream);
int64_t dfb_knn_brick_count(int slab_x, int ry, int rz);
int dfb_knn_build_volume_radii(const float* node_pos, int n_nodes, int k, int rx, int ry, int rz, int x0, int x1, uint16_t* knn,
                               float* brick_radius, dfb_stream_t stream);
int dfb_knn_update_volume(const float* node_pos, int n_old, int n_nodes, int k, int rx, int ry, int rz, int x0, int x1, uint16_t* knn,
                          float* brick_radius, uint8_t* dirty, dfb_stream_t stream);
int64_t dfb_brick_count(int slab_x, int ry, int rz);
int dfb_brick_nodes_build(const uint16_t* knn, int k, int rx, int ry, int rz, int x0, int x1, uint16_t* brick_nodes,
                          uint8_t* brick_count, uint32_t* brick_pairs, dfb_stream_t stream);
int64_t dfb_region_count(int slab_x, int ry, int rz);
int dfb_region_build(const uint16_t* knn, int k, int rx, int ry, int rz, int x0, int x1, uint16_t* region_nodes,
                     uint8_t* region_count, uint32_t* region_pairs, dfb_stream_t stream);
int dfb_brick_nodes_update(const uint16_t* knn, int k, int rx, int ry, int rz, int x0, int x1, const uint8_t* dirty8, uint16_t* brick_nodes,
                           uint8_t* brick_count, uint32_t* brick_pairs, dfb_stream_t stream);
int dfb_region_update(const uint16_t* knn, int k, int rx, int ry, int rz, int x0, int x1, const uint8_t* dirty8, uint16_t* region_nodes,
                      uint8_t* region_count, uint32_t* region_pairs, dfb_stream_t stream);
int dfb_knn_points(const float* pts, int64_t m, const float* node_pos, int n_nodes, int k, int32_t* idx,
                   dfb_stream_t stream);

int dfb_tsdf_update_projective(const dfb_volume* vol, const dfb_warpfield* wf, const dfb_views* views,
                               double tdist, double wmax, int mode, const dfb_workspace* ws,
                               uint8_t* mask_out, uint8_t* frustum_out, dfb_stream_t stream);

int dfb_tsdf_update_volume(const dfb_volume* vol, const dfb_warpfield* wf, const float* curr, int cx, int cy,
                           int cz, double tdist, double wmax, int mode, const dfb_workspace* ws,
                           uint8_t* mask_out, dfb_stream_t stream);

int dfb_fuse_depth_rigid(const dfb_volume* vol, int tsdf_res, const float* depth, int rows, int cols,
                         const double lw34[12], const double K[9], const double Kinv[9], double scale,
                         const double center[3], double tdist, double wmax, int mode, const dfb_workspace* ws,
                         uint8_t* mask_out, uint8_t* frustum_out, dfb_stream_t stream);

int dfb_warp_points(const float* pts, const float* normals, int64_t m, const int32_t* idx, const dfb_warpfield* wf,
                    double* out_pts, double* out_normals, dfb_stream_t stream);

int dfb_dq_blend_points(const float* pts, int64_t m, const int32_t* idx, const dfb_warpfield* wf, double* out_dq,
                        dfb_stream_t stream);

typedef struct dfb_gn_problem {
    int64_t n_vert;
    const float* vertices;
    const float* normals;
    const double* corr;
    const int32_t* vert_knn;
    int n_nodes, k;
    const float* node_pos;
    const float* node_w;
    const int32_t* node_nbr;
    double lw[8];
    int lw_is_f32;
    double rw;
    int huber;
    double f_scale;
    const int32_t* order;
} dfb_gn_problem;

int dfb_gn_residuals(const dfb_gn_problem* prob, const double* x, int x_is_f32, double* f_out, dfb_stream_t stream);
int dfb_gn_residuals_lw(const dfb_gn_problem* prob, const double* node_dq, int dq_is_f32, const double* lw, int lw_is_f32,
                        double* f_out, dfb_stream_t stream);
int dfb_gn_pattern_rows(const dfb_gn_problem* prob, uint32_t* bitmap, int32_t* row_ptr, dfb_stream_t stream);
int dfb_gn_pattern_cols(int n_nodes, const uint32_t* bitmap, const int32_t* row_ptr, int32_t* col_idx, dfb_stream_t stream);
int dfb_gn_normal_eq(const dfb_gn_problem* prob, const double* x, const int32_t* row_ptr, const int32_t* col_idx, int64_t nnzb,
                     double* H, double* g, double* cost, dfb_stream_t stream);
int dfb_gn_lw_normal_eq(const dfb_gn_problem* prob, const double* node_dq, const double* lw, double* H8, double* g8, double* cost,
                        dfb_stream_t stream);
int64_t dfb_gn_solve_workspace_doubles(int n_nodes);
int dfb_gn_solve(int n_nodes, const int32_t* row_ptr, const int32_t* col_idx, const double* H, const double* g, double lambda,
                 int max_iter, double tol, const double* x, double* x_new, double* delta, double* workspace, dfb_stream_t stream);

typedef struct dfb_point_grid {
    const float* pts;
    int64_t n;
    double origin[3];
    double cell;
    int dims[3];
    const int32_t* cell_start;
    const int32_t* order;
} dfb_point_grid;

int64_t dfb_point_grid_scratch_ints(int64_t cells);
int dfb_point_grid_build(const dfb_point_grid* g, int32_t* cell_start, int32_t* order, int32_t* scratch, dfb_stream_t stream);
int dfb_point_grid_knn(const dfb_point_grid* g, const double* queries, int64_t m, int k, int32_t* idx, double* dist2,
                       dfb_stream_t stream);
int dfb_corr_select(const double* warped_pts, const double* warped_normals, int64_t m, const float* live_verts,
                    const int32_t* nn, int k, int32_t* best, double* best_cost, dfb_stream_t stream);
int dfb_corr_projective(const double* warped_pts, const double* warped_normals, int64_t m, const dfb_views* views,
                        double max_distance, double min_normal_dot, int32_t* view, double* cost, double* corr,
                        dfb_stream_t stream);
int dfb_graph_unsupported(const float* verts, int64_t m, const int32_t* vert_knn, int k, const float* node_pos,
                          const float* node_w, uint8_t* unsupported, dfb_stream_t stream);
int dfb_graph_sample_rounds(const dfb_point_grid* g, double radius, int rounds, uint8_t* state, int32_t* undecided,
                            dfb_stream_t stream);

typedef struct dfb_mc_chunk {
    int32_t voff;
    uint32_t m[3];
} dfb_mc_chunk;

int64_t dfb_mc_level_scratch_floats(void);
int dfb_mc_level(const float* vol, int64_t n, float* scratch, float* level_out, dfb_stream_t stream);
int64_t dfb_mc_rows(int rx, int ry, int step);
int64_t dfb_mc_chunks(int rx, int ry, int rz, int step);
int dfb_mc_count(const float* vol, int rx, int ry, int rz, int step, int x_origin, const float* level, dfb_mc_chunk* chunks,
                 int32_t* row_voff, int32_t* row_toff, dfb_stream_t stream);
int dfb_mc_emit(const float* vol, int rx, int ry, int rz, int step, int x_origin, const float* level, const dfb_mc_chunk* chunks,
                const int32_t* row_voff, const int32_t* row_toff, float* verts, float* normals, float* values, int32_t* faces,
                dfb_stream_t stream);

#define DFB_COMM_ID_BYTES 128
#define DFB_COMM_SUM 0
#define DFB_COMM_MAX 1
typedef struct dfb_comm dfb_comm;
int dfb_comm_available(void);
int dfb_comm_unique_id(void* id_out);
int dfb_comm_init(dfb_comm** out, const void* id, int world, int rank, int device);
int dfb_comm_destroy(dfb_comm* c);
int dfb_comm_rank(const dfb_comm* c);
int dfb_comm_world(const dfb_comm* c);
int dfb_comm_broadcast(dfb_comm* c, void* buf, int64_t bytes, int root, dfb_stream_t stream);
int dfb_comm_broadcast_frame(dfb_comm* c, float* depths, int64_t n_depth, float* node_dq, int n_nodes, double* lw, int root,
                             dfb_stream_t stream);
int dfb_comm_allreduce_f64(dfb_comm* c, double* buf, int64_t n, int op, dfb_stream_t stream);
int dfb_comm_sendrecv(dfb_comm* c, const void* send_buf, int64_t send_bytes, int send_peer, void* recv_buf, int64_t recv_bytes,
                      int recv_peer, dfb_stream_t stream);

typedef struct dfb_frame_io {
    dfb_comm* comm;
    dfb_comm* comm_prefetch;
    int root;
    const float* dq_src;
    void* prefetch_dst;
    const void* prefetch_src;
    int64_t prefetch_bytes;
    uint32_t* counters_host;
} dfb_frame_io;
typedef struct dfb_frame_step dfb_frame_step;
int dfb_frame_step_create(dfb_frame_step** out);
void dfb_frame_step_destroy(dfb_frame_step* st);
int dfb_frame_step_run(dfb_frame_step* st, const dfb_volume* vol, const dfb_warpfield* wf, const dfb_views* views, double tdist,
                       double wmax, const dfb_workspace* ws, const dfb_frame_io* io, dfb_stream_t stream);
int dfb_frame_step_stats(const dfb_frame_step* st, int64_t out[5]);

#ifdef __cplusplus
}
#endif
#endif
```

Baseline: 220.3 billion.

## Cache per-voxel blend weights across TSDF updates in a persistent table

Adds a per-voxel table of the k Gaussian blend weights, stored as float and keyed by the volume slab. The exact warp path reads a weight row and uses it when the row is fully populated (no NaN sentinel); otherwise it computes the weights, including the double-precision exp, and writes them back. The table is filled with a NaN sentinel when built, cleared per dirty brick when nodes are appended, and dropped when nodes are reset. This trades repeated exp and distance math for 16–32 bytes of extra memory traffic per voxel, plus write-back on misses and extra VRAM for the table.

```diff
diff --git a/dynamicfusion_body_b200/_capi.py b/dynamicfusion_body_b200/_capi.py
--- a/dynamicfusion_body_b200/_capi.py
+++ b/dynamicfusion_body_b200/_capi.py
@@ -13,6 +13,7 @@
 MODE_BRICK_STREAM = 5
 MODE_BRICK_MIXED = 6
 MODE_BRICK_UPDATE = 7
+WEIGHT_TABLE_K = (4, 8)
 
 _PKG_DIR = os.path.dirname(os.path.abspath(__file__))
 LIB_PATH = os.environ.get("DFB_LIB") or os.path.join(_PKG_DIR, "libdfb_b200.so")
@@ -37,7 +38,7 @@
                 ("has_lw", C.c_int), ("lw_is_f32", C.c_int), ("lw", C.c_double * 8),
                 ("brick_nodes", C.c_void_p), ("brick_count", C.c_void_p), ("brick_pairs", C.c_void_p),
                 ("region_nodes", C.c_void_p), ("region_count", C.c_void_p), ("region_pairs", C.c_void_p),
-                ("region_rec", C.c_void_p)]
+                ("region_rec", C.c_void_p), ("knn_wf", C.c_void_p)]
 
 
 class Views(C.Structure):
@@ -80,6 +81,7 @@
         "knn_brick_count": ([C.c_int, C.c_int, C.c_int], C.c_int64),
         "knn_build_volume_radii": ([vp, C.c_int, C.c_int, C.c_int, C.c_int, C.c_int, C.c_int, C.c_int, vp, vp, vp], C.c_int),
         "knn_update_volume": ([vp, C.c_int, C.c_int, C.c_int, C.c_int, C.c_int, C.c_int, C.c_int, C.c_int, vp, vp, vp, vp], C.c_int),
+        "weight_table_reset": ([vp, C.c_int, C.c_int, C.c_int, C.c_int, C.c_int, C.c_int, vp, vp], C.c_int),
         "brick_nodes_update": ([vp, C.c_int, C.c_int, C.c_int, C.c_int, C.c_int, C.c_int, vp, vp, vp, vp, vp], C.c_int),
         "region_update": ([vp, C.c_int, C.c_int, C.c_int, C.c_int, C.c_int, C.c_int, vp, vp, vp, vp, vp], C.c_int),
         "brick_count": ([C.c_int, C.c_int, C.c_int], C.c_int64),
@@ -172,7 +174,7 @@
     "dfb_gn_lw_normal_eq", "dfb_gn_solve_workspace_doubles", "dfb_gn_solve",
     "dfb_point_grid_scratch_ints", "dfb_point_grid_build", "dfb_point_grid_knn", "dfb_corr_select", "dfb_corr_projective", "dfb_graph_unsupported", "dfb_graph_sample_rounds",
     "dfb_mc_level_scratch_floats", "dfb_mc_level", "dfb_mc_rows", "dfb_mc_chunks", "dfb_mc_count", "dfb_mc_emit",
-    "dfb_knn_brick_count", "dfb_knn_build_volume_radii", "dfb_knn_update_volume", "dfb_brick_nodes_update", "dfb_region_update",
+    "dfb_knn_brick_count", "dfb_knn_build_volume_radii", "dfb_knn_update_volume", "dfb_weight_table_reset", "dfb_brick_nodes_update", "dfb_region_update",
     "dfb_comm_available", "dfb_comm_unique_id", "dfb_comm_init", "dfb_comm_destroy", "dfb_comm_rank", "dfb_comm_world",
     "dfb_comm_broadcast", "dfb_comm_broadcast_frame", "dfb_comm_allreduce_f64", "dfb_comm_sendrecv",
     "dfb_frame_step_create", "dfb_frame_step_destroy", "dfb_frame_step_run", "dfb_frame_step_stats",
diff --git a/dynamicfusion_body_b200/csrc/dfb_math.h b/dynamicfusion_body_b200/csrc/dfb_math.h
--- a/dynamicfusion_body_b200/csrc/dfb_math.h
+++ b/dynamicfusion_body_b200/csrc/dfb_math.h
@@ -115,22 +115,38 @@
     return fsqrt((float)s);
 }
 
+DFB_HD bool weight_row_full(const float* r, int k) {
+    bool full = true;
+    for (int i = 0; i < k; ++i) full = full && r[i] == r[i];
+    return full;
+}
+
 template <int KT = 0>
 DFB_HDN void dq_blend_ref(const float* p, const int* ids, int k_rt, const float* node_pos, const float* node_dq,
-                          const float* node_w, double* se3, float* wi_out, double* n2_out = nullptr, const float4* rec = nullptr) {
+                          const float* node_w, double* se3, float* wi_out, double* n2_out = nullptr, const float4* rec = nullptr,
+                          const float* wf_in = nullptr, float* wf_out = nullptr) {
     double b[8] = {0, 0, 0, 0, 0, 0, 0, 0};
     float wi = 0.f;
     const int k = KT > 0 ? KT : k_rt;
-    double wts[KT > 0 ? KT : 1];
+    float wts[KT > 0 ? KT : 1];
     if (KT > 0) {
+        if (wf_in && weight_row_full(wf_in, KT)) {
 #pragma unroll
-        for (int i = 0; i < (KT > 0 ? KT : 1); ++i) {
-            float nx, ny, nz;
-            if (rec) { const float4 r0 = rec[3 * (size_t)ids[i]]; nx = r0.x; ny = r0.y; nz = r0.z; }
-            else { const float* np_ = node_pos + 3 * (size_t)ids[i]; nx = np_[0]; ny = np_[1]; nz = np_[2]; }
-            const float nrm = norm3_f32_ref(p[0], p[1], p[2], nx, ny, nz);
-            const float q = fdiv(nrm, fmul(2.0f, node_w[ids[i]]));
-            wts[i] = exp((double)fmul(-1.0f, fmul(q, q)));
+            for (int i = 0; i < (KT > 0 ? KT : 1); ++i) wts[i] = wf_in[i];
+        } else {
+#pragma unroll
+            for (int i = 0; i < (KT > 0 ? KT : 1); ++i) {
+                float nx, ny, nz;
+                if (rec) { const float4 r0 = rec[3 * (size_t)ids[i]]; nx = r0.x; ny = r0.y; nz = r0.z; }
+                else { const float* np_ = node_pos + 3 * (size_t)ids[i]; nx = np_[0]; ny = np_[1]; nz = np_[2]; }
+                const float nrm = norm3_f32_ref(p[0], p[1], p[2], nx, ny, nz);
+                const float q = fdiv(nrm, fmul(2.0f, node_w[ids[i]]));
+                wts[i] = (float)exp((double)fmul(-1.0f, fmul(q, q)));
+            }
+            if (wf_out) {
+#pragma unroll
+                for (int i = 0; i < (KT > 0 ? KT : 1); ++i) wf_out[i] = wts[i];
+            }
         }
     }
 #pragma unroll
@@ -141,17 +157,16 @@
             if (rec) { const float4 r0 = rec[3 * (size_t)id]; npx = r0.x; npy = r0.y; npz = r0.z; }
             else { const float* np_ = node_pos + 3 * (size_t)id; npx = np_[0]; npy = np_[1]; npz = np_[2]; }
         }
-        double w;
+        float wf;
         if (KT > 0) {
-            w = wts[KT > 0 ? i : 0];
+            wf = wts[KT > 0 ? i : 0];
         } else {
             const float nrm = norm3_f32_ref(p[0], p[1], p[2], npx, npy, npz);
             const float two_w = fmul(2.0f, node_w[id]);
             const float q = fdiv(nrm, two_w);
             const float arg = fmul(-1.0f, fmul(q, q));
-            w = exp((double)arg);
-        }
-        const float wf = (float)w;
+            wf = (float)exp((double)arg);
+        }
         float dqi[8];
         if (rec) {
             const float4 r1 = rec[3 * (size_t)id + 1], r2 = rec[3 * (size_t)id + 2];
@@ -193,18 +208,19 @@
 template <int KT = 0>
 DFB_HDN void warp_ref(const float* p, const float* nrm_in, const int* ids, int k, const float* node_pos,
                       const float* node_dq, const float* node_w, const double* lw, bool has_lw, bool lw_is_f32,
-                      double* out_p, double* out_n, float* wi_out, bool closed_form = false, const float4* rec = nullptr) {
+                      double* out_p, double* out_n, float* wi_out, bool closed_form = false, const float4* rec = nullptr,
+                      const float* wf_in = nullptr, float* wf_out = nullptr) {
     double pd[3] = {(double)p[0], (double)p[1], (double)p[2]};
     double se3[8];
     if (k > 0) {
         if (closed_form && !(nrm_in && out_n)) {
             double n2;
-            dq_blend_ref<KT>(p, ids, k, node_pos, node_dq, node_w, se3, wi_out, &n2, rec);
+            dq_blend_ref<KT>(p, ids, k, node_pos, node_dq, node_w, se3, wi_out, &n2, rec, wf_in, wf_out);
             dqb_warp_closed(se3, pd, out_p);
             const double inv = 1.0 / n2;
             out_p[0] *= inv; out_p[1] *= inv; out_p[2] *= inv;
         } else {
-            dq_blend_ref<KT>(p, ids, k, node_pos, node_dq, node_w, se3, wi_out, nullptr, rec);
+            dq_blend_ref<KT>(p, ids, k, node_pos, node_dq, node_w, se3, wi_out, nullptr, rec, wf_in, wf_out);
             if (closed_form) dqb_warp_closed(se3, pd, out_p);
             else dqb_warp_ref(se3, false, pd, out_p);
         }
diff --git a/dynamicfusion_body_b200/csrc/dfb_params.h b/dynamicfusion_body_b200/csrc/dfb_params.h
--- a/dynamicfusion_body_b200/csrc/dfb_params.h
+++ b/dynamicfusion_body_b200/csrc/dfb_params.h
@@ -68,6 +68,7 @@
         DFB_REQUIRE(wf->node_rec && wf->node_pos && wf->node_dq && wf->node_w, "node arrays are null");
         DFB_REQUIRE(wf->n_nodes >= wf->k && wf->n_nodes <= 65535, "n_nodes=%d must be in [k,65535]", wf->n_nodes);
         if (need_knn) DFB_REQUIRE(wf->knn, "knn table is null");
+        DFB_REQUIRE(((uintptr_t)wf->knn_wf & 15) == 0, "blend weight table must be 16-byte aligned");
     }
     return DFB_OK;
 }
@@ -116,6 +117,7 @@
     P.scale = 1.0;
     P.node_rec = reinterpret_cast<const float4*>(wf->node_rec);
     P.node_pos = wf->node_pos; P.node_dq = wf->node_dq; P.node_w = wf->node_w; P.knn = wf->knn; P.k = wf->k;
+    P.knn_wf = wf->knn_wf;
     P.has_lw = wf->has_lw; P.lw_is_f32 = wf->lw_is_f32;
     for (int i = 0; i < 8; ++i) P.lw[i] = wf->lw[i];
     P.n_views = views->n_views; P.rows = views->rows; P.cols = views->cols; P.has_E = views->has_extrinsics;
@@ -196,6 +198,7 @@
     P.rx = vol->rx; P.ry = vol->ry; P.rz = vol->rz; P.x0 = vol->x0; P.x1 = vol->x1;
     P.node_rec = reinterpret_cast<const float4*>(wf->node_rec);
     P.node_pos = wf->node_pos; P.node_dq = wf->node_dq; P.node_w = wf->node_w; P.knn = wf->knn; P.k = wf->k;
+    P.knn_wf = wf->knn_wf;
     P.has_lw = wf->has_lw; P.lw_is_f32 = wf->lw_is_f32;
     for (int i = 0; i < 8; ++i) P.lw[i] = wf->lw[i];
     double A[12];
diff --git a/dynamicfusion_body_b200/csrc/dfb_voxel.h b/dynamicfusion_body_b200/csrc/dfb_voxel.h
--- a/dynamicfusion_body_b200/csrc/dfb_voxel.h
+++ b/dynamicfusion_body_b200/csrc/dfb_voxel.h
@@ -20,6 +20,7 @@
     const float* node_dq;
     const float* node_w;
     const uint16_t* knn;
+    float* knn_wf;
     int k;
     int has_lw, lw_is_f32;
     double lw[8];
@@ -59,6 +60,7 @@
     const float* node_dq;
     const float* node_w;
     const uint16_t* knn;
+    float* knn_wf;
     int k;
     int has_lw, lw_is_f32;
     double lw[8];
@@ -167,7 +169,7 @@
 
 template <int KT = 0>
 DFB_HDN void voxel_projective_exact(const ProjParams& P, int x, int y, int z, const uint16_t* ids16, float* v_io,
-                                    float* w_io, int* mask, int* frus) {
+                                    float* w_io, int* mask, int* frus, const float* wf_in = nullptr, float* wf_out = nullptr) {
     double base[3];
     if (P.rigid) {
         const double idx[3] = {(double)x, (double)y, (double)z};
@@ -185,7 +187,7 @@
 #define DFB_EXACT_REC 0
 #endif
         warp_ref<KT>(p, nullptr, ids, P.k, P.node_pos, P.node_dq, P.node_w, P.lw, P.has_lw != 0, P.lw_is_f32 != 0, base,
-                     nullptr, nullptr, true, DFB_EXACT_REC ? P.node_rec : nullptr);
+                     nullptr, nullptr, true, DFB_EXACT_REC ? P.node_rec : nullptr, wf_in, wf_out);
     }
     double v = (double)*v_io, w = (double)*w_io;
     int m = 0, f = 0;
@@ -250,7 +252,8 @@
 }
 
 template <int KT = 0>
-DFB_HDN bool voxel_volume_exact(const VolParams& P, int x, int y, int z, const uint16_t* ids16, float* v_io, float* w_io) {
+DFB_HDN bool voxel_volume_exact(const VolParams& P, int x, int y, int z, const uint16_t* ids16, float* v_io, float* w_io,
+                                const float* wf_in = nullptr, float* wf_out = nullptr) {
     const float p[3] = {(float)x, (float)y, (float)z};
     int ids[8];
     if (KT > 0) {
@@ -261,7 +264,8 @@
     }
     double pw[3];
     float wi = 0.f;
-    warp_ref<KT>(p, nullptr, ids, P.k, P.node_pos, P.node_dq, P.node_w, P.lw, P.has_lw != 0, P.lw_is_f32 != 0, pw, nullptr, &wi, true);
+    warp_ref<KT>(p, nullptr, ids, P.k, P.node_pos, P.node_dq, P.node_w, P.lw, P.has_lw != 0, P.lw_is_f32 != 0, pw, nullptr, &wi, true,
+                 nullptr, wf_in, wf_out);
     double tl = 0.0;
     const bool valid = interpolate_tsdf_ref(pw, P.curr, P.cx, P.cy, P.cz, &tl);
     double v = (double)*v_io, w = (double)*w_io;
diff --git a/dynamicfusion_body_b200/csrc/knn.cu b/dynamicfusion_body_b200/csrc/knn.cu
--- a/dynamicfusion_body_b200/csrc/knn.cu
+++ b/dynamicfusion_body_b200/csrc/knn.cu
@@ -362,6 +362,20 @@
     if (changed) changed_s = 1;
     __syncthreads();
     if (threadIdx.x == 0) dirty[b] = changed_s ? 1 : 0;
+}
+
+__global__ void __launch_bounds__(128) weight_reset_kernel(const uint8_t* dirty8, int k, int sx, int ry, int rz, int nby, int nbz, float* knn_wf) {
+    const int b = blockIdx.x;
+    if (!dirty8[b]) return;
+    const int bz = b % nbz, by = (b / nbz) % nby, bxs = b / (nbz * nby);
+    const int xlo = bxs * KB, ylo = by * KB, zlo = bz * KB;
+    for (int q = 0; q < 4; ++q) {
+        const int j = threadIdx.x * 4 + q;
+        const int z = zlo + (j & 7), y = ylo + ((j >> 3) & 7), xs = xlo + (j >> 6);
+        if (!(xs < sx && y < ry && z < rz)) continue;
+        const size_t i = ((size_t)xs * ry + y) * rz + z;
+        for (int a = 0; a < k; ++a) knn_wf[i * (size_t)k + a] = __uint_as_float(DFB_WEIGHT_EMPTY);
+    }
 }
 
 template <int KMAX>
@@ -439,6 +453,22 @@
     return knn_build(node_pos, n_old, n_nodes, k, rx, ry, rz, x0, x1, knn, brick_radius, dirty, stream);
 }
 
+extern "C" int dfb_weight_table_reset(const uint8_t* dirty8, int k, int rx, int ry, int rz, int x0, int x1, float* knn_wf, dfb_stream_t stream) {
+    DFB_REQUIRE(knn_wf, "null pointer");
+    DFB_REQUIRE(k >= 1 && k <= DFB_MAX_K, "k=%d out of range [1,%d]", k, DFB_MAX_K);
+    DFB_REQUIRE(rx > 0 && ry > 0 && rz > 0 && x0 >= 0 && x1 > x0 && x1 <= rx, "bad grid / slab");
+    cudaStream_t s = (cudaStream_t)stream;
+    if (!dirty8) {
+        DFB_CUDA(cudaMemsetAsync(knn_wf, 0xFF, (size_t)(x1 - x0) * ry * rz * k * sizeof(float), s));
+        return DFB_OK;
+    }
+    const int64_t nby = (ry + KB - 1) / KB, nbz = (rz + KB - 1) / KB, nb = dfb_knn_brick_count(x1 - x0, ry, rz);
+    DFB_REQUIRE(nb < ((int64_t)1 << 31), "too many bricks");
+    weight_reset_kernel<<<(unsigned)nb, 128, 0, s>>>(dirty8, k, x1 - x0, ry, rz, (int)nby, (int)nbz, knn_wf);
+    DFB_LAUNCH_CHECK("weight_reset_kernel");
+    return DFB_OK;
+}
+
 extern "C" int dfb_knn_points(const float* pts, int64_t m, const float* node_pos, int n_nodes, int k, int32_t* idx,
                               dfb_stream_t stream) {
     DFB_REQUIRE(pts && node_pos && idx, "null pointer");
diff --git a/dynamicfusion_body_b200/csrc/tsdf.cu b/dynamicfusion_body_b200/csrc/tsdf.cu
--- a/dynamicfusion_body_b200/csrc/tsdf.cu
+++ b/dynamicfusion_body_b200/csrc/tsdf.cu
@@ -838,8 +838,24 @@
                                        blockIdx.x * UPDATE_SMEM_GROUPS + (threadIdx.x >> 7), n_groups, n_t, threadIdx.x & 127, RecShared{rec_a}, Q);
 }
 
+template <int KT>
+__device__ __forceinline__ void load_wrow(const float* tab, size_t i, float* r) {
+    if (KT > 0 && tab) {
+        const float4* q = reinterpret_cast<const float4*>(tab + i * (size_t)KT);
+#pragma unroll
+        for (int j = 0; j < (KT > 0 ? KT : 4) / 4; ++j) {
+            const float4 v = q[j];
+            r[4 * j] = v.x; r[4 * j + 1] = v.y; r[4 * j + 2] = v.z; r[4 * j + 3] = v.w;
+        }
+    } else {
+#pragma unroll
+        for (int j = 0; j < (KT > 0 ? KT : 1); ++j) r[j] = __uint_as_float(DFB_WEIGHT_EMPTY);
+    }
+}
+
 template <int KMAX, int KT>
-__device__ __forceinline__ void exact_voxel(const ProjParams& P, size_t i, size_t nvox, size_t plane, const uint16_t* ids, float v, float w) {
+__device__ __forceinline__ bool exact_voxel(const ProjParams& P, size_t i, size_t nvox, size_t plane, const uint16_t* ids, float v, float w,
+                                            const float* wrow) {
     int xs, y, z;
     if (nvox <= 0xffffffffull) {
         const uint32_t i32 = (uint32_t)i, plane32 = (uint32_t)plane, rz32 = (uint32_t)P.rz;
@@ -852,13 +868,14 @@
         z = (int)(rem - (size_t)y * P.rz);
     }
     int m, f;
-    voxel_projective_exact<KT>(P, xs + P.x0, y, z, ids, &v, &w, &m, &f);
+    voxel_projective_exact<KT>(P, xs + P.x0, y, z, ids, &v, &w, &m, &f, wrow, KT > 0 && P.knn_wf ? P.knn_wf + i * (size_t)(KT > 0 ? KT : 1) : nullptr);
     if (m) {
         P.tsdf[i] = v;
         P.weight[i] = w;
     }
     if (P.mask_out) P.mask_out[i] = (uint8_t)m;
     if (P.frustum_out) P.frustum_out[i] = (uint8_t)f;
+    return KT > 0 && weight_row_full(wrow, KT > 0 ? KT : 1);
 }
 
 #ifndef DFB_EXACT_MINB
@@ -874,7 +891,8 @@
     const size_t n = use_list ? (size_t)(overflow ? P.capacity : count) : nvox;
     const size_t plane = (size_t)P.ry * P.rz;
     const int kk = KT > 0 ? KT : P.k;
-    uint32_t done = 0;
+    constexpr int KW = KT > 0 ? KT : 1;
+    uint32_t done = 0, hits = 0;
     if (use_list && KT > 0 && !P.rigid && nvox <= 0xffffffffull) {
         const uint32_t stride = gridDim.x * blockDim.x, cnt = (uint32_t)n;
         uint32_t t = blockIdx.x * blockDim.x + threadIdx.x;
@@ -882,21 +900,27 @@
             uint32_t i0 = P.list[t];
             uint32_t i1 = t + stride < cnt && t + stride >= t ? P.list[t + stride] : i0;
             uint16_t ids0[KMAX];
+            float wr0[KW];
             load_ids<KMAX>(P.knn, i0, KMAX, ids0);
+            load_wrow<KT>(P.knn_wf, i0, wr0);
             float v0 = P.tsdf[i0], w0 = P.weight[i0];
             for (;;) {
                 const uint32_t tn = t + stride, tnn = tn + stride;
                 const bool has1 = tn < cnt && tn > t;
                 const uint32_t i2 = (has1 && tnn < cnt && tnn > tn) ? P.list[tnn] : i1;
                 uint16_t ids1[KMAX];
+                float wr1[KW];
                 load_ids<KMAX>(P.knn, i1, KMAX, ids1);
+                load_wrow<KT>(P.knn_wf, i1, wr1);
                 const float v1 = P.tsdf[i1], w1 = P.weight[i1];
-                exact_voxel<KMAX, KT>(P, i0, nvox, plane, ids0, v0, w0);
+                hits += exact_voxel<KMAX, KT>(P, i0, nvox, plane, ids0, v0, w0, wr0);
                 ++done;
                 if (!has1) break;
                 t = tn; i0 = i1; i1 = i2; v0 = v1; w0 = w1;
 #pragma unroll
                 for (int j = 0; j < KMAX; ++j) ids0[j] = ids1[j];
+#pragma unroll
+                for (int j = 0; j < KW; ++j) wr0[j] = wr1[j];
             }
         }
     } else {
@@ -909,7 +933,9 @@
                 int m0, f0;
                 if (voxel_projective_classify<KMAX>(P, (int)xq + P.x0, (int)(rem / P.rz), (int)(rem % P.rz), ids, &m0, &f0) != CLS_UNCERTAIN) continue;
             }
-            exact_voxel<KMAX, KT>(P, i, nvox, plane, ids, P.tsdf[i], P.weight[i]);
+            float wr[KW];
+            load_wrow<KT>(P.knn_wf, i, wr);
+            hits += exact_voxel<KMAX, KT>(P, i, nvox, plane, ids, P.tsdf[i], P.weight[i], wr);
             ++done;
         }
     }
@@ -926,13 +952,19 @@
                 const size_t i = wd * 32 + (size_t)lane;
                 uint16_t ids[KMAX];
                 if (!P.rigid) load_ids<KMAX>(P.knn, i, kk, ids);
-                exact_voxel<KMAX, KT>(P, i, nvox, plane, ids, P.tsdf[i], P.weight[i]);
+                float wr[KW];
+                load_wrow<KT>(P.knn_wf, i, wr);
+                hits += exact_voxel<KMAX, KT>(P, i, nvox, plane, ids, P.tsdf[i], P.weight[i], wr);
                 ++done;
             }
         }
     }
-    for (int o = 16; o > 0; o >>= 1) done += __shfl_xor_sync(0xffffffffu, done, o);
+    for (int o = 16; o > 0; o >>= 1) {
+        done += __shfl_xor_sync(0xffffffffu, done, o);
+        hits += __shfl_xor_sync(0xffffffffu, hits, o);
+    }
     if ((threadIdx.x & 31) == 0 && done) atomicAdd(P.counters + 1, done);
+    if ((threadIdx.x & 31) == 0 && hits) atomicAdd(P.counters + 5, hits);
 }
 
 #ifndef DFB_VOL_FAST_MINB
@@ -971,7 +1003,7 @@
 }
 
 template <int KMAX, int KT>
-__device__ __forceinline__ void vol_exact_voxel(const VolParams& P, size_t i, size_t plane) {
+__device__ __forceinline__ bool vol_exact_voxel(const VolParams& P, size_t i, size_t plane) {
     int xs, y, z;
     if (plane * (size_t)(P.x1 - P.x0) <= 0xffffffffull) {
         const uint32_t i32 = (uint32_t)i, plane32 = (uint32_t)plane, rz32 = (uint32_t)P.rz;
@@ -985,13 +1017,16 @@
     }
     uint16_t ids[KMAX];
     if (P.k > 0) load_ids<KMAX>(P.knn, i, P.k, ids);
+    float wr[KT > 0 ? KT : 1];
+    load_wrow<KT>(P.knn_wf, i, wr);
     float v = P.tsdf[i], w = P.weight[i];
-    const bool upd = voxel_volume_exact<KT>(P, xs + P.x0, y, z, ids, &v, &w);
+    const bool upd = voxel_volume_exact<KT>(P, xs + P.x0, y, z, ids, &v, &w, wr, KT > 0 && P.knn_wf ? P.knn_wf + i * (size_t)(KT > 0 ? KT : 1) : nullptr);
     if (upd) {
         P.tsdf[i] = v;
         P.weight[i] = w;
     }
     if (P.mask_out) P.mask_out[i] = upd ? 1 : 0;
+    return KT > 0 && weight_row_full(wr, KT > 0 ? KT : 1);
 }
 
 #ifndef DFB_VOL_EXACT_MINB
@@ -1006,7 +1041,7 @@
     const bool use_list = !all_mode && (!overflow || sweep_bits);
     const size_t n = use_list ? (size_t)(overflow ? P.capacity : count) : nvox;
     const size_t plane = (size_t)P.ry * P.rz;
-    uint32_t done = 0;
+    uint32_t done = 0, hits = 0;
     for (size_t t = (size_t)blockIdx.x * blockDim.x + threadIdx.x; t < n; t += (size_t)gridDim.x * blockDim.x) {
         const size_t i = use_list ? (size_t)P.list[t] : t;
         if (!use_list && !all_mode) {
@@ -1017,7 +1052,7 @@
             float wi;
             if (voxel_volume_classify<KMAX>(P, xs + P.x0, (int)(rem / P.rz), (int)(rem % P.rz), ids, &wi) != CLS_UNCERTAIN) continue;
         }
-        vol_exact_voxel<KMAX, KT>(P, i, plane);
+        hits += vol_exact_voxel<KMAX, KT>(P, i, plane);
         ++done;
     }
     if (sweep_bits) {
@@ -1030,13 +1065,17 @@
             __syncwarp();
             if (lane == 0) P.overflow_bits[wd] = 0u;
             if ((bits >> lane) & 1u) {
-                vol_exact_voxel<KMAX, KT>(P, wd * 32 + (size_t)lane, plane);
+                hits += vol_exact_voxel<KMAX, KT>(P, wd * 32 + (size_t)lane, plane);
                 ++done;
             }
         }
     }
-    for (int o = 16; o > 0; o >>= 1) done += __shfl_xor_sync(0xffffffffu, done, o);
+    for (int o = 16; o > 0; o >>= 1) {
+        done += __shfl_xor_sync(0xffffffffu, done, o);
+        hits += __shfl_xor_sync(0xffffffffu, hits, o);
+    }
     if ((threadIdx.x & 31) == 0 && done) atomicAdd(P.counters + 1, done);
+    if ((threadIdx.x & 31) == 0 && hits) atomicAdd(P.counters + 5, hits);
 }
 
 __global__ void warp_points_kernel(const float* pts, const float* normals, int64_t m, const int32_t* idx, int k,
diff --git a/dynamicfusion_body_b200/engine.py b/dynamicfusion_body_b200/engine.py
--- a/dynamicfusion_body_b200/engine.py
+++ b/dynamicfusion_body_b200/engine.py
@@ -58,7 +58,7 @@
     def _decode(self, c):
         c = c.astype(np.int64) & 0xffffffff
         return {"deferred": int(c[0]), "exact_processed": int(c[1]), "bricks_streamed": int(c[2]), "bricks_mixed": int(c[3]),
-                "bricks": self.n_bricks, "dqb_voxels": int(c[4])}
+                "bricks": self.n_bricks, "dqb_voxels": int(c[4]), "weight_cache_hits": int(c[5])}
 
     def stats(self):
         return self._decode(self.counters.cpu().numpy())
@@ -115,14 +115,16 @@
 
 class DeviceWarpField:
 
-    def __init__(self, k, device=None):
+    def __init__(self, k, device=None, weight_cache=None):
         self.device = _require_cuda(device)
         self.k = int(k)
+        self.weight_cache = os.environ.get("DFB_WEIGHT_CACHE", "1") != "0" if weight_cache is None else bool(weight_cache)
         self.n_nodes = 0
         self.node_pos = self.node_dq = self.node_w = self.node_rec = None
         self._knn = {}
         self._knn_radii = {}
         self._bricks = {}
+        self._wtab = {}
 
     def set_nodes(self, node_pos, node_dq, node_w):
         n = len(node_pos)
@@ -133,6 +135,7 @@
         self._knn = {}
         self._knn_radii = {}
         self._bricks = {}
+        self._wtab = {}
         self.node_dq = None
         self.set_dq(node_dq)
 
@@ -167,7 +170,15 @@
                                                          _ptr(radii), _stream()))
                 self._knn_radii[key] = radii
             self._knn[key] = t
+            if self.weight_cache and self.k in _capi.WEIGHT_TABLE_K:
+                wt = torch.empty((n, self.k), dtype=torch.float32, device=self.device)
+                _capi.check(L.dfb_weight_table_reset(None, self.k, res[0], res[1], res[2], x0, x1, _ptr(wt), _stream()))
+                self._wtab[key] = wt
         return t
+
+    def weight_table(self, res, x0, x1):
+        self.knn_table(res, x0, x1)
+        return self._wtab.get((tuple(res), x0, x1))
 
     def append_nodes(self, node_pos, node_dq, node_w):
         m = len(node_pos)
@@ -191,11 +202,15 @@
             if radii is None or n_old < self.k:
                 del self._knn[key]
                 self._bricks.pop(key, None)
+                self._wtab.pop(key, None)
                 continue
             dirty = torch.empty(radii.numel(), dtype=torch.uint8, device=self.device)
             _capi.check(L.dfb_knn_update_volume(_ptr(self.node_pos), n_old, self.n_nodes, self.k, res[0], res[1], res[2], x0, x1, _ptr(t),
                                                 _ptr(radii), _ptr(dirty), _stream()))
             self.last_dirty = dirty
+            wt = self._wtab.get(key)
+            if wt is not None:
+                _capi.check(L.dfb_weight_table_reset(_ptr(dirty), self.k, res[0], res[1], res[2], x0, x1, _ptr(wt), _stream()))
             b = self._bricks.get(key)
             if b is not None:
                 nodes, count, pairs, rnodes, rcount, rpairs, rrec = b
@@ -233,7 +248,7 @@
         _capi.check(_capi.lib().dfb_knn_points(_ptr(p), p.shape[0], _ptr(self.node_pos), self.n_nodes, k, _ptr(out), _stream()))
         return out
 
-    def struct(self, lw=None, knn=None, k=None, bricks=None):
+    def struct(self, lw=None, knn=None, k=None, bricks=None, weights=None):
         s = _capi.WarpField()
         if bricks is not None:
             s.brick_nodes = bricks[0].data_ptr()
@@ -253,6 +268,7 @@
         s.n_nodes = self.n_nodes
         s.k = k
         s.knn = knn.data_ptr() if knn is not None else None
+        s.knn_wf = weights.data_ptr() if weights is not None else None
         fill_lw(s, lw)
         return s
 
@@ -309,7 +325,7 @@
     ws = vol.workspace.struct(use_bricks)
     mask, frus = _mask_bufs(vol, want_masks)
     v = vol.struct()
-    s = wf.struct(lw, knn, bricks=bricks)
+    s = wf.struct(lw, knn, bricks=bricks, weights=wf.weight_table(vol.res, vol.x0, vol.x1))
     _capi.check(_capi.lib().dfb_tsdf_update_projective(C.byref(v), C.byref(s), C.byref(views), float(tdist), float(wmax),
                                                        int(mode), C.byref(ws), _ptr(mask), _ptr(frus), _stream()))
     return (mask, frus) if want_masks else None
@@ -322,7 +338,7 @@
     ws = vol.workspace.struct(False)
     mask = torch.zeros(vol.n_voxels, dtype=torch.uint8, device=vol.device) if want_masks else None
     v = vol.struct()
-    s = wf.struct(lw, knn, k=k) if wf is not None else _rigid_struct(lw)
+    s = wf.struct(lw, knn, k=k, weights=None if rigid else wf.weight_table(vol.res, vol.x0, vol.x1)) if wf is not None else _rigid_struct(lw)
     _capi.check(_capi.lib().dfb_tsdf_update_volume(C.byref(v), C.byref(s), _ptr(curr), curr.shape[0], curr.shape[1],
                                                    curr.shape[2], float(tdist), float(wmax), int(mode), C.byref(ws),
                                                    _ptr(mask), _stream()))
@@ -581,9 +597,10 @@
         self.vol, self.wf, self.views = vol, wf, views
         knn = wf.knn_table(vol.res, vol.x0, vol.x1)
         bricks = wf.brick_nodes(vol.res, vol.x0, vol.x1)
-        self._keep = (knn, bricks)
+        weights = wf.weight_table(vol.res, vol.x0, vol.x1)
+        self._keep = (knn, bricks, weights)
         self._v = vol.struct()
-        self._w = wf.struct(lw, knn, bricks=bricks)
+        self._w = wf.struct(lw, knn, bricks=bricks, weights=weights)
         self._ws = vol.workspace.struct(True)
         self.tdist, self.wmax = float(tdist), float(wmax)
 
diff --git a/include/dfb.h b/include/dfb.h
--- a/include/dfb.h
+++ b/include/dfb.h
@@ -51,6 +51,7 @@
     const uint8_t* region_count;
     const uint32_t* region_pairs;
     float* region_rec;
+    float* knn_wf;
 } dfb_warpfield;
 
 typedef struct dfb_views {
@@ -85,6 +86,8 @@
                                float* brick_radius, dfb_stream_t stream);
 int dfb_knn_update_volume(const float* node_pos, int n_old, int n_nodes, int k, int rx, int ry, int rz, int x0, int x1, uint16_t* knn,
                           float* brick_radius, uint8_t* dirty, dfb_stream_t stream);
+#define DFB_WEIGHT_EMPTY 0xFFFFFFFFu
+int dfb_weight_table_reset(const uint8_t* dirty8, int k, int rx, int ry, int rz, int x0, int x1, float* knn_wf, dfb_stream_t stream);
 int64_t dfb_brick_count(int slab_x, int ry, int rz);
 int dfb_brick_nodes_build(const uint16_t* knn, int k, int rx, int ry, int rz, int x0, int x1, uint16_t* brick_nodes,
                           uint8_t* brick_count, uint32_t* brick_pairs, dfb_stream_t stream);
```

After: 223.9 billion (median of 6 runs). 1.02x the previous value.
